# mickeysjm/TaxoExpan

Hardware: AMD Instinct MI355X
Metric: egonet_edges_per_sec_pgat_fwd_bwd (higher is better)
Workload: dtype f32; 1 GPU; MAG-CS synthetic taxonomy (29,654 nodes, d=250), PGAT+WMR+LBM fp32 dims 250/50/500/500 heads [4,1], 128 queries x 32 = 4096 egonets per GPU per step, fwd + InfoNCE + bwd + Adam(amsgrad), dropout 0.1; parallelism=dp1, settle_steps=256

## Files before the change

### include/txe.h

```cpp
#ifndef TXE_H
#define TXE_H
#include <stddef.h>

#ifdef __cplusplus
extern "C" {
#endif

#define TXE_OK 0
#define TXE_ERR_ARG -1
#define TXE_ERR_LAUNCH -2
#define TXE_ERR_WORKSPACE -3

size_t txe_dropout_mask_bytes(long long n_rows, int n_cols);
int txe_dropout_mask(long long n_rows, int n_cols, float p, unsigned long long seed, unsigned* mask, void* stream);

int txe_gat_padded_k(int Kh, int Pd);
int txe_gat_padded_f(int H, int D);
int txe_gat_pack_weights(const float* W, const float* attn_l, const float* attn_r, int H, int D, int Kt, float* Wp, void* stream);
int txe_gat_build_x(const float* h, long long ld_h, int n_nodes, int Kh, const int* pos, const float* P, int Pd, float* X, void* stream);

int txe_gat_layer_prepare(const float* h, long long ld_h, int n_nodes, int Kh, const int* pos, const float* P, int Pd, float* X,
                          const float* W, const float* attn_l, const float* attn_r, int H, int D, float* Wp, float feat_drop_p,
                          unsigned long long seed, unsigned* mask, void* stream);

struct txe_gat_prepare_desc {
    const float* h; long long ld_h; int n_nodes, Kh; const int* pos; const float* P; int Pd; float* X;
    const float *W, *attn_l, *attn_r; int H, D; float* Wp; float feat_drop_p; unsigned long long seed; unsigned* mask;
    int x_dropped;
};
int txe_gat_layers_prepare(const struct txe_gat_prepare_desc* descs, int n_layers, void* stream);

int txe_gcn_layer_prepare(const float* h, long long ld_h, int n_nodes, int Kh, const int* pos, const float* P, int Pd, float* X,
                          const float* W, int Fo, float* Wp, float drop_p, unsigned long long seed, unsigned* mask, int x_dropped,
                          const float* bias_row ,
                          void* stream);
struct txe_gcn_prepare_desc {
    const float* h; long long ld_h; int n_nodes, Kh; const int* pos; const float* P; int Pd; float* X;
    const float* W; int Fo; float* Wp; float drop_p; unsigned long long seed; unsigned* mask; int x_dropped; const float* bias_row;
};
int txe_gcn_layers_prepare(const struct txe_gcn_prepare_desc* descs, int n_layers, const int* rowptr_in, int n_nodes, float* norm, void* stream);

int txe_gather_add_rows(const float* T, long long ld_t, const int* row, const float* T2, long long ld_t2, const int* row2, long long n_rows,
                        int n_cols, float* Y, long long ld_y, void* stream);
size_t txe_gat_dense_ws_bytes(int n_nodes, int Kh, int Pd, int H, int D, int vocab);
int txe_gat_dense_fwd(const float* X, int n_nodes, int Kh, int Pd, const float* Wp, int H, int D, float feat_drop_p,
                      const unsigned* mask, float* Y, void* ws, size_t ws_bytes, void* stream);
size_t txe_gat_dense_split_ws_bytes(int n_nodes, int Kh, int Pd, int H, int D);
size_t txe_gat_dense_split_xt_bytes(int n_nodes, int Kh, int Pd, int H, int D);
int txe_gat_dense_fwd_split(const float* X, int n_nodes, int Kh, int Pd, const float* Wp, int H, int D, const void* Xs, const void* Ws,
                            void* Xt_out, float* Y, void* ws, size_t ws_bytes, void* stream);
int txe_gat_dense_fwd_split_src(const float* h, long long ld_h, const int* pos, const float* P, const unsigned* mask, float feat_drop_p,
                                int n_nodes, int Kh, int Pd, const float* Wp, int H, int D, void* Xt_out, float* Y, void* ws, size_t ws_bytes,
                                void* stream);
int txe_gat_dense_bwd(const float* X, int n_nodes, int Kh, int Pd, const int* pos, int vocab, const float* Wp, const float* W,
                      const float* attn_l, const float* attn_r, int H, int D, float feat_drop_p, const unsigned* mask, const float* d_Y,
                      int need_dh, int act_on, float act_slope, float* d_X, float* dW, float* d_attn_l, float* d_attn_r, float* dP,
                      int x_dropped, const void* Xt, int phases, void* chain, void* ws, size_t ws_bytes, void* stream);
size_t txe_gat_dense_bwd_split_ws_bytes(int n_nodes, int Kh, int Pd, int H, int D);
#define TXE_TAIL_CHAIN_BYTES 1024
int txe_gat_tail_flush(void* chain, void* stream);
int txe_zero_cols(float* x, long long ld, int n_rows, int c0, int c1, void* stream);
int txe_gat_dx_streams(int Kh, int Pd, int need_dh);

int txe_gat_aggregate_table_supported(int H, int D, long long ld_t, int vocab, int nx_kp);
int txe_gat_aggregate_table_fwd(const int* rowptr_in, const int* col_src, int n_nodes, const float* T, long long ld_t, const int* rid,
                                const float* T2, const int* pos, int vocab, int H, int D, float attn_slope, int out_mode,
                                float act_slope, float* out, long long ld_out, const float* nx_wa, int nx_kp, float* nx_a12,
                                int npw, void* stream);

int txe_gat_aggregate_fwd(const int* rowptr_in, const int* col_src, int n_nodes, const float* ft, long long ld_ft,
                          const float* a_src, const float* a_dst, int ld_a, int H, int D, float attn_slope, float attn_drop_p,
                          unsigned long long seed, int out_mode, float act_slope, float* out, long long ld_out, float* alpha,
                          const float* nx_wa, int nx_kp, const unsigned* nx_mask, float nx_feat_drop_p, float* nx_a12, int npw, void* stream);
int txe_gat_aggregate_bwd(const int* rowptr_in, const int* col_src, const int* rowptr_out, const int* col_dst,
                          const int* pos_out, int n_nodes, const float* ft, long long ld_ft, const float* a_src,
                          const float* a_dst, int ld_a, int H, int D, float attn_slope, float attn_drop_p,
                          unsigned long long seed, const float* alpha, const float* d_pre, long long ld_dpre, float* d_ft,
                          long long ld_dft, float* d_a_src, float* d_a_dst, int ld_da, float* dz_ws, int n_pad, void* stream);
int txe_leaky_relu_bwd(const float* d_out, const float* out_act, float slope, long long n, float* d_pre, void* stream);
int txe_head_mean_fwd(const float* x, int H, int D, long long n_rows, float* y, void* stream);
int txe_head_mean_bwd(const float* dy, int H, int D, long long n_rows, float* dx, void* stream);

int txe_gcn_padded_f(int Fo);
int txe_gcn_pack_weights(const float* W, int Kt, int Fo, float* Wp, void* stream);
size_t txe_gcn_dense_ws_bytes(int n_nodes, int Kh, int Pd, int Fo, int vocab);
int txe_gcn_dense_fwd(const float* X, int n_nodes, int Kh, int Pd, const float* Wp, int Fo, float drop_p, const unsigned* mask,
                      float* hw, void* ws, size_t ws_bytes, void* stream);
int txe_gcn_dense_bwd(const float* X, int n_nodes, int Kh, int Pd, const int* pos, int vocab, const float* Wp, int Fo, float drop_p,
                      const unsigned* mask, const float* d_hw, int need_dh, int act_on, float act_slope, float* d_X, float* dW,
                      float* dP, int x_dropped, void* ws, size_t ws_bytes, void* stream);
int txe_gcn_norm(const int* rowptr_in, int n_nodes, float* norm, void* stream);
int txe_gcn_aggregate_fwd(const int* rowptr_in, const int* col_src, int n_nodes, const float* hw, long long ld_hw,
                          const float* norm, const float* bias, int has_act, float act_slope, int F, float* out, long long ld_out,
                          void* stream);
size_t txe_gcn_aggregate_bwd_ws_bytes(int n_nodes, int F);
int txe_gcn_aggregate_bwd(const int* rowptr_out, const int* col_dst, int n_nodes, const float* d_pre, long long ld_dpre,
                          const float* norm, int F, float* d_hw, long long ld_dhw, float* d_bias, void* ws, size_t ws_bytes,
                          void* stream);

int txe_readout_fwd(const int* graph_off, int G, const float* h, long long ld_h, const int* pos, const float* pw, int D,
                    float* hg, float* wsum, void* stream);
int txe_readout_bwd(const int* graph_off, int G, const float* h, long long ld_h, const int* pos, const float* pw, int vocab,
                    int D, const float* hg, const float* wsum, const float* d_hg, float* d_h, long long ld_dh, float* d_pw,
                    float* dpw_ws, void* stream);

int txe_readout_multi_fwd(const int* graph_off, int G, const float* h, long long ld_h, const int* pos, int D, int mode, float* hg,
                          int* argmax, void* stream);
int txe_readout_multi_bwd(const int* graph_off, int G, const int* pos, int D, int mode, const float* d_hg, const int* argmax,
                          float* d_h, long long ld_dh, void* stream);

int txe_bilinear_project(const float* e1, long long ld_e1, int G, int l, const float* W, int r, float* U, long long ld_u,
                         void* sws, size_t sws_bytes, void* stream);
int txe_bilinear_pair_fwd(const float* e1, long long ld_e1, const float* e2, long long ld_e2, int G, int l, int r,
// ... 195 lines not shown
```

### taxoexpan_amd/_lib.py

```python
import ctypes as C
import os

_HERE = os.path.dirname(os.path.abspath(__file__))
LIB_PATH = os.path.join(_HERE, "csrc", "libtxe.so")
TAIL_CHAIN_BYTES = 1024

P, I, L, F, D, U64, SZ = C.c_void_p, C.c_int, C.c_longlong, C.c_float, C.c_double, C.c_ulonglong, C.c_size_t

SIGNATURES = {
    "txe_dropout_mask_bytes": (SZ, [L, I]),
    "txe_dropout_mask": (I, [L, I, F, U64, P, P]),
    "txe_gat_padded_k": (I, [I, I]),
    "txe_gat_padded_f": (I, [I, I]),
    "txe_gat_pack_weights": (I, [P, P, P, I, I, I, P, P]),
    "txe_gat_build_x": (I, [P, L, I, I, P, P, I, P, P]),
    "txe_gat_layer_prepare": (I, [P, L, I, I, P, P, I, P, P, P, P, I, I, P, F, U64, P, P]),
    "txe_gcn_layer_prepare": (I, [P, L, I, I, P, P, I, P, P, I, P, F, U64, P, I, P, P]),
    "txe_gcn_layers_prepare": (I, [P, I, P, I, P, P]),
    "txe_gather_add_rows": (I, [P, L, P, P, L, P, L, I, P, L, P]),
    "txe_gat_dense_ws_bytes": (SZ, [I, I, I, I, I, I]),
    "txe_gat_dense_fwd": (I, [P, I, I, I, P, I, I, F, P, P, P, SZ, P]),
    "txe_gat_dense_split_ws_bytes": (SZ, [I, I, I, I, I]),
    "txe_gat_dense_split_xt_bytes": (SZ, [I, I, I, I, I]),
    "txe_gat_dense_bwd_split_ws_bytes": (SZ, [I, I, I, I, I]),
    "txe_gat_dense_fwd_split": (I, [P, I, I, I, P, I, I, P, P, P, P, P, SZ, P]),
    "txe_gat_dense_bwd": (I, [P, I, I, I, P, I, P, P, P, P, I, I, F, P, P, I, I, F, P, P, P, P, P, I, P, I, P, P, SZ, P]),
    "txe_gat_tail_flush": (I, [P, P]),
    "txe_zero_cols": (I, [P, L, I, I, I, P]),
    "txe_gat_dx_streams": (I, [I, I, I]),
    "txe_gat_aggregate_fwd": (I, [P, P, I, P, L, P, P, I, I, I, F, F, U64, I, F, P, L, P, P, I, P, F, P, I, P]),
    "txe_gat_aggregate_table_supported": (I, [I, I, L, I, I]),
    "txe_gat_aggregate_table_fwd": (I, [P, P, I, P, L, P, P, P, I, I, I, F, I, F, P, L, P, I, P, I, P]),
    "txe_gat_aggregate_bwd": (I, [P, P, P, P, P, I, P, L, P, P, I, I, I, F, F, U64, P, P, L, P, L, P, P, I, P, I, P]),
    "txe_leaky_relu_bwd": (I, [P, P, F, L, P, P]),
    "txe_head_mean_fwd": (I, [P, I, I, L, P, P]),
    "txe_head_mean_bwd": (I, [P, I, I, L, P, P]),
    "txe_gcn_padded_f": (I, [I]),
    "txe_gcn_pack_weights": (I, [P, I, I, P, P]),
    "txe_gcn_dense_ws_bytes": (SZ, [I, I, I, I, I]),
    "txe_gcn_dense_fwd": (I, [P, I, I, I, P, I, F, P, P, P, SZ, P]),
    "txe_gcn_dense_bwd": (I, [P, I, I, I, P, I, P, I, F, P, P, I, I, F, P, P, P, I, P, SZ, P]),
    "txe_gcn_norm": (I, [P, I, P, P]),
    "txe_gcn_aggregate_fwd": (I, [P, P, I, P, L, P, P, I, F, I, P, L, P]),
    "txe_gcn_aggregate_bwd_ws_bytes": (SZ, [I, I]),
    "txe_gcn_aggregate_bwd": (I, [P, P, I, P, L, P, I, P, L, P, P, SZ, P]),
    "txe_readout_fwd": (I, [P, I, P, L, P, P, I, P, P, P]),
    "txe_readout_bwd": (I, [P, I, P, L, P, P, I, I, P, P, P, P, L, P, P, P]),
    "txe_readout_multi_fwd": (I, [P, I, P, L, P, I, I, P, P, P]),
    "txe_readout_multi_bwd": (I, [P, I, P, I, I, P, P, P, L, P]),
    "txe_linear_fwd": (I, [P, L, I, P, L, I, I, P, P, I, I, P, P]),
    "txe_linear_bwd_ws_bytes": (SZ, [I, I, I, I]),
    "txe_linear_bwd": (I, [P, L, I, P, L, I, I, P, I, I, P, P, P, L, P, L, P, P, P, SZ, P]),
    "txe_bilinear_project": (I, [P, L, I, I, P, I, P, L, P, SZ, P]),
    "txe_bilinear_pair_fwd": (I, [P, L, P, L, I, I, I, P, I, P, P, P]),
    "txe_bilinear_query_fwd": (I, [P, L, P, L, I, I, I, P, I, P, P, P]),
    "txe_bilinear_query_project": (I, [P, L, I, I, I, P, P, P]),
    "txe_bilinear_query_dot": (I, [P, L, P, I, I, I, P, P]),
    "txe_bilinear_query_bwd_ws_bytes": (SZ, [I, I, I]),
    "txe_bilinear_query_bwd": (I, [P, L, P, L, I, I, I, I, P, P, P, P, L, P, P, SZ, P]),
    "txe_bilinear_runs_fwd": (I, [P, L, P, L, P, I, I, I, I, P, I, P, P, P]),
    "txe_bilinear_runs_bwd_ws_bytes": (SZ, [I, I, I]),
    "txe_bilinear_runs_bwd": (I, [P, L, P, L, P, I, I, I, I, I, P, P, P, P, L, P, P, SZ, P]),
    "txe_rows_find_runs": (I, [P, L, I, I, P, P, P, P]),
    "txe_score_topk_tiles": (I, [I]),
    "txe_score_topk_block": (I, [P, L, I, P, L, I, I, I, I, I, I, P, P, P, P, P, P, SZ, P, P]),
    "txe_topk_merge": (I, [P, P, I, L, I, I, P, P, P]),
    "txe_bilinear_stacked_fwd": (I, [P, L, P, L, P, P, I, I, I, P, I, P, P, P]),
    "txe_bilinear_stacked_bwd_ws_bytes": (SZ, [I, I, I]),
    "txe_bilinear_stacked_bwd": (I, [P, L, P, L, P, P, I, I, I, I, P, P, P, P, L, P, P, SZ, P]),
    "txe_bilinear_folded_fwd": (I, [P, L, I, I, P, L, I, P, L, I, P, P, I, I, P, I, P, P, P, I, I, I, P]),
    "txe_runs_expand": (I, [P, I, I, P, P]),
    "txe_bilinear_folded_bwd": (I, [P, L, I, I, P, L, I, P, L, I, P, P, I, I, I, P, P, P, P, P, L, P, P, P, P, I, I, P]),
    "txe_bilinear_pair_bwd_ws_bytes": (SZ, [I, I, I]),
    "txe_bilinear_pair_bwd": (I, [P, L, P, L, I, I, I, P, I, P, P, P, P, L, P, L, P, P, SZ, P]),
    "txe_score_block": (I, [P, L, I, P, L, I, I, I, P, L, P, SZ, P, SZ, P, P]),
    "txe_mlp_padded_h": (I, [I]),
    "txe_mlp_project": (I, [P, L, I, I, P, P, P, P, P, P]),
    "txe_mlp_query_project": (I, [P, L, I, I, P, I, P, P, P, P, P]),
    "txe_mlp_score_block": (I, [P, P, I, P, P, P, I, I, P, P, L, P]),
    "txe_mlp_score_positives": (I, [P, P, I, P, P, P, I, I, P, P, P, I, P, P]),
    "txe_mlp_score_count_block": (I, [P, P, I, P, P, P, I, I, P, P, P, I, P, P]),
    "txe_mlp_score_topk_block": (I, [P, P, I, P, P, P, I, I, P, I, I, I, P, P, P, P, P, P]),
    "txe_score_split_ws_bytes": (SZ, [I, I, I]),
    "txe_score_count_block": (I, [P, L, I, P, L, I, I, I, P, P, I, P, P, SZ, P, P]),
    "txe_score_positives": (I, [P, L, I, P, L, I, I, I, P, P, P, SZ, P]),
    "txe_rank_finalize": (I, [P, I, P, P, I, P, P]),
    "txe_gemm_tail_ws_bytes": (SZ, []),
    "txe_gemm_plain_split_ws_bytes": (SZ, [I, I, I]),
    "txe_gat_collapse_split_ws_bytes": (SZ, [I, I, I, I]),
    "txe_gemm_plain": (I, [I, P, L, P, L, P, L, I, I, I, I, I, P, SZ, P]),
    "txe_build_csr_ws_bytes": (SZ, [I, I]),
    "txe_build_csr": (I, [P, P, I, I, P, P, P, P, P, P, P, SZ, P]),
    "txe_rank_block": (I, [P, L, I, I, P, P, P, I, P, P]),
    "txe_gat_collapse_ws_bytes": (SZ, [I, I, I, I, I, I, I]),
    "txe_gat_collapse_fwd": (I, [P, P, P, P, P, P, I, I, I, P, I, I, P, I, F, P, F, F, U64, P, P, P, I, P, P, P, P, P, P, L, P, P, P, P, SZ, P]),
    "txe_gat_collapse_e_tiles": (I, [I, I, I, I]),
    "txe_gat_collapse_fold_scores": (I, [P, I, I, I, I, P, P, P, F, I, I, P, P]),
    "txe_gat_collapse_bwd": (I, [P, P, P, P, P, P, I, I, I, P, I, I, P, I, P, P, P, P, I, F, P, F, F, U64, P, P, P, P, P, P, P, P, L, P, L, I, F,
                                 P, P, P, P, P, P, P, SZ, P]),
    "txe_gat_layers_prepare": (I, [P, I, P]),
    "txe_gat_fused_bwd_supported": (I, [I, I, I, I]),
    "txe_gat_collapse_bwd_fused_ws_bytes": (SZ, [I, I, I, I, I, I, I, I]),
    "txe_gat_collapse_bwd_fused": (I, [P, P, P, P, P, P, I, I, I, P, I, I, P, I, P, P, P, P, I, F, P, F, F, U64, P, P, P, P, P, P, P, P, L, P, L,
                                       F, P, L, I, I, F, F, U64, P, P, L, I, P, P, P, P, P, P, I, P, I, P, P, P, I, P, P, P, P, P, P, SZ, P]),
    "txe_gat_dense_fwd_split_src": (I, [P, L, P, P, P, F, I, I, I, P, I, I, P, P, P, SZ, P]),
    "txe_egonet_walk_plan_bytes": (SZ, [I]),
    "txe_egonet_walk_plan": (I, [P, P, P, P, P, P, I, I, P, P]),
    "txe_gcn_collapse_ws_bytes": (SZ, [I, I, I, I, I, I]),
    "txe_gcn_collapse_fwd": (I, [P, P, P, I, I, P, I, I, P, I, P, F, P, P, P, P, P, P, P, P, P, L, P, SZ, P]),
    "txe_gcn_collapse_bwd": (I, [P, P, P, I, I, P, I, I, P, I, P, I, F, P, P, P, P, P, P, P, P, L, I, F, P, P, P, P, P, I, P, SZ, P]),
    "txe_egonet_ws_bytes": (SZ, [I]),
    "txe_egonet_offsets": (I, [P, P, P, P, P, I, I, U64, I, P, P, SZ, P]),
    "txe_egonet_fill": (I, [P, P, P, P, P, P, I, I, U64, I, P, P, P, P, P, P, P, P, P, P]),
    "txe_sample_anchors": (I, [P, I, I, I, P, P, P, P, P, P, I, P, I, U64, I, I, P, P, P]),
    "txe_sample_groups": (I, [P, I, I, I, P, P, P, P, P, P, I, I, U64, I, I, I, P, P, P, P, P, P]),
    "txe_group_rank_ws_bytes": (SZ, [I]),
    "txe_group_rank": (I, [P, P, I, I, I, P, P, P, P, SZ, P]),
    "txe_group_metrics": (I, [P, P, P, U64, I, P, P]),
    "txe_info_nce": (I, [P, L, I, I, P, P, P, L, P]),
    "txe_adam_step": (I, [I, P, P, P, P, P, P, D, D, D, D, D, L, P]),
    "txe_dropout_uniform_host": (F, [U64, U64]),
    "txe_dropout_mask_word_host": (C.c_uint, [U64, U64, F]),
    "txe_profile_enable": (I, [I]),
    "txe_profile_reset": (I, []),
    "txe_profile_count": (I, []),
    "txe_profile_get": (I, [I, P, I, P, P, P]),
    "txe_profile_stream": (I, [I, P]),
    "txe_stream_order": (I, [P, P]),
    "txe_copy_stream": (I, [P, P, L, P]),
    "txe_split_packed_bytes": (SZ, [I, I]),
    "txe_split_pack": (I, [P, L, I, I, I, P, P]),
    "txe_split_packed_t_bytes": (SZ, [I, I]),
    "txe_split_pack_t": (I, [P, L, I, I, P, P]),
    "txe_gemm_tn_split": (I, [P, L, I, P, I, I, I, I, P, L, L, P]),
    "txe_gemm_nt_split": (I, [P, P, I, I, I, P, L, P]),
}

class GatPrepareDesc(C.Structure):
    _fields_ = [("h", P), ("ld_h", L), ("n_nodes", I), ("Kh", I), ("pos", P), ("P", P), ("Pd", I), ("X", P), ("W", P), ("attn_l", P),
                ("attn_r", P), ("H", I), ("D", I), ("Wp", P), ("feat_drop_p", F), ("seed", U64), ("mask", P), ("x_dropped", I)]


class GcnPrepareDesc(C.Structure):
    _fields_ = [("h", P), ("ld_h", L), ("n_nodes", I), ("Kh", I), ("pos", P), ("P", P), ("Pd", I), ("X", P), ("W", P), ("Fo", I), ("Wp", P),
                ("drop_p", F), ("seed", U64), ("mask", P), ("x_dropped", I), ("bias_row", P)]


_ERR = {-1: "TXE_ERR_ARG", -2: "TXE_ERR_LAUNCH", -3: "TXE_ERR_WORKSPACE"}
VALUE_RETURNING = {"txe_gat_padded_k", "txe_gat_collapse_e_tiles", "txe_gat_padded_f", "txe_gcn_padded_f", "txe_profile_count", "txe_gat_fused_bwd_supported",
                   "txe_gat_aggregate_table_supported", "txe_gat_dx_streams", "txe_score_topk_tiles",
                   "txe_mlp_padded_h"}

_lib = None


class TxeError(RuntimeError):
    pass


def load():
    global _lib
    if _lib is not None:
        return _lib
    if not os.path.exists(LIB_PATH):
        raise TxeError(f"HIP extension missing: {LIB_PATH} not built -- run taxoexpan_amd/csrc/build.py "
                       "(there is no CPU fallback)")
    lib = C.CDLL(LIB_PATH)
    for name, (res, args) in SIGNATURES.items():
        fn = getattr(lib, name)
        fn.restype, fn.argtypes = res, args
    _lib = lib
    return lib


_bound = {}


def call(name, *args):
    ent = _bound.get(name)
    if ent is None:
        ent = _bound[name] = (getattr(load(), name), SIGNATURES[name][0] is I and name not in VALUE_RETURNING)
    rc = ent[0](*args)
    if rc != 0 and ent[1]:
        raise TxeError(f"{name} failed: {_ERR.get(rc, rc)}")
    return rc


_pure = {}
_get_device = None


def _current_device():
    global _get_device
    if _get_device is None:
        import torch
        _get_device = torch._C._cuda_getDevice if torch.cuda.is_available() else (lambda: -1)
    return _get_device()


def pure(name, *args):
    key = (name, _current_device()) + args
    v = _pure.get(key)
    if v is None:
        if len(_pure) > 4096:
            _pure.clear()
        v = _pure[key] = call(name, *args)
    return v


class _NoGuard:
    def __enter__(self):
        return None

    def __exit__(self, *exc):
        return False


_NO_GUARD = _NoGuard()


def on_device(dev):
    import torch
    if dev.index is None or dev.index == torch.cuda.current_device():
        return _NO_GUARD
    return torch.cuda.device(dev)
# ... 20 lines not shown
```

### taxoexpan_amd/csrc/build.py

```python
#!/usr/bin/env python3
import concurrent.futures as cf
import os
import subprocess
import sys

HERE = os.path.dirname(os.path.abspath(__file__))
SOURCES = ["txe_gemm_nt.hip", "txe_gemm_nn.hip", "txe_gemm_tn.hip", "txe_gemm_split.hip", "txe_gat.hip", "txe_gcn.hip", "txe_project.hip", "txe_fold.hip", "txe_fold_bwd.hip", "txe_dxpos.hip", "txe_readout.hip", "txe_match.hip",
           "txe_graph.hip", "txe_rank.hip", "txe_profile.hip", "txe_egonet.hip", "txe_optim.hip", "txe_loss.hip",
           "txe_mlp_score.hip", "txe_sample.hip", "txe_grouprank.hip"]
HEADERS = ["txe_common.h", "txe_gemm.h", "txe_gather.h", "txe_colsum.h", "txe_dxpos.h", "txe_gemm_tnlds.h", "txe_skinny.h", "txe_gemm_split.h", "txe_tail.h", "txe_fold.h"]
LIB = os.path.join(HERE, "libtxe.so")
OBJ_DIR = os.path.join(HERE, "build")
HIPCC = os.environ.get("HIPCC", "/opt/rocm/bin/hipcc")
FLAGS = ["--offload-arch=gfx950", "-O3", "-std=c++17", "-fPIC", "-Wall", "-Wno-unused-function"] + os.environ.get("TXE_HIPCC_FLAGS", "").split()


def _newer(a, b):
    return (not os.path.exists(b)) or os.path.getmtime(a) > os.path.getmtime(b)


def _compile(src):
    obj = os.path.join(OBJ_DIR, src.replace(".hip", ".o"))
    deps = [os.path.join(HERE, src)] + [os.path.join(HERE, h) for h in HEADERS]
    if not any(_newer(d, obj) for d in deps):
        return obj, ""
    cmd = [HIPCC] + FLAGS + ["-c", os.path.join(HERE, src), "-o", obj]
    r = subprocess.run(cmd, capture_output=True, text=True)
    if r.returncode != 0:
        raise RuntimeError(f"hipcc failed for {src}:\n{r.stdout}\n{r.stderr}")
    return obj, r.stderr


def build(force=False, verbose=True):
    os.makedirs(OBJ_DIR, exist_ok=True)
    srcs = [s for s in SOURCES if os.path.exists(os.path.join(HERE, s))]
    if force:
        for s in srcs:
            o = os.path.join(OBJ_DIR, s.replace(".hip", ".o"))
            if os.path.exists(o):
                os.remove(o)
    with cf.ThreadPoolExecutor(max_workers=min(8, len(srcs))) as ex:
        results = list(ex.map(_compile, srcs))
    objs = [o for o, _ in results]
    warn = "".join(w for _, w in results)
    if verbose and warn.strip():
        print(warn, file=sys.stderr)
    if force or any(_newer(o, LIB) for o in objs):
        cmd = [HIPCC, "--offload-arch=gfx950", "-shared", "-fPIC"] + objs + ["-o", LIB]
        r = subprocess.run(cmd, capture_output=True, text=True)
        if r.returncode != 0:
            raise RuntimeError(f"link failed:\n{r.stdout}\n{r.stderr}")
    return LIB


if __name__ == "__main__":
    print(build(force="--force" in sys.argv))
```

### taxoexpan_amd/csrc/txe_gemm_split.h

```cpp
#pragma once
#include <hip/hip_runtime.h>
#include <stdint.h>

namespace txe {

constexpr int SPL_BM = 128, SPL_BN = 128, SPL_KT = 16;
constexpr int SPL_FRAG_BYTES = 1024;

static inline size_t split_packed_bytes(int rows, int cols) {
    const size_t rb = (size_t)((rows + 767) / 768) * 24, nkt = (size_t)(cols + SPL_KT - 1) / SPL_KT;
    return rb * nkt * 3 * SPL_FRAG_BYTES;
}

static inline size_t split_pair_bytes(int M, int N, int K) {
    return (split_packed_bytes(M, K) + 255) / 256 * 256 + (split_packed_bytes(N, K) + 255) / 256 * 256;
}

typedef float split_f2 __attribute__((ext_vector_type(2)));
typedef __bf16 split_b2 __attribute__((ext_vector_type(2)));
__device__ __forceinline__ unsigned pk_bf16(float lo, float hi) {
    const split_f2 v = {lo, hi};
    return __builtin_bit_cast(unsigned, __builtin_convertvector(v, split_b2));
}
__device__ __forceinline__ void split3x2(float x0, float x1, unsigned& w1, unsigned& w2, unsigned& w3) {
    w1 = pk_bf16(x0, x1);
    const float r0 = x0 - __uint_as_float(w1 << 16), r1 = x1 - __uint_as_float(w1 & 0xffff0000u);
    w2 = pk_bf16(r0, r1);
    const float q0 = r0 - __uint_as_float(w2 << 16), q1 = r1 - __uint_as_float(w2 & 0xffff0000u);
    w3 = pk_bf16(q0, q1);
}
constexpr unsigned SPL_RAW_MARK = 0x7FC07FC0u;
__device__ __forceinline__ bool split_exceptional(float x) {
    return (__float_as_uint(x) & 0x7fffffffu) >= (247u << 23);
}
__device__ __forceinline__ void split_raw2(float x0, float x1, unsigned& w1, unsigned& w2, unsigned& w3) {
    const unsigned b0 = __float_as_uint(x0), b1 = __float_as_uint(x1);
    w1 = (b0 >> 16) | (b1 & 0xffff0000u);
    w2 = (b0 & 0xffffu) | (b1 << 16);
    w3 = SPL_RAW_MARK;
}
__device__ __forceinline__ void split_decode8(const uint4& w1, const uint4& w2, const uint4& w3, float (&x)[8]) {
    const unsigned a[4] = {w1.x, w1.y, w1.z, w1.w}, b[4] = {w2.x, w2.y, w2.z, w2.w}, c[4] = {w3.x, w3.y, w3.z, w3.w};
    const bool raw = c[0] == SPL_RAW_MARK;
#pragma unroll
    for (int i = 0; i < 4; ++i) {
        if (raw) {
            x[2 * i] = __uint_as_float((a[i] << 16) | (b[i] & 0xffffu));
            x[2 * i + 1] = __uint_as_float((a[i] & 0xffff0000u) | (b[i] >> 16));
        } else {
            x[2 * i] = (__uint_as_float(a[i] << 16) + __uint_as_float(b[i] << 16)) + __uint_as_float(c[i] << 16);
            x[2 * i + 1] = (__uint_as_float(a[i] & 0xffff0000u) + __uint_as_float(b[i] & 0xffff0000u)) + __uint_as_float(c[i] & 0xffff0000u);
        }
    }
}
__device__ __forceinline__ bool not_finite(float v) { return (__float_as_uint(v) & 0x7f800000u) == 0x7f800000u; }

__device__ __forceinline__ void split3x8(const float (&x)[8], uint4& w1, uint4& w2, uint4& w3) {
    split3x2(x[0], x[1], w1.x, w2.x, w3.x);
    split3x2(x[2], x[3], w1.y, w2.y, w3.y);
    split3x2(x[4], x[5], w1.z, w2.z, w3.z);
    split3x2(x[6], x[7], w1.w, w2.w, w3.w);
}
__device__ __forceinline__ void split_raw8(const float (&x)[8], uint4& w1, uint4& w2, uint4& w3) {
    split_raw2(x[0], x[1], w1.x, w2.x, w3.x);
    split_raw2(x[2], x[3], w1.y, w2.y, w3.y);
    split_raw2(x[4], x[5], w1.z, w2.z, w3.z);
    split_raw2(x[6], x[7], w1.w, w2.w, w3.w);
}
__device__ __forceinline__ bool split_exceptional8(const float (&x)[8]) {
    bool bad = false;
#pragma unroll
    for (int q = 0; q < 8; ++q) bad |= split_exceptional(x[q]);
    return bad;
}
__device__ __forceinline__ void split3x4(const float (&x)[4], uint2& w1, uint2& w2, uint2& w3) {
    split3x2(x[0], x[1], w1.x, w2.x, w3.x);
    split3x2(x[2], x[3], w1.y, w2.y, w3.y);
}
__device__ __host__ __forceinline__ int split_slot_row(int side, int rb, int s) {
    return side == 0 ? 32 * rb + s : 128 * (rb >> 2) + 64 * ((rb & 3) >> 1) + 2 * s + (rb & 1);
}

static inline size_t split_packed_t_bytes(int rows, int cols) {
    return (size_t)((rows + 15) / 16) * (size_t)(((cols + 159) / 160) * 5) * 3 * SPL_FRAG_BYTES;
}
static inline bool split_tn_eligible(int M, int N) { return M % 128 == 0 && N % 4 == 0 && M > 0 && N > 0; }
static inline bool split_tn_fits(int n_rows, long long lda) { return (double)n_rows * (double)lda * 4.0 < 2147483648.0; }

int split_pack_launch(const float* src, long long ld, int rows, int cols, int side, void* packed, hipStream_t stream);
struct SplitEpi {
    const unsigned* mask; int mask_ld, mask_col0; float drop_scale;
    const float* act_src; long long ld_act; float act_slope; int cols_act;
};
int gemm_nt_split_launch(const void* Ap, const void* Bp, int M, int N, int K, float* C, long long ldc, double alg_flops, hipStream_t stream,
                         const SplitEpi* epi = nullptr);
int split_pack_t_launch(const float* src, long long ld, int rows, int cols, void* packed, hipStream_t stream);
struct Epi;
int gemm_nt_split_epi_launch(const void* Ap, const void* Bp, const Epi& E, int M, int N, int K, hipStream_t stream);
struct SplitVSrc { const float* h; long long ld_h; const int* pos; const float* P; int Kh, Pd; const unsigned* mask; int wpr; float scale; };
int split_pack_layer_launch(const float* X, long long ldx, int n, const float* W, long long ldw, int f, int K, int Kt_cols, void* Xs, void* Ws,
                            void* Xt, hipStream_t stream, const SplitVSrc* vs = nullptr);
int gemm_tn_split_launch(const float* A, long long lda, int M, const void* Bt, int N, int n_rows, int S, int ksplit, float* part, long long ldc,
                         long long split_stride, double alg_flops, hipStream_t stream);

}
```

### taxoexpan_amd/csrc/txe_gemm_split.hip

```cpp
#include <string.h>
#include "txe_common.h"
#include "txe_gemm.h"
#include "txe_gemm_split.h"

namespace txe {

typedef __attribute__((ext_vector_type(8))) short bf16x8;
typedef __attribute__((ext_vector_type(16))) float f32x16s;

template <int NC, int R>
__device__ __forceinline__ void vsrc_load_rows(const SplitVSrc& v, const int (&row)[R], const int c0, float (&x)[R][NC]) {
    unsigned word[R];
    const bool masked = v.mask != nullptr && c0 < v.wpr * 32;
#pragma unroll
    for (int r = 0; r < R; ++r) word[r] = masked ? v.mask[(long long)row[r] * v.wpr + (c0 >> 5)] : 0xFFFFFFFFu;
    if (c0 + NC <= v.Kh) {
        const bool two = (NC & 1) == 0 && ((reinterpret_cast<uintptr_t>(v.h + c0) & 7) == 0) && (v.ld_h & 1) == 0;
        if (two) {
#pragma unroll
            for (int r = 0; r < R; ++r) {
                const float* hr = v.h + (long long)row[r] * v.ld_h + c0;
#pragma unroll
                for (int q = 0; q + 1 < NC; q += 2) { const float2 t = *reinterpret_cast<const float2*>(hr + q); x[r][q] = t.x; x[r][q + 1] = t.y; }
            }
        } else {
#pragma unroll
            for (int r = 0; r < R; ++r)
#pragma unroll
                for (int q = 0; q < NC; ++q) x[r][q] = v.h[(long long)row[r] * v.ld_h + c0 + q];
        }
    } else if (c0 >= v.Kh + v.Pd) {
#pragma unroll
        for (int r = 0; r < R; ++r)
#pragma unroll
            for (int q = 0; q < NC; ++q) x[r][q] = 0.f;
        return;
    } else {
        int pr[R];
#pragma unroll
        for (int r = 0; r < R; ++r) pr[r] = (v.Pd > 0) ? v.pos[row[r]] : 0;
#pragma unroll
        for (int r = 0; r < R; ++r)
#pragma unroll
            for (int q = 0; q < NC; ++q) {
                const int c = c0 + q;
                const float hv = v.h[(long long)row[r] * v.ld_h + min(c, v.Kh - 1)];
                const float pv = (v.Pd > 0) ? v.P[(long long)pr[r] * v.Pd + min(max(c - v.Kh, 0), v.Pd - 1)] : 0.f;
                x[r][q] = (c < v.Kh) ? hv : ((c < v.Kh + v.Pd) ? pv : 0.f);
            }
    }
    if (masked) {
#pragma unroll
        for (int r = 0; r < R; ++r)
#pragma unroll
            for (int q = 0; q < NC; ++q) x[r][q] = ((word[r] >> ((c0 & 31) + q)) & 1u) ? x[r][q] * v.scale : 0.f;
    }
}
struct SplitPackArgs { const float* src; long long ld; int rows, cols, side, nrb, nkt; uint4* dst; int transposed; SplitVSrc v; };
__device__ __forceinline__ void split_pack_job(const SplitPackArgs& a, const int bid, const int nb) {
    const float* __restrict__ src = a.src;
    uint4* __restrict__ dst = a.dst;
    const int nkt = a.nkt, rows = a.rows, cols = a.cols;
    const long long ld = a.ld;
    const long long total = (long long)a.nrb * nkt * 64;
    for (long long i = (long long)bid * blockDim.x + threadIdx.x; i < total; i += (long long)nb * blockDim.x) {
        const int l = (int)(i & 63);
        const long long f = i >> 6;
        const int kt = (int)(f % nkt), rb = (int)(f / nkt);
        const int row = split_slot_row(a.side, rb, l & 31), k0 = kt * SPL_KT + 8 * (l >> 5);
        float x[8];
#pragma unroll
        for (int q = 0; q < 8; ++q) x[q] = 0.f;
        if (a.v.h != nullptr) {
            if (row < rows) {
                const int r1[1] = {row};
                float x1[1][8];
                vsrc_load_rows<8, 1>(a.v, r1, k0, x1);
#pragma unroll
                for (int q = 0; q < 8; ++q) x[q] = x1[0][q];
            }
        } else if (a.transposed) {
            if (row < rows) {
#pragma unroll
                for (int q = 0; q < 8; ++q)
                    if (k0 + q < cols) x[q] = src[(long long)(k0 + q) * ld + row];
            }
        } else if (row < rows) {
            const float* p = src + (long long)row * ld + k0;
            if (k0 + 7 < cols && ((reinterpret_cast<uintptr_t>(p) & 15) == 0)) {
                const float4 u = *reinterpret_cast<const float4*>(p), v = *reinterpret_cast<const float4*>(p + 4);
                x[0] = u.x; x[1] = u.y; x[2] = u.z; x[3] = u.w; x[4] = v.x; x[5] = v.y; x[6] = v.z; x[7] = v.w;
            } else {
#pragma unroll
                for (int q = 0; q < 8; ++q)
                    if (k0 + q < cols) x[q] = p[q];
            }
        }
        uint4 w1, w2, w3;
        if (__ballot(split_exceptional8(x)) != 0ull) split_raw8(x, w1, w2, w3);
        else split3x8(x, w1, w2, w3);
        uint4* o = dst + f * 3 * 64 + l;
        o[0] = w1; o[64] = w2; o[128] = w3;
    }
}
__global__ __launch_bounds__(256) void split_pack_kernel(const SplitPackArgs a) { split_pack_job(a, blockIdx.x, gridDim.x); }

struct SplitGemm {
    const char* A; const char* B;
    int nkt;
    float* C; long long ldc; int M, N;
    int nbm, nbn, apply_exp;
    const unsigned* mask; int mask_ld, mask_col0, mask_on; float drop_scale;
    const float* act_src; long long ld_act; float act_slope; int act_on, cols_act;
};

template <int MI>
__device__ __forceinline__ void gemm_nt_split_slow_tile(const char* __restrict__ A, const char* __restrict__ B, const int nkt, const int tm,
                                                        const int tn, float* __restrict__ Cs) {
    constexpr int NA = 2 * MI, NB = 4;
    const int c = threadIdx.x & 127;
    const uint4* fb0 = reinterpret_cast<const uint4*>(B + ((long long)(NB * tn + 2 * (c >> 6) + (c & 1)) * nkt * 3) * SPL_FRAG_BYTES) + ((c & 63) >> 1);
#pragma unroll 1
    for (int r = threadIdx.x >> 7; r < 64 * MI; r += 2) {
        const uint4* fa0 = reinterpret_cast<const uint4*>(A + ((long long)(NA * tm + (r >> 5)) * nkt * 3) * SPL_FRAG_BYTES) + (r & 31);
        float sum = 0.f;
#pragma unroll 1
        for (int h = 0; h < 2 * nkt; ++h) {
            const uint4* fa = fa0 + (h >> 1) * 192 + (h & 1) * 32;
            const uint4* fb = fb0 + (h >> 1) * 192 + (h & 1) * 32;
            float a[8], b[8];
            split_decode8(fa[0], fa[64], fa[128], a);
            split_decode8(fb[0], fb[64], fb[128], b);
#pragma unroll
            for (int q = 0; q < 8; ++q) sum = __builtin_fmaf(a[q], b[q], sum);
        }
        Cs[r * 129 + c] = sum;
    }
}

template <int MI, int NST, int MINB, int EPI = 0>
__global__ __launch_bounds__(256, MINB) void gemm_nt_split_kernel(const SplitGemm p, const Epi E) {
    constexpr int NA = 2 * MI, NB = 4;
    constexpr int NF = 3 * (NA + NB), CP = (NF + 3) / 4;
    static_assert(NST == 2 || NF % 4 == 0, "the three-stage ring waits on an exact copy count");
    constexpr int STAGE_U4 = NF * 64;
    __shared__ __attribute__((aligned(16))) uint4 smem_u4[NST * STAGE_U4];
    uint4* const st0 = smem_u4;
    uint4* const st1 = smem_u4 + STAGE_U4;
    uint4* const st2 = smem_u4 + (NST == 3 ? 2 : 0) * STAGE_U4;
    static_assert(EPI != 2 || (MI == 2 && NST * STAGE_U4 * 4 >= 128 * 132 + 128 * 10), "the epilogue's C tile + count scratch live in the stages");
    typedef __attribute__((address_space(3))) uint4 lds_u4;
    const int w = __builtin_amdgcn_readfirstlane(threadIdx.x >> 6), l = threadIdx.x & 63;
    const int lb = xcd_remap(blockIdx.x, gridDim.x);
    int tm, tn;
    {
        constexpr int GM = 16, GN = 8;
        const int srt = GM * p.nbn, sr = lb / srt, rem = lb - sr * srt;
        const int hgt = min(GM, p.nbm - sr * GM);
        const int cg = rem / (hgt * GN), r = rem - cg * hgt * GN, wg = min(GN, p.nbn - cg * GN);
        tm = sr * GM + r / wg; tn = cg * GN + r % wg;
    }
    const int wm = w >> 1, wn = w & 1;
    const int nkt = p.nkt;
    int cnt_pb = 0, cnt_np = 0;
    float cnt_th[8] = {0.f, 0.f, 0.f, 0.f, 0.f, 0.f, 0.f, 0.f};
    if constexpr (EPI == 2) {
        const int m0 = tm * 128, n0 = tn * SPL_BN;
        if (E.cnt_mode == 3) {
            const int lo = E.cnt_off[m0], hi = E.cnt_off[min(m0 + 128, p.M)];
            if (n0 >= hi || n0 + SPL_BN <= lo) return;
        }
        if ((E.cnt_mode == 1 || E.cnt_mode == 2) && threadIdx.x < 128 && m0 + (int)threadIdx.x < p.M) {
            cnt_pb = E.cnt_off[m0 + threadIdx.x];
            cnt_np = E.cnt_off[m0 + threadIdx.x + 1] - cnt_pb;
#pragma unroll
            for (int k = 0; k < 8; ++k) cnt_th[k] = E.cnt_thr[(k < cnt_np) ? cnt_pb + k : 0];
        }
    }
    const char* gsrc[CP];
#pragma unroll
    for (int q = 0; q < CP; ++q) {
        const int f = min(CP * w + q, NF - 1);
        const bool isa = f < 3 * NA;
        const int blk = isa ? f / 3 : (f - 3 * NA) / 3, pl = isa ? f % 3 : (f - 3 * NA) % 3;
        const char* base = isa ? p.A : p.B;
        const long long b0 = isa ? (long long)NA * tm + blk : (long long)NB * tn + blk;
        gsrc[q] = base + (b0 * nkt) * (3 * SPL_FRAG_BYTES) + pl * SPL_FRAG_BYTES;
// ... 72 lines not shown
#undef TXE_SP_STEP
#undef TXE_SP_SYNC
#undef TXE_SP_COMPUTE
#undef TXE_SP_MFMA
#undef TXE_SP_PRODUCTS
#undef TXE_SP_ISSUE
#undef TXE_SP_COPY

    {
        bool odd = false;
#pragma unroll
        for (int i = 0; i < MI; ++i)
#pragma unroll
            for (int j = 0; j < 2; ++j)
#pragma unroll
                for (int e = 0; e < 16; ++e) odd |= not_finite(acc[i][j][e]);
        static_assert(NST * STAGE_U4 * 4 >= 64 * MI * 129, "the recomputed tile lives in the stage ring");
        if (__syncthreads_or(odd)) {
            float* Cs = reinterpret_cast<float*>(smem_u4);
            gemm_nt_split_slow_tile<MI>(p.A, p.B, nkt, tm, tn, Cs);
            __syncthreads();
#pragma unroll
            for (int i = 0; i < MI; ++i)
#pragma unroll
                for (int j = 0; j < 2; ++j)
#pragma unroll
                    for (int e = 0; e < 16; ++e)
                        acc[i][j][e] = Cs[(32 * MI * wm + 32 * i + 4 * (l >> 5) + (e & 3) + 8 * (e >> 2)) * 129 + 64 * wn + 2 * (l & 31) + j];
            __syncthreads();
        }
    }

    if constexpr (EPI == 2) {
        float* Cs = reinterpret_cast<float*>(smem_u4);
        __syncthreads();
#pragma unroll
        for (int i = 0; i < MI; ++i)
#pragma unroll
            for (int j = 0; j < 2; ++j)
#pragma unroll
                for (int e = 0; e < 16; ++e) {
                    const int row = 32 * MI * wm + 32 * i + 4 * (l >> 5) + (e & 3) + 8 * (e >> 2);
                    Cs[row * 132 + 64 * wn + 2 * (l & 31) + j] = acc[i][j][e];
                }
        __syncthreads();
        gemm_tile_epilogue<128, NST * STAGE_U4 * 4>(E, Cs, tm * 128, tn * SPL_BN, p.M, p.N, tn, p.nbn, 0, cnt_pb, cnt_np, cnt_th);
        return;
    }
    const int c0 = tn * SPL_BN + 64 * wn + 2 * (l & 31);
    const int r0 = tm * (64 * MI) + 32 * MI * wm + 4 * (l >> 5);
    const bool vec = ((p.ldc & 1) == 0) && ((reinterpret_cast<uintptr_t>(p.C) & 7) == 0);
#pragma unroll
    for (int i = 0; i < MI; ++i)
#pragma unroll
        for (int e = 0; e < 16; ++e) {
            const int m = r0 + 32 * i + (e & 3) + 8 * (e >> 2);
            if (m < p.M) {
                float* dst = p.C + (long long)m * p.ldc + c0;
                float v0 = acc[i][0][e], v1 = acc[i][1][e];
                if constexpr (EPI == 1) {
#pragma unroll
                    for (int q = 0; q < 2; ++q) {
                        const int c = c0 + q;
                        if (c >= p.N) continue;
                        float g = 1.f;
                        if (p.mask_on) {
                            const int cm = c + p.mask_col0;
                            g = ((p.mask[(long long)m * p.mask_ld + (cm >> 5)] >> (cm & 31)) & 1u) ? p.drop_scale : 0.f;
                        }
                        if (p.act_on && c < p.cols_act && !(p.act_src[(long long)m * p.ld_act + c] > 0.f)) g *= p.act_slope;
                        if (q == 0) v0 *= g; else v1 *= g;
                    }
                }
                if (p.apply_exp) { v0 = __expf(v0); v1 = __expf(v1); }
                if (vec && c0 + 1 < p.N) *reinterpret_cast<float2*>(dst) = make_float2(v0, v1);
                else {
                    if (c0 < p.N) dst[0] = v0;
                    if (c0 + 1 < p.N) dst[1] = v1;
                }
            }
        }
}

struct SplitPackTArgs { const float* src; long long ld; int rows, cols, nht, nnt; uint4* dst; SplitVSrc v; };
__device__ __forceinline__ void split_pack_t_job(const SplitPackTArgs& a, const int bid, const int nb) {
    const float* __restrict__ src = a.src;
    uint4* __restrict__ dst = a.dst;
    const int rows = a.rows, nht = a.nht;
    const long long ld = a.ld;
    const long long total = (long long)a.nnt * nht * 64;
    const int nkb = nht * 5;
    for (long long i = (long long)bid * blockDim.x + threadIdx.x; i < total; i += (long long)nb * blockDim.x) {
        const int l = (int)(i & 63), s = l & 31, nh = l >> 5;
        const long long g = i >> 6;
        const int h = (int)(g % nht), nt = (int)(g / nht);
        const int n0 = nt * 16 + nh * 8;
        float4 q[8];
        float o[8];
        const int c4 = min(160 * h + 4 * s, a.cols - 4), c1 = min(160 * h + 128 + s, a.cols - 1);
        const bool ok4 = 160 * h + 4 * s + 3 < a.cols, ok1 = 160 * h + 128 + s < a.cols;
        if (a.v.h != nullptr) {
            int rr[8];
            float t4[8][4], t1[8][1];
#pragma unroll
            for (int r = 0; r < 8; ++r) rr[r] = min(n0 + r, rows - 1);
            vsrc_load_rows<4, 8>(a.v, rr, c4, t4);
            vsrc_load_rows<1, 8>(a.v, rr, c1, t1);
#pragma unroll
            for (int r = 0; r < 8; ++r) { q[r] = make_float4(t4[r][0], t4[r][1], t4[r][2], t4[r][3]); o[r] = t1[r][0]; }
        } else {
#pragma unroll
        for (int r = 0; r < 8; ++r) {
            const int row = min(n0 + r, rows - 1);
            const float* p = src + (long long)row * ld;
            q[r] = *reinterpret_cast<const float4*>(p + c4);
            o[r] = p[c1];
        }
        }
#pragma unroll
        for (int r = 0; r < 8; ++r) {
            if (n0 + r >= rows || !ok4) q[r] = make_float4(0.f, 0.f, 0.f, 0.f);
            if (n0 + r >= rows || !ok1) o[r] = 0.f;
        }
        uint4* base = dst + ((long long)nt * nkb + 5 * h) * 3 * 64 + l;
#pragma unroll
        for (int j = 0; j < 5; ++j) {
            float x[8];
#pragma unroll
            for (int r = 0; r < 8; ++r) x[r] = j == 0 ? q[r].x : (j == 1 ? q[r].y : (j == 2 ? q[r].z : (j == 3 ? q[r].w : o[r])));
            uint4 w1, w2, w3;
            if (__ballot(split_exceptional8(x)) != 0ull) split_raw8(x, w1, w2, w3);
            else split3x8(x, w1, w2, w3);
            base[(j * 3 + 0) * 64] = w1; base[(j * 3 + 1) * 64] = w2; base[(j * 3 + 2) * 64] = w3;
        }
    }
}
__global__ __launch_bounds__(256) void split_pack_t_kernel(const SplitPackTArgs a) { split_pack_t_job(a, blockIdx.x, gridDim.x); }

struct SplitPackMulti { SplitPackArgs a[2]; SplitPackTArgs t; int nb[3]; };
__global__ __launch_bounds__(256) void split_pack_multi_kernel(const SplitPackMulti m) {
    int b = blockIdx.x;
    if (b < m.nb[0]) { split_pack_job(m.a[0], b, m.nb[0]); return; }
    b -= m.nb[0];
    if (b < m.nb[1]) { split_pack_job(m.a[1], b, m.nb[1]); return; }
    split_pack_t_job(m.t, b - m.nb[1], m.nb[2]);
}

struct SplitTn {
    const float* A; long long lda; const char* Bt; int nkb;
    float* C; long long ldc, split_stride;
    int n_rows, ksplit, ntm, ntn, N;
};
constexpr int SPT_A_U4 = 4 * 3 * 64, SPT_B_U4 = 5 * 3 * 64, SPT_STAGE_U4 = SPT_A_U4 + SPT_B_U4;
constexpr int SPT_RAW_F = 16 * 128;

__device__ __forceinline__ void gemm_tn_split_slow_block(const SplitTn& p, const int tm, const int h, const int kbeg, const int kend,
                                                         const int blk, float* __restrict__ Cs) {
#pragma unroll 1
    for (int o = threadIdx.x; o < 32 * 160; o += 256) {
        const int sa = o / 160, cc = o - sa * 160;
        const int j = cc < 128 ? (cc & 3) : 4, sb = cc < 128 ? (cc >> 2) : cc - 128;
        const float* a = p.A + (long long)tm * 128 + 64 * (blk >> 1) + 2 * sa + (blk & 1);
        float sum = 0.f;
#pragma unroll 1
        for (int n0 = kbeg; n0 < kend; n0 += 8) {
            const uint4* f = reinterpret_cast<const uint4*>(p.Bt + ((((long long)(n0 >> 4) * p.nkb + 5 * h + j) * 3) * SPL_FRAG_BYTES)) + ((n0 >> 3) & 1) * 32 + sb;
            float b[8];
            split_decode8(f[0], f[64], f[128], b);
#pragma unroll
            for (int q = 0; q < 8; ++q)
                if (n0 + q < kend) sum = __builtin_fmaf(a[(long long)(n0 + q) * p.lda], b[q], sum);
        }
        Cs[sa * 161 + cc] = sum;
    }
}

__global__ __launch_bounds__(256, 2) void gemm_tn_split_kernel(const SplitTn p) {
    __shared__ __attribute__((aligned(16))) uint4 st0[SPT_STAGE_U4];
    __shared__ __attribute__((aligned(16))) uint4 st1[SPT_STAGE_U4];
    __shared__ __attribute__((aligned(16))) float raw0[SPT_RAW_F];
    __shared__ __attribute__((aligned(16))) float raw1[SPT_RAW_F];
    typedef __attribute__((address_space(3))) uint4 lds_u4;
    typedef __attribute__((address_space(3))) float lds_f;
    const int w = __builtin_amdgcn_readfirstlane(threadIdx.x >> 6), l = threadIdx.x & 63;
    const int ntiles = p.ntm * p.ntn;
    const int vb = xcd_remap(blockIdx.x, gridDim.x);
    const int z = vb / ntiles, lb = vb % ntiles;
    const int tm = lb / p.ntn, h = lb % p.ntn;
    const int kbeg = z * p.ksplit, kend = min(p.n_rows, kbeg + p.ksplit);
    const int nk = kend > kbeg ? (kend - kbeg + 15) / 16 : 0;
    const char* gb = p.Bt + (((long long)(kbeg / 16) * p.nkb + 5 * h) * 3 + 4 * w) * SPL_FRAG_BYTES;
    const long long adv_b = (long long)p.nkb * 3 * SPL_FRAG_BYTES;
    const unsigned lane_off = l * 16;
    const float* ga = p.A + (long long)tm * 128;
    const unsigned a_col = (l & 31) * 16;
    const int last_row = p.n_rows - 1;
    const int g = l >> 5, s = l & 31;

    f32x16s acc[5];
#pragma unroll
    for (int j = 0; j < 5; ++j)
#pragma unroll
        for (int e = 0; e < 16; ++e) acc[j][e] = 0.f;

#define TXE_ST_COPY(v_, g_, d_)                                                                                       \
    asm volatile("s_mov_b32 m0, %2\n\tglobal_load_lds_dwordx4 %0, %1" ::"v"(v_), "s"(g_), "s"((unsigned)(uintptr_t)(d_)) : "memory");
#define TXE_ST_ISSUE_B(st_, t_)                                                                                       \
    {                                                                                                                \
        const char* sb = gb + (long long)min((t_), nk - 1) * adv_b;                                                  \
        lds_u4* d0 = (lds_u4*)(st_) + SPT_A_U4 + (4 * w) * 64;                                                       \
        const int q3 = w < 3 ? 3 : 2;                                                                                \
        TXE_ST_COPY(lane_off, sb, d0)                                                                                \
        TXE_ST_COPY(lane_off, sb + SPL_FRAG_BYTES, d0 + 64)                                                          \
        TXE_ST_COPY(lane_off, sb + 2 * SPL_FRAG_BYTES, d0 + 128)                                                     \
        TXE_ST_COPY(lane_off, sb + q3 * SPL_FRAG_BYTES, d0 + q3 * 64)                                                \
    }
#define TXE_ST_ISSUE_A(raw_, t_)                                                                                      \
    _Pragma("unroll") for (int i = 0; i < 2; ++i) {                                                                  \
        const int row = min(kbeg + min((t_), nk - 1) * 16 + 4 * w + 2 * i + (l >> 5), last_row);                     \
// ... 14 lines not shown
    }
#define TXE_ST_MFMA(pa_, pb_)                                                                                         \
    _Pragma("unroll") for (int j = 0; j < 5; ++j)                                                                    \
        acc[j] = __builtin_amdgcn_mfma_f32_32x32x16_bf16(fa[pa_], fb[j][pb_], acc[j], 0, 0, 0);
#define TXE_ST_COMPUTE(st_)                                                                                           \
    {                                                                                                                \
        bf16x8 fa[3], fb[5][3];                                                                                      \
        _Pragma("unroll") for (int c = 0; c < 3; ++c) fa[c] = __builtin_bit_cast(bf16x8, (st_)[(w * 3 + c) * 64 + l]); \
        _Pragma("unroll") for (int j = 0; j < 5; ++j)                                                                \
            _Pragma("unroll") for (int c = 0; c < 3; ++c)                                                            \
                fb[j][c] = __builtin_bit_cast(bf16x8, (st_)[SPT_A_U4 + (j * 3 + c) * 64 + l]);                       \
        TXE_ST_MFMA(2, 0) TXE_ST_MFMA(0, 2) TXE_ST_MFMA(1, 1) TXE_ST_MFMA(1, 0) TXE_ST_MFMA(0, 1) TXE_ST_MFMA(0, 0)  \
    }
#define TXE_ST_STEP(cur_, nxt_, rcur_, rnxt_, t_)                                                                     \
    asm volatile("s_waitcnt vmcnt(2)" ::: "memory");                                            \
    __syncthreads();                                          \
    TXE_ST_ISSUE_B(nxt_, (t_) + 1)                                                                                   \
    TXE_ST_ISSUE_A(rcur_, (t_) + 2)                                     \
    __builtin_amdgcn_sched_barrier(0);                                                                               \
    TXE_ST_COMPUTE(cur_)                                                                                             \
    __builtin_amdgcn_sched_barrier(0);                                                                               \
    asm volatile("s_waitcnt vmcnt(6)" ::: "memory");                   \
    if ((t_) + 1 < nk) TXE_ST_CONVERT(rnxt_, nxt_)

    if (nk > 0) {
        TXE_ST_ISSUE_B(st0, 0)
        TXE_ST_ISSUE_A(raw0, 0)
        TXE_ST_ISSUE_A(raw1, 1)
        asm volatile("s_waitcnt vmcnt(2)" ::: "memory");
        TXE_ST_CONVERT(raw0, st0)
        for (int t = 0; t < nk; t += 2) {
            TXE_ST_STEP(st0, st1, raw0, raw1, t)
            if (t + 1 >= nk) break;
            TXE_ST_STEP(st1, st0, raw1, raw0, t + 1)
        }
        asm volatile("s_waitcnt vmcnt(0)" ::: "memory");
    }
#undef TXE_ST_STEP
#undef TXE_ST_COMPUTE
#undef TXE_ST_MFMA
#undef TXE_ST_CONVERT
#undef TXE_ST_ISSUE_A
#undef TXE_ST_ISSUE_B
#undef TXE_ST_COPY

    {
        bool odd = false;
#pragma unroll
        for (int j = 0; j < 5; ++j)
#pragma unroll
            for (int e = 0; e < 16; ++e) odd |= not_finite(acc[j][e]);
        static_assert(SPT_STAGE_U4 * 4 >= 32 * 161, "a block's recomputed rows live in one fragment stage");
        if (__syncthreads_or(odd)) {
            float* Cs = reinterpret_cast<float*>(st0);
#pragma unroll 1
            for (int blk = 0; blk < 4; ++blk) {
                gemm_tn_split_slow_block(p, tm, h, kbeg, kend, blk, Cs);
                __syncthreads();
                if (blk == w) {
#pragma unroll
                    for (int e = 0; e < 16; ++e) {
                        const float* row = Cs + ((e & 3) + 8 * (e >> 2) + 4 * (l >> 5)) * 161;
#pragma unroll
                        for (int j = 0; j < 4; ++j) acc[j][e] = row[4 * (l & 31) + j];
                        acc[4][e] = row[128 + (l & 31)];
                    }
                }
                __syncthreads();
            }
        }
    }

    float* cb = p.C + (long long)z * p.split_stride + (long long)(tm * 128 + 64 * (w >> 1) + (w & 1)) * p.ldc + 160 * h;
    const int sl = l & 31;
#pragma unroll
    for (int e = 0; e < 16; ++e) {
        const int slot = (e & 3) + 8 * (e >> 2) + 4 * (l >> 5);
        float* dst = cb + (long long)(2 * slot) * p.ldc;
        if (160 * h + 4 * sl + 3 < p.N) *reinterpret_cast<float4*>(dst + 4 * sl) = make_float4(acc[0][e], acc[1][e], acc[2][e], acc[3][e]);
        if (160 * h + 128 + sl < p.N) dst[128 + sl] = acc[4][e];
    }
}

static bool fill_pack(SplitPackArgs& a, int& nb, const float* src, long long ld, int rows, int cols, int side, void* packed) {
    const int tr = side >> 1;
    if (!src || !packed || rows < 1 || cols < 1 || ld < (tr ? rows : cols) || side < 0 || side > 3) return false;
    a.src = src; a.ld = ld; a.rows = rows; a.cols = cols; a.side = side & 1; a.dst = (uint4*)packed; a.transposed = tr;
    memset(&a.v, 0, sizeof(a.v));
    a.nrb = ((rows + 767) / 768) * 24; a.nkt = (cols + SPL_KT - 1) / SPL_KT;
    const long long total = (long long)a.nrb * a.nkt * 64;
    nb = (int)((total + 255) / 256 < 8192 ? (total + 255) / 256 : 8192);
    return true;
}
static bool fill_pack_t(SplitPackTArgs& a, int& nb, const float* src, long long ld, int rows, int cols, void* packed) {
    if (!src || !packed || rows < 1 || cols < 4 || cols % 4 != 0 || ld < cols || (ld & 3) != 0 || (reinterpret_cast<uintptr_t>(src) & 15) != 0)
        return false;
    a.src = src; a.ld = ld; a.rows = rows; a.cols = cols; a.nht = (cols + 159) / 160; a.nnt = (rows + 15) / 16; a.dst = (uint4*)packed;
    memset(&a.v, 0, sizeof(a.v));
    const long long total = (long long)a.nnt * a.nht * 64;
    nb = (int)((total + 255) / 256);
    return true;
}
int split_pack_launch(const float* src, long long ld, int rows, int cols, int side, void* packed, hipStream_t stream) {
    SplitPackArgs a;
    int nb;
    if (!fill_pack(a, nb, src, ld, rows, cols, side, packed)) return TXE_ERR_ARG;
    ProfScope prof("split_pack_kernel", stream, 10.0 * rows * (double)cols, 1);
    hipLaunchKernelGGL(split_pack_kernel, dim3(nb), dim3(256), 0, stream, a);
    TXE_CHECK_LAUNCH();
    return TXE_OK;
}
int split_pack_layer_launch(const float* X, long long ldx, int n, const float* W, long long ldw, int f, int K, int Kt_cols, void* Xs, void* Ws,
                            void* Xt, hipStream_t stream, const SplitVSrc* vs) {
    SplitPackMulti m;
    memset(&m, 0, sizeof(m));
    if (vs && (!vs->h || vs->Kh < 1 || vs->Pd < 0 || vs->ld_h < vs->Kh || (vs->Pd > 0 && (!vs->pos || !vs->P)) || (vs->mask && vs->wpr < 1))) return TXE_ERR_ARG;
    if (vs) X = reinterpret_cast<const float*>(W);
    if (!fill_pack(m.a[0], m.nb[0], X, ldx, n, K, 0, Xs) || !fill_pack(m.a[1], m.nb[1], W, ldw, f, K, 1, Ws)) return TXE_ERR_ARG;
    if (Xt && !fill_pack_t(m.t, m.nb[2], X, ldx, n, Kt_cols, Xt)) return TXE_ERR_ARG;
    if (vs) { m.a[0].v = *vs; m.t.v = *vs; }
    ProfScope prof("split_pack_multi_kernel", stream, 10.0 * K * ((Xt ? 2.0 : 1.0) * n + f), 1);
    hipLaunchKernelGGL(split_pack_multi_kernel, dim3(m.nb[0] + m.nb[1] + m.nb[2]), dim3(256), 0, stream, m);
    TXE_CHECK_LAUNCH();
    return TXE_OK;
}

int gemm_nt_split_launch(const void* Ap, const void* Bp, int M, int N, int K, float* C, long long ldc, double alg_flops, hipStream_t stream,
                         const SplitEpi* epi) {
    if (!Ap || !Bp || !C || M < 1 || N < 1 || K < 1 || ldc < N) return TXE_ERR_ARG;
    SplitGemm p;
    memset(&p, 0, sizeof(p));
    p.A = (const char*)Ap; p.B = (const char*)Bp; p.nkt = (K + SPL_KT - 1) / SPL_KT;
    p.C = C; p.ldc = ldc; p.M = M; p.N = N;
    p.nbm = (M + 127) / 128; p.nbn = (N + SPL_BN - 1) / SPL_BN;
    const Epi E0 = epi_plain(C, ldc, N);
    ProfScope prof(epi ? "gemm_nt_split_kernel<2, 3, 2, 1>" : "gemm_nt_split_kernel<2, 3, 2, 0>", stream, alg_flops > 0.0 ? alg_flops : 2.0 * M * (double)N * K, 0);
    const dim3 grid(p.nbm * p.nbn), blk(256);
    if (epi) {
        p.mask = epi->mask; p.mask_ld = epi->mask_ld; p.mask_col0 = epi->mask_col0; p.mask_on = epi->mask ? 1 : 0;
        p.drop_scale = epi->drop_scale;
        p.act_src = epi->act_src; p.ld_act = epi->ld_act; p.act_slope = epi->act_slope; p.act_on = epi->act_src ? 1 : 0; p.cols_act = epi->cols_act;
        hipLaunchKernelGGL((gemm_nt_split_kernel<2, 3, 2, 1>), grid, blk, 0, stream, p, E0);
        TXE_CHECK_LAUNCH();
        return TXE_OK;
    }
    hipLaunchKernelGGL((gemm_nt_split_kernel<2, 3, 2>), grid, blk, 0, stream, p, E0);
    TXE_CHECK_LAUNCH();
    return TXE_OK;
}

int gemm_nt_split_epi_launch(const void* Ap, const void* Bp, const Epi& E, int M, int N, int K, hipStream_t stream) {
    if (!Ap || !Bp || M < 1 || N < 1 || K < 1 || E.mask_on || E.act_on || E.c2) return TXE_ERR_ARG;
    SplitGemm p;
    memset(&p, 0, sizeof(p));
    p.A = (const char*)Ap; p.B = (const char*)Bp; p.nkt = (K + SPL_KT - 1) / SPL_KT;
    p.C = E.c; p.ldc = E.ldc; p.M = M; p.N = N;
    p.nbm = (M + 127) / 128; p.nbn = (N + SPL_BN - 1) / SPL_BN;
    Epi E2 = E;
    {
        const void* valid = E2.c ? (const void*)E2.c : (const void*)Ap;
        E2.act_src = (const float*)valid;
        E2.mask = (const unsigned*)valid;
    }
    ProfScope prof("gemm_nt_split_kernel<2, 3, 2, 2>", stream, E.alg_flops > 0.0 ? E.alg_flops : 2.0 * M * (double)N * K, 0);
    hipLaunchKernelGGL((gemm_nt_split_kernel<2, 3, 2, 2>), dim3(p.nbm * p.nbn), dim3(256), 0, stream, p, E2);
    TXE_CHECK_LAUNCH();
    return TXE_OK;
}

int split_pack_t_launch(const float* src, long long ld, int rows, int cols, void* packed, hipStream_t stream) {
    SplitPackTArgs a;
    int nb;
    if (!fill_pack_t(a, nb, src, ld, rows, cols, packed)) return TXE_ERR_ARG;
    ProfScope prof("split_pack_t_kernel", stream, 10.0 * rows * (double)cols, 1);
    hipLaunchKernelGGL(split_pack_t_kernel, dim3(nb), dim3(256), 0, stream, a);
    TXE_CHECK_LAUNCH();
    return TXE_OK;
}

int gemm_tn_split_launch(const float* A, long long lda, int M, const void* Bt, int N, int n_rows, int S, int ksplit, float* part, long long ldc,
                         long long split_stride, double alg_flops, hipStream_t stream) {
    if (!A || !Bt || !part || !split_tn_eligible(M, N) || n_rows < 1 || S < 1 || ksplit < 16 || ksplit % 16 != 0 || ldc < N || (ldc & 3) != 0 ||
        (lda & 3) != 0 || (reinterpret_cast<uintptr_t>(A) & 15) != 0 || !split_tn_fits(n_rows, lda) || (reinterpret_cast<uintptr_t>(part) & 15) != 0 || (split_stride & 3) != 0)
        return TXE_ERR_ARG;
    SplitTn p;
    p.A = A; p.lda = lda; p.Bt = (const char*)Bt; p.nkb = ((N + 159) / 160) * 5; p.N = N;
    p.C = part; p.ldc = ldc; p.split_stride = split_stride;
    p.n_rows = n_rows; p.ksplit = ksplit; p.ntm = M / 128; p.ntn = (N + 159) / 160;
    ProfScope prof("gemm_tn_split_kernel", stream, alg_flops > 0.0 ? alg_flops : 2.0 * M * (double)N * n_rows, 0);
    hipLaunchKernelGGL(gemm_tn_split_kernel, dim3(p.ntm * p.ntn * S), dim3(256), 0, stream, p);
    TXE_CHECK_LAUNCH();
    return TXE_OK;
}

}
using namespace txe;
extern "C" {

size_t txe_split_packed_bytes(int rows, int cols) { return (rows < 1 || cols < 1) ? 0 : split_packed_bytes(rows, cols); }

int txe_split_pack(const float* src, long long ld, int rows, int cols, int side, void* packed, void* stream) {
    return split_pack_launch(src, ld, rows, cols, side, packed, (hipStream_t)stream);
}

// ... 17 lines not shown
```

### taxoexpan_amd/csrc/txe_project.hip

```cpp
#include <string.h>

#include "txe_gemm.h"
#include "txe_gather.h"
#include "txe_dxpos.h"
#include "txe_gemm_split.h"
#include "txe_tail.h"

namespace txe {

constexpr int FOLD_DG = 16;
__device__ __forceinline__ void fold_attn_job(const int bx, const int r , const float* __restrict__ W, long long ldw, int Kt,
                                              const float* __restrict__ attn_l, const float* __restrict__ attn_r, int H, int D,
                                              float* __restrict__ wa, long long ld_wa) {
    __shared__ float red[FOLD_DG][64];
    const int h = r % H;
    const float* attn = ((r < H) ? attn_l : attn_r) + (long long)h * D;
    const float* Wh = W + (long long)h * D * ldw;
    const int kl = threadIdx.x & 63, dg = threadIdx.x >> 6;
    const int k = bx * 64 + kl;
    const int kc = (k < Kt) ? k : 0;
    float acc = 0.f;
#pragma unroll 4
    for (int d = dg; d < D; d += FOLD_DG) acc = fmaf(attn[d], Wh[(long long)d * ldw + kc], acc);
    red[dg][kl] = acc;
    __syncthreads();
    if (dg == 0 && k < Kt) {
        float s = 0.f;
#pragma unroll
        for (int g = 0; g < FOLD_DG; ++g) s += red[g][kl];
        wa[(long long)r * ld_wa + k] = s;
    }
}
__global__ __launch_bounds__(64 * FOLD_DG) void fold_attn_kernel(const float* __restrict__ W, long long ldw, int Kt,
                                                                 const float* __restrict__ attn_l, const float* __restrict__ attn_r,
                                                                 int H, int D, float* __restrict__ wa, long long ld_wa) {
    fold_attn_job(blockIdx.x, blockIdx.y, W, ldw, Kt, attn_l, attn_r, H, D, wa, ld_wa);
}

__global__ void reduce_ext_rows_kernel(const float* __restrict__ part, int S, long long split_stride, int F, int H2, int ldp,
                                       float* __restrict__ dwa) {
    ext_rows_job(blockIdx.y, blockIdx.x * blockDim.x + threadIdx.x, part, S, split_stride, F, ldp, dwa);
}

__device__ __forceinline__ void unfold_job(const int f, const UnfoldArgs& a) {
    __shared__ float red[2][4];
    const int h = f / a.D;
    const float al = a.attn_l[f], ar = a.attn_r[f];
    float dl = 0.f, dr = 0.f;
    for (int k = threadIdx.x; k < a.Kt; k += blockDim.x) {
        const float* pp = a.part + (long long)f * a.ldp + k;
        const float gl = a.dwa[(long long)h * a.ldp + k], gr = a.dwa[(long long)(a.H + h) * a.ldp + k];
        const float wv = a.W[(long long)f * a.ldw + k];
        float acc = 0.f;
        for (int s0 = 0; s0 < a.S; s0 += 8) {
            float v[8];
#pragma unroll
            for (int j = 0; j < 8; ++j) v[j] = pp[(long long)min(s0 + j, a.S - 1) * a.split_stride];
#pragma unroll
            for (int j = 0; j < 8; ++j) acc += (s0 + j < a.S) ? v[j] : 0.f;
        }
        a.dW[(long long)f * a.ld_dw + k] = acc + al * gl + ar * gr;
        dl = fmaf(gl, wv, dl);
        dr = fmaf(gr, wv, dr);
    }
    dl = wave_sum(dl);
    dr = wave_sum(dr);
    const int w = threadIdx.x >> 6;
    if ((threadIdx.x & 63) == 0) { red[0][w] = dl; red[1][w] = dr; }
    __syncthreads();
    if (threadIdx.x == 0) {
        a.d_attn_l[f] = red[0][0] + red[0][1] + red[0][2] + red[0][3];
        a.d_attn_r[f] = red[1][0] + red[1][1] + red[1][2] + red[1][3];
    }
}

__global__ void reduce_splits_kernel(const float* __restrict__ part, int S, long long stride, long long n, float* __restrict__ out) {
    for (long long i = (long long)blockIdx.x * blockDim.x + threadIdx.x; i < n; i += (long long)gridDim.x * blockDim.x) {
        float acc = 0.f;
        for (int s = 0; s < S; ++s) acc += part[(long long)s * stride + i];
        out[i] = acc;
    }
}

__global__ __launch_bounds__(256) void pos_segsum_stage1(const float* __restrict__ x, long long ldx, const int* __restrict__ pos,
                                                         int n_rows, int cols, int vocab, int rows_per_block,
                                                         float* __restrict__ part ) {
    Seg1Args a{x, ldx, cols, part};
    segsum1_job(blockIdx.x, a, pos, n_rows, vocab, rows_per_block);
}
__global__ __launch_bounds__(256) void pos_segsum_stage2(const float* __restrict__ part, int nb, int vocab, int cols,
                                                         float* __restrict__ out) {
    Seg2Args a{part, nb, vocab * cols, out};
    segsum2_job(blockIdx.x, a);
}
int pos_segsum_launch(const float* x, long long ldx, const int* pos, int n_rows, int cols, int vocab, int nb, int rows_per_block, float* part,
                      float* out, hipStream_t s) {
    if (n_rows > 0) {
        hipLaunchKernelGGL(pos_segsum_stage1, dim3(nb), dim3(256), 0, s, x, ldx, pos, n_rows, cols, vocab, rows_per_block, part);
        TXE_CHECK_LAUNCH();
    }
    hipLaunchKernelGGL(pos_segsum_stage2, dim3((vocab * cols + 63) / 64), dim3(256), 0, s, (const float*)part, n_rows > 0 ? nb : 0, vocab, cols, out);
    TXE_CHECK_LAUNCH();
    return TXE_OK;
}

__global__ __launch_bounds__(256) void gat_bwd_reduce_a_kernel(const TailA a) { reduce_a_job(blockIdx.x, a); }
int tail_a_launch(const TailA& a, hipStream_t s) {
    hipLaunchKernelGGL(gat_bwd_reduce_a_kernel, dim3(a.nb_dx + a.nb_s1a + a.nb_s1b + a.nb_r), dim3(256), 0, s, a);
    TXE_CHECK_LAUNCH();
    return TXE_OK;
}
__device__ __forceinline__ void tail_b_job(int b, const TailB& a) {
    if (b < a.nb_u) { unfold_job(b, a.u); return; }
    b -= a.nb_u;
    if (b < a.nb_2a) { segsum2_job(b, a.s2a); return; }
    segsum2_job(b - a.nb_2a, a.s2b);
}
__global__ __launch_bounds__(256) void gat_bwd_reduce_b_kernel(const TailB a) { tail_b_job(blockIdx.x, a); }

// ... 135 lines not shown
            if (h) {
#pragma unroll
                for (int u = 0; u < PREP_UX; ++u) {
                    const float* hrow = h + (long long)(r0 + max(li[u], 0)) * ld_h;
                    const int c = ci[u];
                    if (v2) {
                        const float2 a = *reinterpret_cast<const float2*>(hrow + min(c, Kh - 2));
                        const float2 b = *reinterpret_cast<const float2*>(hrow + min(c + 2, Kh - 2));
                        hv[u][0] = a.x; hv[u][1] = a.y; hv[u][2] = b.x; hv[u][3] = b.y;
                    } else {
#pragma unroll
                        for (int e = 0; e < 4; ++e) hv[u][e] = hrow[min(c + e, Kh - 1)];
                    }
                }
            }
            if (lds_words && pb == 0) {
                for (int wi = threadIdx.x; wi < nr * nw; wi += T) {
                    const int lr = wi / nw, wl = w_lo + (wi - lr * nw);
                    const unsigned long long w = (unsigned long long)(r0 + lr) * wpr + wl;
                    const unsigned word = (wl < wpr) ? drop_mask_word(drop_seed, w, drop_thr16) : 0u;
                    s_words[wi] = word;
                    if (mask && wl < wpr) mask[w] = word;
                }
                __syncthreads();
            }
            if (Pd > 0) {
#pragma unroll
                for (int u = 0; u < PREP_UX; ++u) {
                    const float* prow = P + (long long)pr[u] * Pd;
#pragma unroll
                    for (int e = 0; e < 4; ++e) pv[u][e] = prow[min(max(ci[u] + e - Kh, 0), Pd - 1)];
                }
            }
#pragma unroll
            for (int u = 0; u < PREP_UX; ++u) {
                if (li[u] < 0) continue;
                const int r = r0 + li[u], c = ci[u];
                float v[4];
#pragma unroll
                for (int e = 0; e < 4; ++e) v[e] = (c + e < Kh) ? (h ? hv[u][e] : 0.f) : ((c + e < Kt) ? pv[u][e] : 0.f);
                if (drop && c < Kt) {
                    const unsigned word = lds_words ? s_words[li[u] * nw + (c >> 5) - w_lo]
                                                    : drop_mask_word(drop_seed, (unsigned long long)r * wpr + (c >> 5), drop_thr16);
#pragma unroll
                    for (int e = 0; e < 4; ++e)
                        v[e] = ((word >> ((c & 31) + e)) & 1u) ? v[e] * drop_scale : 0.f;
                }
                float* dst = X + (long long)r * Kp + c;
                if (!h && c < Kh) {
#pragma unroll
                    for (int e = 0; e < 4; ++e)
                        if (c + e >= Kh) dst[e] = v[e];
                } else {
                    *reinterpret_cast<float4*>(dst) = make_float4(v[0], v[1], v[2], v[3]);
                }
            }
        }
        if (lds_words) __syncthreads();
    }
}
__global__ void build_x_kernel(const float* __restrict__ h, long long ld_h, const int* __restrict__ pos, const float* __restrict__ P,
                               int n_rows, int Kh, int Pd, int Kp, float* __restrict__ X) {
    build_x_job(blockIdx.x, gridDim.x, h, ld_h, pos, P, n_rows, Kh, Pd, Kp, X);
}

static inline int build_x_blocks(int T, int n_rows, int Kh, int Pd, int Kp, bool has_h, bool drop, int cap) {
    const int q0 = has_h ? 0 : (Kh >> 2), qn = (Kp >> 2) - q0, nw = (Kp >> 5) - ((q0 * 4) >> 5);
    if (qn <= 0 || n_rows <= 0) return 0;
    int RB = (T * PREP_UX) / qn;
    if (RB < 1) RB = 1;
    if (drop && nw <= PREP_LDSW && RB * nw > PREP_LDSW) RB = PREP_LDSW / nw;
    const long long b = ((long long)n_rows + RB - 1) / RB;
    return (int)(b < cap ? b : cap);
}
struct PrepArgs {
    int nb_x, nb_w, nb_f, nb_m, fold_bx;
    const float* h; long long ld_h; const int* pos; const float* P; int n_rows, Kh, Pd, Kp; float* X;
    const float *W, *attn_l, *attn_r; int H, D, F, Fe, Fp, Kt; float* Wp;
    int pk_rows, pk_ext, pk_prows, pk_cols, pk_pcols;
    const float* pk_extra;
    long long n_words; unsigned long long seed; unsigned thr16; unsigned* mask;
    int x_dropped; float drop_scale;
    int x_mask;
};
__device__ __forceinline__ void prepare_jobs(const PrepArgs& a, int b) {
    if (b < a.nb_f) {
        fold_attn_job(b % a.fold_bx, b / a.fold_bx, a.W, (long long)a.Kt, a.Kt, a.attn_l, a.attn_r, a.H, a.D, a.Wp + (long long)a.F * a.Kp,
                      (long long)a.Kp);
        return;
    }
    b -= a.nb_f;
    if (b < a.nb_w) { pack_w_job(b, a.nb_w, a.W, a.pk_rows, a.pk_ext, a.pk_prows, a.pk_cols, a.pk_pcols, a.Wp, a.pk_extra); return; }
    b -= a.nb_w;
    if (b < a.nb_m) { dropout_mask_job(b, a.nb_m, a.n_words, a.seed, a.thr16, a.mask); return; }
    b -= a.nb_m;
    build_x_job(b, a.nb_x, a.h, a.ld_h, a.pos, a.P, a.n_rows, a.Kh, a.Pd, a.Kp, a.X, a.seed, a.x_dropped ? a.thr16 : 0u, a.drop_scale,
                a.x_mask ? a.mask : nullptr);
}
__global__ __launch_bounds__(64 * FOLD_DG) void gat_prepare_kernel(const PrepArgs a) { prepare_jobs(a, blockIdx.x); }

__global__ void zero_cols_kernel(float* __restrict__ x, long long ld, int n_rows, int c0, int c1) {
    const int wdt = c1 - c0;
    const long long n = (long long)n_rows * wdt;
    for (long long i = (long long)blockIdx.x * blockDim.x + threadIdx.x; i < n; i += (long long)gridDim.x * blockDim.x)
        x[(i / wdt) * ld + c0 + (i % wdt)] = 0.f;
}

__global__ __launch_bounds__(256) void gather_add_rows_kernel(const float* __restrict__ T, long long ld_t, const int* __restrict__ row,
                                                              const float* __restrict__ T2, long long ld_t2, const int* __restrict__ row2,
                                                              long long n_rows, int nvec, float* __restrict__ Y, long long ld_y) {
    const long long total = n_rows * nvec;
    for (long long i = (long long)blockIdx.x * blockDim.x + threadIdx.x; i < total; i += (long long)gridDim.x * blockDim.x) {
        const long long v = i / nvec;
        const int j = (int)(i % nvec);
        float4 a = *reinterpret_cast<const float4*>(T + (long long)row[v] * ld_t + 4 * j);
        if (T2) {
            const float4 b = *reinterpret_cast<const float4*>(T2 + (long long)row2[v] * ld_t2 + 4 * j);
            a.x += b.x; a.y += b.y; a.z += b.z; a.w += b.w;
        }
        *reinterpret_cast<float4*>(Y + v * ld_y + 4 * j) = a;
    }
}

struct DenseWs {
    float* dwa;
    float* dxpart;
    float* ppart;
    float* part;
    void* tail;
    size_t tail_bytes;
    int splits, seg_blocks, seg_rows;
    size_t total;
};

static DenseWs plan_dense_ws(void* ws, int n, int Fp, int H2, int Kp, int Pd, int vocab, bool dx_stream = true, int min_splits = 0) {
    DenseWs p;
    char* b = (char*)ws;
    size_t off = 0;
    auto take = [&](size_t bytes) { float* r = (float*)(b + off); off += align_up(bytes, 256); return r; };
    p.dwa = take((size_t)H2 * Kp * 4);
    p.seg_rows = 64;
    p.seg_blocks = (n + p.seg_rows - 1) / p.seg_rows;
    if (p.seg_blocks < 1) p.seg_blocks = 1;
    const int ppart_blocks = dxpos_blocks(n) > p.seg_blocks ? dxpos_blocks(n) : p.seg_blocks;
    p.ppart = take((size_t)ppart_blocks * (vocab > 0 ? vocab : 1) * (Pd > 0 ? Pd : 1) * 4);
    p.dxpart = take((Pd > 0 && dx_stream) ? dxpos_part_bytes(n, Fp) : 0);
    p.splits = choose_splits(Fp, Kp, n);
    p.part = take((size_t)(p.splits > min_splits ? p.splits : min_splits) * Fp * Kp * 4);
    p.tail_bytes = gemm_tail_ws_bytes();
    p.tail = take(p.tail_bytes);
    p.total = off;
    return p;
}

static int gcn_dwt_splits(int n, int Kp, int Fop) {
    if (n < 4096 || ((Kp + 159) / 160) * 160 > ((Kp + 63) / 64) * 64) return 0;
    const int tiles = ((Fop + 127) / 128) * ((Kp + 159) / 160);
    const int slots = 2 * device_cu_count();
    int S = slots / tiles;
    const int nkt = (n + GEMM_BK - 1) / GEMM_BK;
    if (S > nkt / 8) S = nkt / 8;
    if (S > 64) S = 64;
    return S >= 2 ? S : 0;
}
__global__ __launch_bounds__(256) void reduce_splits_transposed_kernel(const float* __restrict__ part, int S, long long stride, int rows, int cols,
                                                                        int ldp, float* __restrict__ out) {
    __shared__ float tile[8][33];
    const int f0 = blockIdx.x * 8, k0 = blockIdx.y * 32;
    const int tx = threadIdx.x & 31, ty = threadIdx.x >> 5;
    const int f = min(f0 + ty, cols - 1), k = min(k0 + tx, rows - 1);
    const float* p = part + (long long)f * ldp + k;
    float acc = 0.f;
    for (int s0 = 0; s0 < S; s0 += 16) {
        float v[16];
#pragma unroll
        for (int q = 0; q < 16; ++q) v[q] = p[(long long)min(s0 + q, S - 1) * stride];
#pragma unroll
        for (int q = 0; q < 16; ++q) acc += (s0 + q < S) ? v[q] : 0.f;
    }
    tile[ty][tx] = acc;
    __syncthreads();
    const int kk = threadIdx.x >> 3, ff = threadIdx.x & 7;
    if (k0 + kk < rows && f0 + ff < cols) out[(long long)(k0 + kk) * cols + f0 + ff] = tile[ff][kk];
}

}
using namespace txe;
extern "C" {

int txe_gat_padded_k(int Kh, int Pd) { return round_up(Kh + Pd, 32); }
int txe_gat_padded_f(int H, int D) { return round_up(H * D + 2 * H, 128); }

int txe_gat_pack_weights(const float* W, const float* attn_l, const float* attn_r, int H, int D, int Kt, float* Wp, void* stream) {
    if (!W || !attn_l || !attn_r || !Wp || H < 1 || D < 1 || Kt < 1) return TXE_ERR_ARG;
    const int F = H * D, Fe = F + 2 * H, Fp = round_up(Fe, 128), Kp = round_up(Kt, 32);
    hipStream_t s = (hipStream_t)stream;
    const long long n = (long long)Fp * Kp;
    hipLaunchKernelGGL(pack_w_kernel, dim3((int)((n + 255) / 256 < 2048 ? (n + 255) / 256 : 2048)), dim3(256), 0, s, W, F, Fe, Fp, Kt, Kp, Wp);
    hipLaunchKernelGGL(fold_attn_kernel, dim3((Kt + 63) / 64, 2 * H), dim3(64 * FOLD_DG), 0, s, W, (long long)Kt, Kt, attn_l, attn_r, H, D,
                       Wp + (long long)F * Kp, (long long)Kp);
    TXE_CHECK_LAUNCH();
    return TXE_OK;
}

int txe_gat_build_x(const float* h, long long ld_h, int n_nodes, int Kh, const int* pos, const float* P, int Pd, float* X, void* stream) {
    if (n_nodes < 0 || Kh < 1 || Pd < 0 || !X || (Pd > 0 && (!pos || !P))) return TXE_ERR_ARG;
    if (n_nodes == 0) return TXE_OK;
    const int Kp = round_up(Kh + Pd, 32);
    const long long n = (long long)n_nodes * (Kp - (h ? 0 : Kh));
    if (n == 0) return TXE_OK;
    hipLaunchKernelGGL(build_x_kernel, dim3((int)((n + 255) / 256 < 4096 ? (n + 255) / 256 : 4096)), dim3(256), 0, (hipStream_t)stream, h,
                       ld_h, pos, P, n_nodes, Kh, Pd, Kp, X);
    TXE_CHECK_LAUNCH();
    return TXE_OK;
}

int txe_gat_layer_prepare(const float* h, long long ld_h, int n_nodes, int Kh, const int* pos, const float* P, int Pd, float* X,
                          const float* W, const float* attn_l, const float* attn_r, int H, int D, float* Wp, float feat_drop_p,
                          unsigned long long seed, unsigned* mask, void* stream) {
    if (n_nodes < 0 || Kh < 1 || Pd < 0 || !X || (Pd > 0 && (!pos || !P)) || !W || !attn_l || !attn_r || !Wp || H < 1 || D < 1)
        return TXE_ERR_ARG;
    if (feat_drop_p < 0.f || feat_drop_p >= 1.f || (feat_drop_p > 0.f && !mask)) return TXE_ERR_ARG;
    const int T = 64 * FOLD_DG;
    PrepArgs a;
    memset(&a, 0, sizeof(a));
    a.Kt = Kh + Pd; a.Kp = round_up(a.Kt, 32);
    a.F = H * D; a.Fe = a.F + 2 * H; a.Fp = round_up(a.Fe, 128);
    auto blocks = [&](long long n, int cap) { const long long b = (n + T - 1) / T; return (int)(b < cap ? b : cap); };
    const long long nx = (long long)n_nodes * (a.Kp - (h ? 0 : Kh));
    a.nb_x = nx > 0 ? build_x_blocks(T, n_nodes, Kh, Pd, a.Kp, h != nullptr, false, 2048) : 0;
    a.n_words = (feat_drop_p > 0.f) ? (long long)n_nodes * ((a.Kt + 31) / 32) : 0;
    a.nb_m = blocks(a.n_words, 1024);
    a.nb_w = blocks(((long long)a.Fp * a.Kp / 4 + PREP_U - 1) / PREP_U, 512);
    a.fold_bx = (a.Kt + 63) / 64;
    a.nb_f = a.fold_bx * 2 * H;
    a.h = h; a.ld_h = ld_h; a.pos = pos; a.P = P; a.n_rows = n_nodes; a.Kh = Kh; a.Pd = Pd; a.X = X;
    a.W = W; a.attn_l = attn_l; a.attn_r = attn_r; a.H = H; a.D = D; a.Wp = Wp;
    a.pk_rows = a.F; a.pk_ext = a.Fe; a.pk_prows = a.Fp; a.pk_cols = a.Kt; a.pk_pcols = a.Kp;
    a.seed = seed; a.thr16 = (unsigned)(feat_drop_p * 65536.0f + 0.5f); a.mask = mask;
    a.x_dropped = 0; a.drop_scale = 1.f;
    hipLaunchKernelGGL(gat_prepare_kernel, dim3(a.nb_x + a.nb_m + a.nb_w + a.nb_f), dim3(T), 0, (hipStream_t)stream, a);
    TXE_CHECK_LAUNCH();
    return TXE_OK;
}

struct txe_gat_prepare_desc {
    const float* h; long long ld_h; int n_nodes, Kh; const int* pos; const float* P; int Pd; float* X;
    const float *W, *attn_l, *attn_r; int H, D; float* Wp; float feat_drop_p; unsigned long long seed; unsigned* mask;
    int x_dropped;
};
}
namespace txe {
constexpr int PREP_MAXL = 4;
struct PrepMulti {
    int n; int nb_end[PREP_MAXL]; PrepArgs a[PREP_MAXL];
    int nb_norm; const int* norm_rowptr; int norm_n; float* norm;
};
__global__ __launch_bounds__(64 * FOLD_DG) void gat_prepare_multi_kernel(const PrepMulti m) {
    int b = blockIdx.x, i = 0;
    if (b < m.nb_norm) {
        const int v = b * (64 * FOLD_DG) + threadIdx.x;
        if (v < m.norm_n) { const int deg = m.norm_rowptr[v + 1] - m.norm_rowptr[v]; m.norm[v] = deg > 0 ? 1.0f / sqrtf((float)deg) : 0.f; }
        return;
    }
    b -= m.nb_norm;
    while (i + 1 < m.n && b >= m.nb_end[i]) ++i;
    prepare_jobs(m.a[i], b - ((i > 0) ? m.nb_end[i - 1] : 0));
}
static int fill_prep(PrepArgs& a, const txe_gat_prepare_desc& d) {
    if (d.n_nodes < 0 || d.Kh < 1 || d.Pd < 0 || (!d.X && !d.h) || (d.Pd > 0 && (!d.pos || !d.P)) || !d.W || !d.attn_l || !d.attn_r || !d.Wp || d.H < 1 ||
        d.D < 1 || d.feat_drop_p < 0.f || d.feat_drop_p >= 1.f || (d.feat_drop_p > 0.f && !d.mask))
        return TXE_ERR_ARG;
    const int T = 64 * FOLD_DG;
    a.Kt = d.Kh + d.Pd; a.Kp = round_up(a.Kt, 32);
    a.F = d.H * d.D; a.Fe = a.F + 2 * d.H; a.Fp = round_up(a.Fe, 128);
    auto blocks = [&](long long n, int cap) { const long long b = (n + T - 1) / T; return (int)(b < cap ? b : cap); };
    const long long nx = d.X ? (long long)d.n_nodes * (a.Kp - (d.h ? 0 : d.Kh)) : 0;
    a.seed = d.seed; a.thr16 = (unsigned)(d.feat_drop_p * 65536.0f + 0.5f); a.mask = d.mask;
    a.x_dropped = (d.x_dropped && d.feat_drop_p > 0.f && a.thr16 != 0u) ? 1 : 0;
    a.x_mask = (a.x_dropped && d.h != nullptr && nx > 0) ? 1 : 0;
    a.drop_scale = 1.f / (1.f - d.feat_drop_p);
    a.nb_x = nx > 0 ? build_x_blocks(T, d.n_nodes, d.Kh, d.Pd, a.Kp, d.h != nullptr, a.x_dropped != 0, 2048) : 0;
    a.n_words = (d.feat_drop_p > 0.f) ? (long long)d.n_nodes * ((a.Kt + 31) / 32) : 0;
    a.nb_m = a.x_mask ? 0 : blocks(a.n_words, 1024);
    a.nb_w = blocks(((long long)a.Fp * a.Kp / 4 + PREP_U - 1) / PREP_U, 512);
    a.fold_bx = (a.Kt + 63) / 64;
    a.nb_f = a.fold_bx * 2 * d.H;
    a.h = d.h; a.ld_h = d.ld_h; a.pos = d.pos; a.P = d.P; a.n_rows = d.n_nodes; a.Kh = d.Kh; a.Pd = d.Pd; a.X = d.X;
    a.W = d.W; a.attn_l = d.attn_l; a.attn_r = d.attn_r; a.H = d.H; a.D = d.D; a.Wp = d.Wp;
    a.pk_rows = a.F; a.pk_ext = a.Fe; a.pk_prows = a.Fp; a.pk_cols = a.Kt; a.pk_pcols = a.Kp;
    return TXE_OK;
}
}
extern "C" {
int txe_gat_layers_prepare(const struct txe_gat_prepare_desc* descs, int n_layers, void* stream) {
    if (!descs || n_layers < 1) return TXE_ERR_ARG;
    for (int i0 = 0; i0 < n_layers; i0 += PREP_MAXL) {
        PrepMulti m;
        memset(&m, 0, sizeof(m));
        m.n = n_layers - i0 < PREP_MAXL ? n_layers - i0 : PREP_MAXL;
        int total = 0;
        for (int i = 0; i < m.n; ++i) {
            const int rc = fill_prep(m.a[i], descs[i0 + i]);
            if (rc) return rc;
            total += m.a[i].nb_x + m.a[i].nb_m + m.a[i].nb_w + m.a[i].nb_f;
            m.nb_end[i] = total;
        }
        if (total == 0) continue;
        hipLaunchKernelGGL(gat_prepare_multi_kernel, dim3(total), dim3(64 * FOLD_DG), 0, (hipStream_t)stream, m);
        TXE_CHECK_LAUNCH();
    }
    return TXE_OK;
}

struct txe_gcn_prepare_desc {
    const float* h; long long ld_h; int n_nodes, Kh; const int* pos; const float* P; int Pd; float* X;
    const float* W; int Fo; float* Wp; float drop_p; unsigned long long seed; unsigned* mask; int x_dropped; const float* bias_row;
};
}
namespace txe {
static int fill_prep_gcn(PrepArgs& a, const txe_gcn_prepare_desc& d) {
    if (d.n_nodes < 0 || d.Kh < 1 || d.Pd < 0 || !d.X || (d.Pd > 0 && (!d.pos || !d.P)) || !d.W || !d.Wp || d.Fo < 1) return TXE_ERR_ARG;
    if (d.bias_row && ((d.Kh + d.Pd) % 32) == 0) return TXE_ERR_ARG;
    if (d.drop_p < 0.f || d.drop_p >= 1.f || (d.drop_p > 0.f && !d.mask)) return TXE_ERR_ARG;
    const int T = 64 * FOLD_DG;
    memset(&a, 0, sizeof(a));
    a.Kt = d.Kh + d.Pd; a.Kp = round_up(a.Kt, 32);
    auto blocks = [&](long long n, int cap) { const long long b = (n + T - 1) / T; return (int)(b < cap ? b : cap); };
    const long long nx = (long long)d.n_nodes * (a.Kp - (d.h ? 0 : d.Kh));
    a.seed = d.seed; a.thr16 = (unsigned)(d.drop_p * 65536.0f + 0.5f); a.mask = d.mask;
    a.x_dropped = (d.x_dropped && d.drop_p > 0.f && a.thr16 != 0u) ? 1 : 0;
    a.x_mask = (a.x_dropped && d.h != nullptr && nx > 0) ? 1 : 0;
    a.drop_scale = 1.f / (1.f - d.drop_p);
    a.nb_x = nx > 0 ? build_x_blocks(T, d.n_nodes, d.Kh, d.Pd, a.Kp, d.h != nullptr, a.x_dropped != 0, 2048) : 0;
    a.n_words = (d.drop_p > 0.f) ? (long long)d.n_nodes * ((a.Kt + 31) / 32) : 0;
    a.nb_m = a.x_mask ? 0 : blocks(a.n_words, 1024);
    a.pk_rows = a.Kt; a.pk_ext = a.Kt; a.pk_prows = round_up(a.Kp, 128); a.pk_cols = d.Fo; a.pk_pcols = round_up(d.Fo, 32);
    a.nb_w = blocks(((long long)a.pk_prows * a.pk_pcols / 4 + PREP_U - 1) / PREP_U, 512);
    a.nb_f = 0; a.fold_bx = 1;
    a.h = d.h; a.ld_h = d.ld_h; a.pos = d.pos; a.P = d.P; a.n_rows = d.n_nodes; a.Kh = d.Kh; a.Pd = d.Pd; a.X = d.X;
    a.W = d.W; a.Wp = d.Wp; a.pk_extra = d.bias_row;
    return TXE_OK;
}
}
extern "C" {
int txe_gcn_layer_prepare(const float* h, long long ld_h, int n_nodes, int Kh, const int* pos, const float* P, int Pd, float* X,
                          const float* W, int Fo, float* Wp, float drop_p, unsigned long long seed, unsigned* mask, int x_dropped,
                          const float* bias_row, void* stream) {
    const txe_gcn_prepare_desc d{h, ld_h, n_nodes, Kh, pos, P, Pd, X, W, Fo, Wp, drop_p, seed, mask, x_dropped, bias_row};
    PrepArgs a;
    const int rc = fill_prep_gcn(a, d);
    if (rc) return rc;
    hipLaunchKernelGGL(gat_prepare_kernel, dim3(a.nb_x + a.nb_m + a.nb_w), dim3(64 * FOLD_DG), 0, (hipStream_t)stream, a);
    TXE_CHECK_LAUNCH();
    return TXE_OK;
}

int txe_gcn_layers_prepare(const struct txe_gcn_prepare_desc* descs, int n_layers, const int* rowptr_in, int n_nodes, float* norm, void* stream) {
    if (!descs || n_layers < 1 || (rowptr_in && (n_nodes < 0 || !norm))) return TXE_ERR_ARG;
    for (int i0 = 0; i0 < n_layers; i0 += PREP_MAXL) {
        PrepMulti m;
        memset(&m, 0, sizeof(m));
        m.n = n_layers - i0 < PREP_MAXL ? n_layers - i0 : PREP_MAXL;
        if (i0 == 0 && rowptr_in && n_nodes > 0) {
            m.nb_norm = (n_nodes + 64 * FOLD_DG - 1) / (64 * FOLD_DG); m.norm_rowptr = rowptr_in; m.norm_n = n_nodes; m.norm = norm;
        }
        int total = 0;
        for (int i = 0; i < m.n; ++i) {
            const int rc = fill_prep_gcn(m.a[i], descs[i0 + i]);
            if (rc) return rc;
            total += m.a[i].nb_x + m.a[i].nb_m + m.a[i].nb_w;
            m.nb_end[i] = total;
        }
        if (total + m.nb_norm == 0) continue;
        hipLaunchKernelGGL(gat_prepare_multi_kernel, dim3(total + m.nb_norm), dim3(64 * FOLD_DG), 0, (hipStream_t)stream, m);
        TXE_CHECK_LAUNCH();
    }
    return TXE_OK;
}

int txe_gather_add_rows(const float* T, long long ld_t, const int* row, const float* T2, long long ld_t2, const int* row2, long long n_rows,
                        int n_cols, float* Y, long long ld_y, void* stream) {
    if (n_rows < 0 || n_cols < 4 || (n_cols & 3) || !T || !row || !Y || (T2 && !row2) || (ld_t & 3) || (ld_y & 3) || (T2 && (ld_t2 & 3)))
        return TXE_ERR_ARG;
    if ((((uintptr_t)T | (uintptr_t)Y | (uintptr_t)T2) & 15) != 0) return TXE_ERR_ARG;
    if (n_rows == 0) return TXE_OK;
    const int nvec = n_cols / 4;
    const long long total = n_rows * nvec;
    const int nb = (int)((total + 255) / 256 < 16384 ? (total + 255) / 256 : 16384);
    ProfScope prof("gather_add_rows_kernel", (hipStream_t)stream, 4.0 * 2.0 * n_rows * (double)n_cols, 1);
    hipLaunchKernelGGL(gather_add_rows_kernel, dim3(nb), dim3(256), 0, (hipStream_t)stream, T, ld_t, row, T2, ld_t2, row2, n_rows, nvec, Y, ld_y);
    TXE_CHECK_LAUNCH();
    return TXE_OK;
}

int txe_gat_dx_streams(int Kh, int Pd, int need_dh) {
    if (need_dh || Pd < 1 || Kh < 1) return 0;
    const int c0 = (Kh / 4) * 4;
    return (Kh + Pd - c0 <= DXPOS_MAXC && Kh - c0 + Pd <= DXPOS_MAXC) ? 1 : 0;
}

static inline size_t dense_bwd_split_bytes(int n_nodes, int Fp, int Kt) {
    return align_up(split_packed_bytes(n_nodes, Fp), 256) + align_up(split_packed_bytes(Kt, Fp), 256);
}
size_t txe_gat_dense_bwd_split_ws_bytes(int n_nodes, int Kh, int Pd, int H, int D) {
    if (n_nodes < 1 || Kh < 1 || Pd < 0 || H < 1 || D < 1) return 0;
    return dense_bwd_split_bytes(n_nodes, round_up(H * D + 2 * H, 128), Kh + Pd);
}
size_t txe_gat_dense_ws_bytes(int n_nodes, int Kh, int Pd, int H, int D, int vocab) {
    return plan_dense_ws(nullptr, n_nodes, round_up(H * D + 2 * H, 128), 2 * H, round_up(Kh + Pd, 32), Pd, vocab).total;
}

int txe_gat_dense_fwd(const float* X, int n_nodes, int Kh, int Pd, const float* Wp, int H, int D, float feat_drop_p,
                      const unsigned* mask, float* Y, void* ws, size_t ws_bytes, void* stream) {
    if (n_nodes < 0 || Kh < 1 || Pd < 0 || H < 1 || D < 1 || !X || !Wp || !Y) return TXE_ERR_ARG;
    if (feat_drop_p < 0.f || feat_drop_p >= 1.f) return TXE_ERR_ARG;
    if (n_nodes == 0) return TXE_OK;
    const int Fe = H * D + 2 * H, Fp = round_up(Fe, 128), Kp = round_up(Kh + Pd, 32);
    VMat A = vmat_plain(X, Kp, n_nodes, Kp);
    vmat_set_mask(A, mask, feat_drop_p);
    VMat B = vmat_plain(Wp, Kp, Fp, Kp);
    Epi E = epi_plain(Y, Fp, Fe);
    E.alg_flops = 2.0 * n_nodes * (double)Fe * (Kh + Pd);
    E.k_valid = Kh + Pd;
    const bool tail_ok = ws && ws_bytes >= gemm_tail_ws_bytes();
    return gemm_nt(A, B, E, n_nodes, Fe, Kp, 1, (hipStream_t)stream, tail_ok ? ws : nullptr, tail_ok ? ws_bytes : 0);
}

size_t txe_gat_dense_split_ws_bytes(int n_nodes, int Kh, int Pd, int H, int D) {
    if (n_nodes < 1 || Kh < 1 || Pd < 0 || H < 1 || D < 1) return 0;
    const int Fp = round_up(H * D + 2 * H, 128), Kp = round_up(Kh + Pd, 32);
    return align_up(split_packed_bytes(n_nodes, Kp), 256) + align_up(split_packed_bytes(Fp, Kp), 256);
}
size_t txe_gat_dense_split_xt_bytes(int n_nodes, int Kh, int Pd, int H, int D) {
    if (n_nodes < 1 || Kh < 1 || Pd < 0 || H < 1 || D < 1) return 0;
    const int Fp = round_up(H * D + 2 * H, 128), Kp = round_up(Kh + Pd, 32);
    return (split_tn_eligible(Fp, Kp) && split_tn_fits(n_nodes, Fp)) ? split_packed_t_bytes(n_nodes, Kp) : 0;
}
int txe_gat_dense_fwd_split(const float* X, int n_nodes, int Kh, int Pd, const float* Wp, int H, int D, const void* Xs, const void* Ws,
                            void* Xt_out, float* Y, void* ws, size_t ws_bytes, void* stream) {
    if (n_nodes < 0 || Kh < 1 || Pd < 0 || H < 1 || D < 1 || !Y || (!Xs && !X) || (!Ws && !Wp)) return TXE_ERR_ARG;
    if (n_nodes == 0) return TXE_OK;
    const int Fe = H * D + 2 * H, Fp = round_up(Fe, 128), Kp = round_up(Kh + Pd, 32);
    hipStream_t s = (hipStream_t)stream;
    char* w = (char*)ws;
    size_t off = 0;
    int rc;
    if (Xt_out && (!X || !split_tn_eligible(Fp, Kp))) return TXE_ERR_ARG;
    bool xt_done = false;
    const int Kc = round_up(Kh + Pd, 16);
    if (!Xs && !Ws) {
        const size_t ba = align_up(split_packed_bytes(n_nodes, Kp), 256), bb = align_up(split_packed_bytes(Fp, Kp), 256);
        if (!ws || ws_bytes < ba + bb) return TXE_ERR_WORKSPACE;
        rc = split_pack_layer_launch(X, Kp, n_nodes, Wp, Kp, Fp, Kc, Kp, w, w + ba, Xt_out, s);
        if (rc) return rc;
        Xs = w; Ws = w + ba; xt_done = true;
    }
    if (!Xs) {
        const size_t b = align_up(split_packed_bytes(n_nodes, Kp), 256);
        if (!ws || ws_bytes < off + b) return TXE_ERR_WORKSPACE;
        rc = split_pack_launch(X, Kp, n_nodes, Kc, 0, w + off, s);
        if (rc) return rc;
        Xs = w + off; off += b;
    }
    if (!Ws) {
        const size_t b = align_up(split_packed_bytes(Fp, Kp), 256);
        if (!ws || ws_bytes < off + b) return TXE_ERR_WORKSPACE;
        rc = split_pack_launch(Wp, Kp, Fp, Kc, 1, w + off, s);
        if (rc) return rc;
        Ws = w + off; off += b;
    }
    rc = gemm_nt_split_launch(Xs, Ws, n_nodes, Fe, Kc, Y, Fp, 2.0 * n_nodes * (double)Fe * (Kh + Pd), s);
    if (rc) return rc;
    if (Xt_out && !xt_done) return split_pack_t_launch(X, Kp, n_nodes, Kp, Xt_out, s);
    return TXE_OK;
}

int txe_gat_dense_fwd_split_src(const float* h, long long ld_h, const int* pos, const float* P, const unsigned* mask, float feat_drop_p,
                                int n_nodes, int Kh, int Pd, const float* Wp, int H, int D, void* Xt_out, float* Y, void* ws, size_t ws_bytes,
                                void* stream) {
    if (n_nodes < 0 || Kh < 1 || Pd < 0 || H < 1 || D < 1 || !Y || !h || !Wp || ld_h < Kh || (Pd > 0 && (!pos || !P)) || feat_drop_p < 0.f ||
        feat_drop_p >= 1.f || (feat_drop_p > 0.f && !mask))
        return TXE_ERR_ARG;
    if (n_nodes == 0) return TXE_OK;
    const int Fe = H * D + 2 * H, Fp = round_up(Fe, 128), Kp = round_up(Kh + Pd, 32);
    hipStream_t s = (hipStream_t)stream;
    char* w = (char*)ws;
    if (Xt_out && !split_tn_eligible(Fp, Kp)) return TXE_ERR_ARG;
    const int Kc = round_up(Kh + Pd, 16);
    const size_t ba = align_up(split_packed_bytes(n_nodes, Kp), 256), bb = align_up(split_packed_bytes(Fp, Kp), 256);
    if (!ws || ws_bytes < ba + bb) return TXE_ERR_WORKSPACE;
    SplitVSrc vs{h, ld_h, pos, P, Kh, Pd, feat_drop_p > 0.f ? mask : nullptr, (Kh + Pd + 31) / 32, 1.f / (1.f - feat_drop_p)};
    int rc = split_pack_layer_launch(nullptr, Kp, n_nodes, Wp, Kp, Fp, Kc, Kp, w, w + ba, Xt_out, s, &vs);
    if (rc) return rc;
    return gemm_nt_split_launch(w, w + ba, n_nodes, Fe, Kc, Y, Fp, 2.0 * n_nodes * (double)Fe * (Kh + Pd), s);
}

int txe_gat_dense_bwd(const float* X, int n_nodes, int Kh, int Pd, const int* pos, int vocab, const float* Wp, const float* W,
                      const float* attn_l, const float* attn_r, int H, int D, float feat_drop_p, const unsigned* mask, const float* d_Y,
                      int need_dh, int act_on, float act_slope, float* d_X, float* dW, float* d_attn_l, float* d_attn_r, float* dP,
                      int x_dropped, const void* Xt, int phases, void* chain, void* ws, size_t ws_bytes, void* stream) {
    if (n_nodes < 0 || Kh < 1 || Pd < 0 || H < 1 || D < 1 || (!X && (!Xt || act_on)) || !Wp || !W || !attn_l || !attn_r || !d_Y || !dW || !d_attn_l || !d_attn_r || !ws)
        return TXE_ERR_ARG;
    static_assert(sizeof(TailChain) <= TXE_TAIL_CHAIN_BYTES, "txe.h: TXE_TAIL_CHAIN_BYTES");
    if ((need_dh || Pd > 0) && !d_X) return TXE_ERR_ARG;
    if (Pd > 0 && (!pos || !dP || vocab < 1 || vocab > MAX_VOCAB)) return TXE_ERR_ARG;
    if (feat_drop_p < 0.f || feat_drop_p >= 1.f) return TXE_ERR_ARG;
    const int F = H * D, H2 = 2 * H, Fe = F + H2, Fp = round_up(Fe, 128), Kt = Kh + Pd, Kp = round_up(Kt, 32);
    DenseWs p = plan_dense_ws(ws, n_nodes, Fp, H2, Kp, Pd, vocab);
    if (ws_bytes < p.total) return TXE_ERR_WORKSPACE;
    hipStream_t s = (hipStream_t)stream;
    int rc;
    const int c0 = need_dh ? 0 : (Kh / 4) * 4;
    const bool stream_dx = txe_gat_dx_streams(Kh, Pd, need_dh) == 1 && n_nodes > 0;
    DxPosArgs da;
    memset(&da, 0, sizeof(da));
    if (stream_dx) {
        da.dY = d_Y; da.ld_dy = Fp; da.n_rows = n_nodes; da.K = Fp;
        da.Wp = Wp; da.ld_w = Kp; da.Kp = Kp; da.c0 = c0; da.NC = Kt - c0;
        da.mask = mask; da.mask_ld = (Kt + 31) / 32; da.mask_on = (mask && feat_drop_p > 0.f) ? 1 : 0;
        da.drop_scale = da.mask_on ? 1.f / (1.f - feat_drop_p) : 1.f;
        da.dX = d_X; da.ld_dx = Kp;
        da.pos = pos; da.vocab = vocab; da.Pd = Pd; da.pcol0 = Kh - c0; da.ppart = p.ppart; da.part = p.dxpart;
        rc = dxpos_prepare(da);
        if (rc) return rc;
    }
    if ((phases & 1) && stream_dx) {
        rc = dxpos_launch(da, s);
        if (rc) return rc;
    } else if ((phases & 1) && (phases & 16) && need_dh && n_nodes > 0) {
        if (ws_bytes < p.total + dense_bwd_split_bytes(n_nodes, Fp, Kt)) return TXE_ERR_WORKSPACE;
        char* sw = (char*)ws + p.total;
        const size_t ba = align_up(split_packed_bytes(n_nodes, Fp), 256);
        const int Fc = round_up(Fe, 16);
        rc = split_pack_launch(d_Y, Fp, n_nodes, Fc, 0, sw, s);
        if (rc) return rc;
        rc = split_pack_launch(Wp, Kp, Kt, Fc, 3, sw + ba, s);
        if (rc) return rc;
        SplitEpi e;
        memset(&e, 0, sizeof(e));
        e.drop_scale = 1.f;
        if (mask && feat_drop_p > 0.f) { e.mask = mask; e.mask_ld = (Kt + 31) / 32; e.mask_col0 = 0; e.drop_scale = 1.f / (1.f - feat_drop_p); }
        if (act_on) { e.act_src = X; e.ld_act = Kp; e.act_slope = act_slope; e.cols_act = Kh; }
        rc = gemm_nt_split_launch(sw, sw + ba, n_nodes, Kt, Fc, d_X, Kp, 2.0 * n_nodes * (double)Kt * Fe, s, &e);
        if (rc) return rc;
    } else if ((phases & 1) && Kt - c0 > 0 && n_nodes > 0 && (need_dh || Pd > 0)) {
        VMat A = vmat_plain(d_Y, Fp, n_nodes, Fp);
        VMat B = vmat_plain(Wp + c0, Kp, Fp, Kp - c0);
        Epi E = epi_plain(d_X + c0, Kp, Kh > c0 ? Kh - c0 : 0);
        E.c2 = d_X + c0 + E.cols_main; E.ldc2 = Kp;
        epi_set_mask(E, mask, Kt, c0, feat_drop_p);
        if (act_on && need_dh) epi_set_act(E, X + c0, Kp, act_slope);
        E.alg_flops = 2.0 * n_nodes * (double)(need_dh ? Kt : Pd) * Fe;
        rc = gemm_nn(A, B, E, n_nodes, Kt - c0, Fp, 1, s, p.tail, p.tail_bytes);
        if (rc) return rc;
    }
    VMat A = vmat_plain(d_Y, Fp, n_nodes, Fp);
    VMat B = vmat_plain(X, Kp, n_nodes, Kp);
    if (!x_dropped) vmat_set_mask(B, mask, feat_drop_p);
    Epi E = epi_plain(p.part, Kp, Kp);
    E.split_stride = (long long)Fp * Kp;
    E.alg_flops = 2.0 * Fe * (double)Kt * n_nodes;
    const int splits = p.splits;
    if ((phases & 2) && Xt && x_dropped + (feat_drop_p == 0.f) > 0 && split_tn_eligible(Fp, Kp) && split_tn_fits(n_nodes, Fp) && n_nodes > 0) {
        const int ks = round_up((n_nodes + splits - 1) / splits, 16);
        rc = gemm_tn_split_launch(d_Y, Fp, Fp, Xt, Kp, n_nodes, splits, ks, p.part, Kp, E.split_stride, E.alg_flops, s);
        if (rc) return rc;
    } else if (phases & 2) {
        if (!X) return TXE_ERR_ARG;
        rc = gemm_tn(A, B, E, Fp, Kp, n_nodes, splits, s);
        if (rc) return rc;
    }
    if (!(phases & 4)) return TXE_OK;
    const int S = n_nodes > 0 ? splits : 0;
    const int nseg = (Pd > 0 && n_nodes > 0) ? (stream_dx ? dxpos_blocks(n_nodes) : p.seg_blocks) : 0;
    TailA ta;
    memset(&ta, 0, sizeof(ta));
    ta.nb_dx = stream_dx ? nseg : 0; ta.dx = da;
// ... 145 lines not shown
```

### taxoexpan_amd/ops.py

```python
import weakref

import torch

from . import _lib
from ._lib import call, ptr, pure

LEAKY_SLOPE = 0.01


def _need_cuda(*ts):
    for t in ts:
        if t is not None and not t.is_cuda:
            raise RuntimeError("taxoexpan_amd: tensors must live on the MI355X (no CPU fallback exists); "
                               "got a host tensor")


def _f32(t):
    if t is None:
        return None
    if t.dtype != torch.float32:
        t = t.float()
    return t if t.is_contiguous() else t.contiguous()


def _rows(t):
    if t.dtype != torch.float32:
        t = t.float()
    if t.dim() != 2 or t.stride(1) != 1 or t.stride(0) < t.shape[1]:
        t = t.contiguous()
    return t, t.stride(0)


_BACKWARD_TWICE = ("taxoexpan_amd: backward through this propagation stack a second time -- its saved activations (several hundred MB per "
                   "batch) are released by the first backward; run the forward again (retain_graph=True is not supported here)")
_NO_FUSED_LOGITS = False
_NO_TABLE_SWEEP = False
_NO_SIDE_STREAM = False
_NO_MATCH_FOLD = False
_NO_FOLD_EDOT = False
_NO_FUSED_BWD = False
_NO_QUERY_RUNS = False
_NO_SPLIT_GEMM = False
_NO_TAIL_CHAIN = False
_FWD_SWEEP = 0
_NO_VIRTUAL_X = False
_NO_WALK_PLAN = False
_NO_EGO_WALK = False
_I32_MEMO = {}


def _i32(t, device):
    if t is None:
        return None
    if t.dtype == torch.int32 and t.device == device:
        return t.contiguous()
    key = id(t)
    hit = _I32_MEMO.get(key)
    if hit is not None and hit[0]() is t and hit[1] == t._version and hit[2] == device:
        return hit[3]
    out = t.to(device=device, dtype=torch.int32).contiguous()
    if len(_I32_MEMO) > 64:
        for k in [k for k, v in _I32_MEMO.items() if v[0]() is None]:
            del _I32_MEMO[k]
        if len(_I32_MEMO) > 64:
            _I32_MEMO.clear()
    _I32_MEMO[key] = (weakref.ref(t), t._version, device, out)
    return out


def _empty(shape, ref, dtype=torch.float32):
    return torch.empty(shape, dtype=dtype, device=ref.device)


def _ws(nbytes, ref):
    return torch.empty(max(int(nbytes), 16), dtype=torch.uint8, device=ref.device)


def new_seed():
    return int(torch.randint(0, 2 ** 62, (1,), dtype=torch.int64).item())


ROUTES = {}


def note_route(kind, name):
    ROUTES[kind] = name
    if _CAPTURE is not None:
        _CAPTURE.routes.append((kind, name))


_GRAD_READY = None
_GRAD_FLUSH = None
_CAPTURE = None


class _CaptureList(list):

    def __init__(self):
        super().__init__()
        self.routes = []


class debug_capture:

    def __enter__(self):
        global _CAPTURE
        self._prev, _CAPTURE = _CAPTURE, _CaptureList()
        return _CAPTURE

    def __exit__(self, *exc):
        global _CAPTURE
        _CAPTURE = self._prev
        return False


def apply_stack(fn, csr, cfg, *args):
    cfg.grad_enabled = torch.is_grad_enabled()
    return fn.apply(csr, cfg, *args)


class GatheredRows:

    def __init__(self, table, index):
        self.table, self.index = table, index
        self._tensor = None

    shape = property(lambda self: torch.Size((self.index.shape[0], self.table.shape[1])))
    device = property(lambda self: self.table.device)
# ... 86 lines not shown
    s = _lib.stream_ptr()
    Kt = pure("txe_gat_padded_k", Kh, 0)
    Xt = _empty((n_tab, Kt), tab)
    call("txe_gat_build_x", ptr(tab), tab.stride(0), n_tab, Kh, None, None, 0, ptr(Xt), s)
    Wp = _empty((Fp, Kp), tab)
    call("txe_gat_pack_weights", ptr(st.W), ptr(st.al), ptr(st.ar), st.H, st.D, Kh + st.Pd, ptr(Wp), s)
    tws = _tail_ws(tab)
    T = _empty((n_tab, Fp), tab)
    if _NO_SPLIT_GEMM:
        call("txe_gemm_plain", 0, ptr(Xt), Kt, ptr(Wp), Kp, ptr(T), Fp, n_tab, Fp, min(Kt, Kp), 1, 0, ptr(tws), tws.numel(), s)
    else:
        wsb = pure("txe_gemm_plain_split_ws_bytes", n_tab, Fp, min(Kt, Kp))
        sws = _ws(wsb, tab)
        call("txe_gemm_plain", 0, ptr(Xt), Kt, ptr(Wp), Kp, ptr(T), Fp, n_tab, Fp, min(Kt, Kp), 1, 8, ptr(sws), wsb, s)
    T2 = None
    if st.Pd > 0:
        T2 = _empty((st.P.shape[0], Fp), tab)
        call("txe_gemm_plain", 0, ptr(st.P), st.Pd, ptr(Wp) + 4 * Kh, Kp, ptr(T2), Fp, st.P.shape[0], Fp, st.Pd, 1, 0, None, 0, s)
    if _PROJ_CACHE is not None:
        _PROJ_CACHE[key] = (T, T2, Wp, src.table, st.W)
        return _PROJ_CACHE[key]
    return T, T2


def _gcn_table_projection(st, src):
    key = ("gcn", src.table.data_ptr(), tuple(src.table.shape), st.W.data_ptr(), None if st.P is None else st.P.data_ptr())
    if _PROJ_CACHE is not None and key in _PROJ_CACHE:
        return _PROJ_CACHE[key]
    tab = src.table
    n_tab, Kh, Fop = tab.shape[0], st.Kh, st.Fop
    s = _lib.stream_ptr()
    Kt = pure("txe_gat_padded_k", Kh, 0)
    Xt = _empty((n_tab, Kt), tab)
    call("txe_gat_build_x", ptr(tab), tab.stride(0), n_tab, Kh, None, None, 0, ptr(Xt), s)
    kp128 = (st.Kp + 127) // 128 * 128
    Wp = _empty((kp128, Fop), tab)
    call("txe_gcn_pack_weights", ptr(st.W), Kh + st.Pd, st.Fo, ptr(Wp), s)
    tws = _tail_ws(tab)
    T = _empty((n_tab, Fop), tab)
    call("txe_gemm_plain", 1, ptr(Xt), Kt, ptr(Wp), Fop, ptr(T), Fop, n_tab, Fop, min(Kt, kp128), 1, 0, ptr(tws), tws.numel(), s)
    T2 = None
    if st.Pd > 0:
        T2 = _empty((st.P.shape[0], Fop), tab)
        call("txe_gemm_plain", 1, ptr(st.P), st.Pd, ptr(Wp) + 4 * Kh * Fop, Fop, ptr(T2), Fop, st.P.shape[0], Fop, st.Pd, 1, 0, None, 0, s)
    if _PROJ_CACHE is not None:
        _PROJ_CACHE[key] = (T, T2, Wp, src.table, st.W)
        return _PROJ_CACHE[key]
    return T, T2


class GATConfig:

    def __init__(self, heads, out_dims, pos_dims, vocab, attn_slope, act_slope, feat_p, attn_p, final, seed):
        self.heads, self.out_dims, self.pos_dims, self.vocab = list(heads), list(out_dims), list(pos_dims), vocab
        self.attn_slope, self.act_slope = float(attn_slope), act_slope
        self.feat_p, self.attn_p = float(feat_p), float(attn_p)
        self.final = final
        self.seed = int(seed)
        self.n_layers = len(self.heads)


def dropout_mask(n_rows, n_cols, p, seed, ref):
    if p <= 0.0:
        return None
    mask = torch.empty((n_rows, (n_cols + 31) // 32), dtype=torch.int32, device=ref.device)
    call("txe_dropout_mask", n_rows, n_cols, p, seed, ptr(mask), _lib.stream_ptr())
    return mask


_tail_ws_cache = {}


def _tail_ws(ref):
    key = (ref.device.index, torch.cuda.current_stream(ref.device).cuda_stream)
    t = _tail_ws_cache.get(key)
    if t is None:
        t = torch.empty(pure("txe_gemm_tail_ws_bytes"), dtype=torch.uint8, device=ref.device)
        _tail_ws_cache[key] = t
    return t


class _GatLayerState:
    __slots__ = ("X", "Wp", "mask", "Y", "alpha", "W", "al", "ar", "P", "Kh", "Pd", "Kp", "Fp", "H", "D", "seed", "cl", "prepared", "x_dropped", "Xt",
                 "vx")


def _virtual_x_ok(st, h, ld_h, N, need, first_is_folded):
    if _NO_SPLIT_GEMM or _NO_VIRTUAL_X or first_is_folded or N == 0 or not torch.is_tensor(h) or h.dtype != torch.float32:
        return False
    if pure("txe_gat_dense_split_ws_bytes", N, st.Kh, st.Pd, st.H, st.D) == 0:
        return False
    return (not need) or pure("txe_gat_dense_split_xt_bytes", N, st.Kh, st.Pd, st.H, st.D) > 0


def _x_dropped_ok(cfg, states, l, collapse):
    L = len(states)
    if collapse and l == L - 1:
        return False
    if l == 0:
        return True
    sp = states[l - 1]
    return sp.D % 4 == 0 and states[l].Kp % 4 == 0 and sp.H <= 4


def _gat_layers_prepare(items, feat_p):
    import ctypes
    descs = (_lib.GatPrepareDesc * len(items))()
    for d, (st, h, ld_h, pos, dropped) in zip(descs, items):
        N = st.X.shape[0]
        st.vx = getattr(st, "vx", False)
        st.Wp = _empty((st.Fp, st.Kp), st.X)
        st.mask = torch.empty((N, (st.Kh + st.Pd + 31) // 32), dtype=torch.int32, device=st.X.device) if feat_p > 0.0 else None
        d.h, d.ld_h, d.n_nodes, d.Kh, d.pos, d.P, d.Pd, d.X = ptr(h), ld_h, N, st.Kh, ptr(pos), ptr(st.P), st.Pd, (None if st.vx else ptr(st.X))
        d.W, d.attn_l, d.attn_r, d.H, d.D, d.Wp = ptr(st.W), ptr(st.al), ptr(st.ar), st.H, st.D, ptr(st.Wp)
        d.feat_drop_p, d.seed, d.mask = feat_p, st.seed, ptr(st.mask)
        st.x_dropped = bool(dropped and feat_p > 0.0)
        d.x_dropped = int(st.x_dropped)
        st.prepared = True
    call("txe_gat_layers_prepare", ctypes.cast(descs, ctypes.c_void_p), len(items), _lib.stream_ptr())


def _gat_layer_prepare(st, h, ld_h, pos, feat_p):
    if getattr(st, "prepared", False):
        return
    N = st.X.shape[0]
    s = _lib.stream_ptr()
    st.Wp = _empty((st.Fp, st.Kp), st.X)
    st.mask = torch.empty((N, (st.Kh + st.Pd + 31) // 32), dtype=torch.int32, device=st.X.device) if feat_p > 0.0 else None
    call("txe_gat_layer_prepare", ptr(h), ld_h, N, st.Kh, ptr(pos), ptr(st.P), st.Pd, ptr(st.X), ptr(st.W), ptr(st.al), ptr(st.ar),
         st.H, st.D, ptr(st.Wp), feat_p, st.seed, ptr(st.mask), s)


def _gat_collapse_fwd(csr, st, h, ld_h, pos, rpos, pw, feat_p, attn_p, attn_slope, a12=None, z_only=False, fold_job=None, link=None):
    N, G, E = st.X.shape[0], csr.n_graphs, csr.n_edges
    ready = a12 is not None
    if not ready:
        _gat_layer_prepare(st, h, ld_h, pos, feat_p)
        a12 = _empty((max(N, 1), 2), st.X)
    alpha, coef = _empty((max(E, 1),), st.X), _empty((max(N, 1),), st.X)
    wsum, Z, hg = _empty((max(G, 1),), st.X), _empty((max(G, 1), st.Kp), st.X), (None if z_only else _empty((G, st.D), st.X))
    gid = torch.empty(max(N, 1), dtype=torch.int32, device=st.X.device)
    wsb = pure("txe_gat_collapse_ws_bytes", N, E, G, st.Kh, st.Pd, st.D, 8)
    split_hg = not z_only and G > 0 and not _NO_SPLIT_GEMM
    if split_hg:
        wsb += pure("txe_gat_collapse_split_ws_bytes", G, st.Kh, st.Pd, st.D)
    ws = _ws(wsb, st.X)
    Tf = zrow = e_part = None
    if z_only and fold_job is not None and link is not None and N > 0 and G > 0 and not _NO_FOLD_EDOT:
        nt = pure("txe_gat_collapse_e_tiles", N, G, st.Kh, st.Pd)
        fw = fold_job(st.Wp, st.D) if nt > 0 else None
        if fw is not None:
            Tf, zrow, e_part = fw["T"], _fold_job_run_ids(fw, G, st.X), _empty((N, nt), st.X)
            link.fwd, link.e_part = fw, e_part
            fw["score"] = (csr.graph_off, N, G, st.Kh, st.Pd, coef, wsum, feat_p, int(st.mask is not None and feat_p > 0.0))
    call("txe_gat_collapse_fwd", ptr(csr.rowptr_in), ptr(csr.col_src), ptr(csr.rowptr_out), ptr(csr.col_dst), ptr(csr.pos_out),
         ptr(csr.graph_off), N, E, G, ptr(st.X), st.Kh, st.Pd, ptr(st.Wp), st.D, feat_p, ptr(st.mask), attn_slope, attn_p, st.seed + 1,
         ptr(rpos), ptr(pw), ptr(a12), int(ready) | (2 if split_hg else 0), ptr(alpha), ptr(coef), ptr(wsum), ptr(gid), ptr(Z), ptr(hg), st.D, ptr(Tf), ptr(zrow),
         ptr(e_part), ptr(ws), wsb, _lib.stream_ptr())
    st.cl = (a12, alpha, coef, wsum, gid, Z, hg)
    return Z if z_only else hg


def _gat_collapse_bwd(csr, st, pos, rpos, pw, vocab, feat_p, attn_p, attn_slope, d_hg, act_on, act_slope):
    N, G, E = st.X.shape[0], csr.n_graphs, csr.n_edges
    a12, alpha, coef, wsum, gid, Z, hg = st.cl
    d_hg, ld = _rows(d_hg)
    dW, dal, dar = torch.empty_like(st.W), torch.empty_like(st.al), torch.empty_like(st.ar)
    dP = torch.empty_like(st.P) if st.P is not None else None
    d_pw = torch.empty_like(pw) if pw is not None else None
    d_X = _empty((N, st.Kp), st.X)
    v = max(vocab, pw.numel() if pw is not None else 0)
    wsb = pure("txe_gat_collapse_ws_bytes", N, E, G, st.Kh, st.Pd, st.D, max(v, 8))
    ws = _ws(wsb, st.X)
    call("txe_gat_collapse_bwd", ptr(csr.rowptr_in), ptr(csr.col_src), ptr(csr.rowptr_out), ptr(csr.col_dst), ptr(csr.pos_out),
         ptr(csr.graph_off), N, E, G, ptr(st.X), st.Kh, st.Pd, ptr(pos if pos is not None else rpos), v, ptr(st.Wp), ptr(st.W),
         ptr(st.al), ptr(st.ar), st.D, feat_p, ptr(st.mask), attn_slope, attn_p, st.seed + 1, ptr(pw), ptr(a12), ptr(alpha), ptr(coef),
         ptr(wsum), ptr(gid), ptr(Z), ptr(hg), st.D, ptr(d_hg), ld, int(act_on), act_slope if act_slope else 1.0, ptr(d_X), ptr(dW), ptr(dal), ptr(dar), ptr(dP),
         ptr(d_pw), ptr(ws), wsb, _lib.stream_ptr())
    return d_X, dW, dal, dar, dP, d_pw


def _gat_layer_fwd(csr, st, h, ld_h, pos, out, ld_out, feat_p, attn_p, attn_slope, out_mode, act_slope, save, nxt=None, out_drop=None):
    H, D, Kh, Pd, Kp, Fp = st.H, st.D, st.Kh, st.Pd, st.Kp, st.Fp
    F = H * D
    s = _lib.stream_ptr()
    if isinstance(h, GatheredRows):
        N = h.index.shape[0]
        T, T2 = _gat_table_projection(st, h)[:2]
        nx_kp = nxt[0].Kp if nxt is not None else 0
        if (T2 is not None and pos is not None and not save and not _NO_TABLE_SWEEP and attn_p == 0.0
                and pure("txe_gat_aggregate_table_supported", H, D, Fp, T2.shape[0], nx_kp) == 1):
            st.Y = st.alpha = None
            call("txe_gat_aggregate_table_fwd", ptr(csr.rowptr_in), ptr(csr.col_src), N, ptr(T), Fp, ptr(_i32(h.index, T.device)), ptr(T2),
                 ptr(pos), T2.shape[0], H, D, attn_slope, out_mode, act_slope, ptr(out), ld_out,
                 *((ptr(nxt[0].Wp) + 4 * nxt[0].D * nxt[0].Kp, nx_kp, ptr(nxt[1])) if nxt is not None else (None, 0, None)),
                 4 if _NO_EGO_WALK else (_FWD_SWEEP if H == 4 and D % 4 == 0 else 0), s)
            return
        st.Y = _empty((N, Fp), T)
        call("txe_gather_add_rows", ptr(T), Fp, ptr(_i32(h.index, T.device)), ptr(T2), Fp, ptr(pos) if T2 is not None else None, N, Fp,
             ptr(st.Y), Fp, s)
    else:
        N = st.X.shape[0]
        _gat_layer_prepare(st, h, ld_h, pos, feat_p)
        st.Y = _empty((N, Fp), st.X)
        tws = _tail_ws(st.X)
        dropped = getattr(st, "x_dropped", False)
        if (dropped or feat_p == 0.0) and not _NO_SPLIT_GEMM:
            wsb = pure("txe_gat_dense_split_ws_bytes", N, Kh, Pd, H, D)
            sws = _ws(wsb, st.X)
            xtb = pure("txe_gat_dense_split_xt_bytes", N, Kh, Pd, H, D) if save else 0
            st.Xt = _ws(xtb, st.X) if xtb else None
            if getattr(st, "vx", False):
                call("txe_gat_dense_fwd_split_src", ptr(h), ld_h, ptr(pos), ptr(st.P), ptr(st.mask), feat_p if st.mask is not None else 0.0,
                     N, Kh, Pd, ptr(st.Wp), H, D, ptr(st.Xt), ptr(st.Y), ptr(sws), wsb, s)
            else:
                call("txe_gat_dense_fwd_split", ptr(st.X), N, Kh, Pd, ptr(st.Wp), H, D, None, None, ptr(st.Xt), ptr(st.Y), ptr(sws), wsb, s)
            note_route("proj", "bf16x6")
        else:
            call("txe_gat_dense_fwd", ptr(st.X), N, Kh, Pd, ptr(st.Wp), H, D, 0.0 if dropped else feat_p, None if dropped else ptr(st.mask), ptr(st.Y),
                 ptr(tws), tws.numel(), s)
            note_route("proj", "fp32")
        _launch_pending_prefetch()
    st.alpha = _empty((max(csr.n_edges, 1), H), st.Y) if save else None
    call("txe_gat_aggregate_fwd", ptr(csr.rowptr_in), ptr(csr.col_src), N, ptr(st.Y), Fp, ptr(st.Y) + 4 * F, ptr(st.Y) + 4 * (F + H), Fp,
         H, D, attn_slope, attn_p, st.seed + 1, out_mode, act_slope, ptr(out), ld_out, ptr(st.alpha),
         *((ptr(nxt[0].Wp) + 4 * nxt[0].D * nxt[0].Kp, nxt[0].Kp, ptr(nxt[0].mask), feat_p, ptr(nxt[1])) if nxt is not None
           else ((None, out_drop.Kp, ptr(out_drop.mask), feat_p, None) if out_drop is not None else (None, 0, None, 0.0, None))),
         4 if _NO_EGO_WALK else (_FWD_SWEEP if H == 4 and D % 4 == 0 else 0), s)


def _gat_aggregate_bwd(csr, st, attn_p, attn_slope, d_pre, ld_dpre):
    N = st.X.shape[0]
    H, D, Fp = st.H, st.D, st.Fp
    F, Fe = H * D, H * D + 2 * H
    d_Y = _empty((N, Fp), st.X)
    dz = _empty((max(csr.n_edges, 1) * H,), st.X)
    call("txe_gat_aggregate_bwd", ptr(csr.rowptr_in), ptr(csr.col_src), ptr(csr.rowptr_out), ptr(csr.col_dst), ptr(csr.pos_out),
         N, ptr(st.Y), Fp, ptr(st.Y) + 4 * F, ptr(st.Y) + 4 * (F + H), Fp, H, D, attn_slope, attn_p, st.seed + 1, ptr(st.alpha),
         ptr(d_pre), ld_dpre, ptr(d_Y), Fp, ptr(d_Y) + 4 * F, ptr(d_Y) + 4 * (F + H), Fp, ptr(dz), Fp - Fe, _lib.stream_ptr())
    return d_Y


class _TailChain:

    def __init__(self):
        import ctypes
        self.buf = ctypes.create_string_buffer(_lib.TAIL_CHAIN_BYTES)
        self.ptr = ctypes.cast(self.buf, ctypes.c_void_p)
        self.keep = []


def _gat_dense_bwd(st, pos, vocab, feat_p, d_Y, need_dh, act_on, act_slope, chain=None, defer=False):
    N = st.X.shape[0]
    dW, dal, dar = torch.empty_like(st.W), torch.empty_like(st.al), torch.empty_like(st.ar)
    dP = torch.empty_like(st.P) if st.P is not None else None
    d_X = _empty((N, st.Kp), st.X) if (need_dh or st.Pd > 0) else None
    wsb = pure("txe_gat_dense_ws_bytes", N, st.Kh, st.Pd, st.H, st.D, vocab)
    split_dx = bool(need_dh) and not _NO_SPLIT_GEMM
    if split_dx:
        wsb += pure("txe_gat_dense_bwd_split_ws_bytes", N, st.Kh, st.Pd, st.H, st.D)
    ws = _ws(wsb, st.X)
    def run(phases):
        call("txe_gat_dense_bwd", None if getattr(st, "vx", False) else ptr(st.X), N, st.Kh, st.Pd, ptr(pos), vocab, ptr(st.Wp), ptr(st.W), ptr(st.al), ptr(st.ar), st.H, st.D, feat_p,
             ptr(st.mask), ptr(d_Y), int(need_dh), int(act_on), act_slope if act_slope else 1.0, ptr(d_X), ptr(dW), ptr(dal), ptr(dar),
             ptr(dP), int(getattr(st, "x_dropped", False)), ptr(getattr(st, "Xt", None)), phases, chain.ptr if chain is not None else None, ptr(ws), wsb, _lib.stream_ptr())
    run(7 | (16 if split_dx else 0) | (64 if (defer and chain is not None) else 0))
    if chain is not None:
        chain.keep += [ws, d_Y, st]
    return d_X, dW, dal, dar, dP


def _gat_layer_bwd(csr, st, pos, vocab, feat_p, attn_p, attn_slope, d_pre, ld_dpre, need_dh, act_on, act_slope, chain=None, defer=False):
    d_Y = _gat_aggregate_bwd(csr, st, attn_p, attn_slope, d_pre, ld_dpre)
    return _gat_dense_bwd(st, pos, vocab, feat_p, d_Y, need_dh, act_on, act_slope, chain, defer)


def _order(first, then):
    call("txe_stream_order", first.cuda_stream, then.cuda_stream)


_side_streams = {}


def _side_stream(device):
    s = _side_streams.get(device.index)
    if s is None:
        s = _side_streams[device.index] = torch.cuda.Stream(device=device)
    return s


def _fused_bwd_ok(csr, st, sp):
    return (not _NO_FUSED_BWD and sp.alpha is not None and sp.H * sp.D == st.Kh and st.cl is not None and csr.n_edges > 0
            and pure("txe_gat_fused_bwd_supported", st.Kh, st.Pd, sp.H, sp.D) == 1)


class FoldLink:
    __slots__ = ("part", "S", "fwd", "e_part", "m", "by_k", "one_col")

    def __init__(self):
        self.part, self.S = None, 0
        self.by_k, self.one_col = False, -1
        self.fwd, self.e_part, self.m = None, None, None


def walk_plan(csr):
# ... 31 lines not shown
    v = max(vocab, pw.numel() if pw is not None else 0)
    wsb = pure("txe_gat_collapse_bwd_fused_ws_bytes", N, E, G, st.Kh, st.Pd, st.D, max(v, 8), sp.H)
    ws = _ws(wsb, st.X)
    def run(phases):
        call("txe_gat_collapse_bwd_fused", ptr(csr.rowptr_in), ptr(csr.col_src), ptr(csr.rowptr_out), ptr(csr.col_dst), ptr(csr.pos_out),
             ptr(csr.graph_off), N, E, G, ptr(st.X), st.Kh, st.Pd, ptr(pos if pos is not None else rpos), v, ptr(st.Wp), ptr(st.W),
             ptr(st.al), ptr(st.ar), st.D, feat_p, ptr(st.mask), attn_slope, attn_p, st.seed + 1, ptr(pw), ptr(a12), ptr(alpha), ptr(coef),
             ptr(wsum), ptr(gid), ptr(Z), ptr(hg), st.D, ptr(d_hg), ld, act_slope if act_slope else 1.0, ptr(sp.Y), sp.Fp, sp.H, sp.D,
             attn_slope, attn_p, sp.seed + 1, ptr(sp.alpha), ptr(d_Yp), sp.Fp, sp.Fp - Fe, ptr(dz), ptr(dW), ptr(dal), ptr(dar), ptr(dP),
             ptr(d_pw), phases | (512 if edot else 0) | (1024 if _NO_EGO_WALK else 0), ptr(link.part) if (link is not None and link.S > 0) else None,
             link.S if link is not None else 0, *((ptr(link.e_part), ptr(link.m[0]), ptr(link.m[1]), int(link.m[2]), ptr(link.fwd["T"]),
                                                  ptr(link.fwd["run_id"]), ptr(zgid)) if edot else (None, None, None, 0, None, None, None)),
             ptr(plan), chain.ptr if chain is not None else None, ptr(ws), wsb, _lib.stream_ptr())
    zgid = torch.empty(max(N, 1), dtype=torch.int32, device=st.X.device) if edot else None
    plan = walk_plan(csr) if (sp.H == 4 and not _NO_EGO_WALK and not _NO_WALK_PLAN) else None
    last = 8 | (64 if chain is not None else 0)
    if chain is not None:
        chain.keep += [ws, d_hg, st, sp, zgid] + ([link.part, link.fwd, link.m] if link is not None else [])
    if link is not None:
        if ld != st.Kp and not edot:
            raise RuntimeError("folded graph vector: dZ must have the padded row pitch")
        run(4 | 256)
        run(last | 256)
    elif _NO_SIDE_STREAM:
        run(7 | last)
    else:
        main, side = torch.cuda.current_stream(), _side_stream(st.X.device)
        _order(main, side)
        with torch.cuda.stream(side):
            run(2 | 128)
        run(1 | 128)
        run(4 | 128)
        _order(side, main)
        run(last | 128)
    return d_Yp, dW, dal, dar, dP, d_pw


class GATStackFunction(torch.autograd.Function):
    accepts_gathered_rows = True

    @staticmethod
    def forward(ctx, csr, cfg, h, pos, rpos, pw, *params):
        need = getattr(cfg, "grad_enabled", True) and any(ctx.needs_input_grad)
        z_only = (cfg.final == "collapse_z")
        collapse = (cfg.final == "collapse") or z_only
        table = _use_table(h, need, cfg.feat_p) and not (collapse and cfg.n_layers == 1)
        if isinstance(h, GatheredRows) and not table:
            h = h.tensor()
        if table:
            _need_cuda(h.table, *[p for p in params if p is not None])
            src, ld_h = h, 0
        else:
            _need_cuda(h, *[p for p in params if p is not None])
            h, ld_h = _rows(h)
            src = h
        pos = _i32(pos, h.device)
        rpos = _i32(rpos, h.device) if (collapse and pw is not None) else None
        pwf = _f32(pw.reshape(-1)) if (collapse and pw is not None) else None
        L = cfg.n_layers
        N = h.shape[0]
        states = []
        with _lib.on_device(h.device):
            kh = h.shape[1]
            ref = h.table if table else h
            for l in range(L):
                st = _GatLayerState()
                st.W, st.al, st.ar, st.P = (_f32(p) for p in params[4 * l:4 * l + 4])
                st.H, st.D, st.Kh = cfg.heads[l], cfg.out_dims[l], kh
                st.Pd = 0 if st.P is None else st.P.shape[1]
                st.Kp = pure("txe_gat_padded_k", st.Kh, st.Pd)
                st.Fp = pure("txe_gat_padded_f", st.H, st.D)
                st.seed = cfg.seed + 16 * l
                st.X = None
                states.append(st)
                kh = st.H * st.D
            h = ref
            states[0].X = None if table else _empty((N, states[0].Kp), h)
            if N > 0:
                for l in range(1, L):
                    states[l].X = _empty((N, states[l].Kp), h)
                states[0].vx = (not table) and _virtual_x_ok(states[0], src, ld_h, N, need, collapse and L == 1)
                _gat_layers_prepare([(st, (src if l == 0 else None), (ld_h if l == 0 else 0), pos if st.P is not None else None,
                                      _x_dropped_ok(cfg, states, l, collapse))
                                     for l, st in enumerate(states) if not (table and l == 0)], cfg.feat_p)
            fused_a12 = None
            for l, st in enumerate(states):
                last = (l == L - 1)
                F = st.H * st.D
                if last and collapse:
                    res = _gat_collapse_fwd(csr, st, src if l == 0 else None, ld_h if l == 0 else 0, pos if st.P is not None else None,
                                            rpos, pwf, cfg.feat_p, cfg.attn_p, cfg.attn_slope, a12=fused_a12, z_only=z_only,
                                            fold_job=getattr(cfg, "fold_job", None) if (z_only and need) else None,
                                            link=getattr(cfg, "link", None))
                    if z_only:
                        res = (res, st.Wp)
                        ctx.mark_non_differentiable(st.Wp)
                        ctx.set_materialize_grads(False)
                    if not need:
                        st.cl = st.mask = st.Wp = st.X = None
                    break
                if last:
                    out, ld_out = _empty((N, F), h), F
                else:
                    if states[l + 1].X is None:
                        states[l + 1].X = _empty((N, states[l + 1].Kp), h)
                    out, ld_out = states[l + 1].X, states[l + 1].Kp
                out_mode = 0 if (last or cfg.act_slope is None) else 1
                nxt = None
                if (collapse and l + 1 == L - 1 and N > 0 and st.D % 4 == 0 and states[l + 1].Kp - st.H * st.D <= 128 and states[l + 1].Kp <= 4096
                        and not _NO_FUSED_LOGITS):
                    sn = states[l + 1]
                    _gat_layer_prepare(sn, None, 0, pos if sn.P is not None else None, cfg.feat_p)
                    fused_a12 = _empty((N, 2), h)
                    nxt = (sn, fused_a12)
                out_drop = states[l + 1] if (not last and nxt is None and getattr(states[l + 1], "x_dropped", False)) else None
                _gat_layer_fwd(csr, st, src if l == 0 else None, ld_h if l == 0 else 0, pos if st.P is not None else None, out, ld_out,
                               cfg.feat_p, cfg.attn_p, cfg.attn_slope, out_mode, cfg.act_slope or 1.0, need, nxt, out_drop)
                if not need:
                    st.Y = st.mask = st.Wp = None
                    if l > 0:
                        st.X = None
            H, D = cfg.heads[-1], cfg.out_dims[-1]
            if collapse:
                pass
            elif cfg.final == "mean":
                if H == 1:
                    res = out.view(N, D)
                else:
                    res = _empty((N, D), h)
                    call("txe_head_mean_fwd", ptr(out), H, D, N, ptr(res), _lib.stream_ptr())
            else:
                res = out.view(N, H, D)
        ctx.csr, ctx.cfg, ctx.pos, ctx.states = csr, cfg, pos, (states if need else None)
        ctx.rpos, ctx.pwf, ctx.pw_shape = rpos, pwf, (pw.shape if pwf is not None else None)
        ctx.h_req = ctx.needs_input_grad[2]
        ctx.param_ids, ctx.pw_id = [id(p) for p in params], id(pw)
        ctx.link = getattr(cfg, "link", None) if z_only else None
        note_route("stack", cfg.final + ("+edot" if (z_only and ctx.link is not None and ctx.link.e_part is not None) else ""))
        if _CAPTURE is not None:
            _CAPTURE.append((csr, cfg, states))
        return res

    @staticmethod
    def backward(ctx, d_res, *_unused):
        csr, cfg, pos, states = ctx.csr, ctx.cfg, ctx.pos, ctx.states
        if states is None:
            raise RuntimeError(_BACKWARD_TWICE)
        L = cfg.n_layers
        H, D = cfg.heads[-1], cfg.out_dims[-1]
        z_only = (cfg.final == "collapse_z")
        collapse = (cfg.final == "collapse") or z_only
        link = ctx.link if z_only else None
        edot = link is not None and link.e_part is not None and link.m is not None
        if d_res is None and not edot:
            ctx.states = None
            return (None,) * (6 + 4 * L)
        d_res = None if edot else _f32(d_res)
        N = states[0].X.shape[0]
        grads = [None] * (4 * L)
        d_pw = None
        note_route("stack_bwd", "fused+edot" if edot else ("collapse" if collapse else "layers"))
        with _lib.on_device(states[0].X.device):
            if collapse:
                d_pre, ld_dpre = None, 0
            elif cfg.final == "mean" and H > 1:
                d_pre = _empty((N, H * D), d_res)
                call("txe_head_mean_bwd", ptr(d_res), H, D, N, ptr(d_pre), _lib.stream_ptr())
# ... 1090 lines not shown
```

Baseline: 42.72 million egonet-edges/s.

## Fuse bf16x3 split packing of X and W planes into GAT layer prepare

Adds a packed prepare path that writes the split-precision X and W planes, and the transposed X, while the layer inputs are built and dropout-masked. The dense projection forward can then run straight from these pre-packed planes instead of repacking X and W in a separate kernel. It also adds a fold-attention-and-pack job for weights and lets the split-pack launch skip the W side when it is already packed. The aim is to remove a pack pass and extra global memory traffic per layer, at the cost of more workspace and a more complex prepare kernel.

```diff
diff --git a/include/txe.h b/include/txe.h
--- a/include/txe.h
+++ b/include/txe.h
@@ -29,6 +29,11 @@
     int x_dropped;
 };
 int txe_gat_layers_prepare(const struct txe_gat_prepare_desc* descs, int n_layers, void* stream);
+
+struct txe_gat_prepare_pack { void* Xs; void* Ws; void* Xt; };
+int txe_gat_layers_prepare_packed(const struct txe_gat_prepare_desc* descs, const struct txe_gat_prepare_pack* packs, int n_layers, int flags,
+                                  void* stream);
+int txe_gat_dense_fwd_planes(const void* Xs, const void* Ws, int n_nodes, int Kh, int Pd, int H, int D, float* Y, void* stream);
 
 int txe_gcn_layer_prepare(const float* h, long long ld_h, int n_nodes, int Kh, const int* pos, const float* P, int Pd, float* X,
                           const float* W, int Fo, float* Wp, float drop_p, unsigned long long seed, unsigned* mask, int x_dropped,
diff --git a/taxoexpan_amd/_lib.py b/taxoexpan_amd/_lib.py
--- a/taxoexpan_amd/_lib.py
+++ b/taxoexpan_amd/_lib.py
@@ -99,6 +99,8 @@
     "txe_gat_collapse_bwd": (I, [P, P, P, P, P, P, I, I, I, P, I, I, P, I, P, P, P, P, I, F, P, F, F, U64, P, P, P, P, P, P, P, P, L, P, L, I, F,
                                  P, P, P, P, P, P, P, SZ, P]),
     "txe_gat_layers_prepare": (I, [P, I, P]),
+    "txe_gat_layers_prepare_packed": (I, [P, P, I, I, P]),
+    "txe_gat_dense_fwd_planes": (I, [P, P, I, I, I, I, I, P, P]),
     "txe_gat_fused_bwd_supported": (I, [I, I, I, I]),
     "txe_gat_collapse_bwd_fused_ws_bytes": (SZ, [I, I, I, I, I, I, I, I]),
     "txe_gat_collapse_bwd_fused": (I, [P, P, P, P, P, P, I, I, I, P, I, I, P, I, P, P, P, P, I, F, P, F, F, U64, P, P, P, P, P, P, P, P, L, P, L,
@@ -141,6 +143,10 @@
                 ("attn_r", P), ("H", I), ("D", I), ("Wp", P), ("feat_drop_p", F), ("seed", U64), ("mask", P), ("x_dropped", I)]
 
 
+class GatPreparePack(C.Structure):
+    _fields_ = [("Xs", P), ("Ws", P), ("Xt", P)]
+
+
 class GcnPrepareDesc(C.Structure):
     _fields_ = [("h", P), ("ld_h", L), ("n_nodes", I), ("Kh", I), ("pos", P), ("P", P), ("Pd", I), ("X", P), ("W", P), ("Fo", I), ("Wp", P),
                 ("drop_p", F), ("seed", U64), ("mask", P), ("x_dropped", I), ("bias_row", P)]
diff --git a/taxoexpan_amd/csrc/build.py b/taxoexpan_amd/csrc/build.py
--- a/taxoexpan_amd/csrc/build.py
+++ b/taxoexpan_amd/csrc/build.py
@@ -8,7 +8,7 @@
 SOURCES = ["txe_gemm_nt.hip", "txe_gemm_nn.hip", "txe_gemm_tn.hip", "txe_gemm_split.hip", "txe_gat.hip", "txe_gcn.hip", "txe_project.hip", "txe_fold.hip", "txe_fold_bwd.hip", "txe_dxpos.hip", "txe_readout.hip", "txe_match.hip",
            "txe_graph.hip", "txe_rank.hip", "txe_profile.hip", "txe_egonet.hip", "txe_optim.hip", "txe_loss.hip",
            "txe_mlp_score.hip", "txe_sample.hip", "txe_grouprank.hip"]
-HEADERS = ["txe_common.h", "txe_gemm.h", "txe_gather.h", "txe_colsum.h", "txe_dxpos.h", "txe_gemm_tnlds.h", "txe_skinny.h", "txe_gemm_split.h", "txe_tail.h", "txe_fold.h"]
+HEADERS = ["txe_common.h", "txe_gemm.h", "txe_gather.h", "txe_colsum.h", "txe_dxpos.h", "txe_gemm_tnlds.h", "txe_skinny.h", "txe_gemm_split.h", "txe_split_pack.h", "txe_tail.h", "txe_fold.h"]
 LIB = os.path.join(HERE, "libtxe.so")
 OBJ_DIR = os.path.join(HERE, "build")
 HIPCC = os.environ.get("HIPCC", "/opt/rocm/bin/hipcc")
diff --git a/taxoexpan_amd/csrc/txe_gemm_split.h b/taxoexpan_amd/csrc/txe_gemm_split.h
--- a/taxoexpan_amd/csrc/txe_gemm_split.h
+++ b/taxoexpan_amd/csrc/txe_gemm_split.h
@@ -97,7 +97,10 @@
 int split_pack_t_launch(const float* src, long long ld, int rows, int cols, void* packed, hipStream_t stream);
 struct Epi;
 int gemm_nt_split_epi_launch(const void* Ap, const void* Bp, const Epi& E, int M, int N, int K, hipStream_t stream);
-struct SplitVSrc { const float* h; long long ld_h; const int* pos; const float* P; int Kh, Pd; const unsigned* mask; int wpr; float scale; };
+struct SplitVSrc {
+    const float* h; long long ld_h; const int* pos; const float* P; int Kh, Pd; const unsigned* mask; int wpr; float scale;
+    unsigned long long seed; unsigned thr16; unsigned* mask_out;
+};
 int split_pack_layer_launch(const float* X, long long ldx, int n, const float* W, long long ldw, int f, int K, int Kt_cols, void* Xs, void* Ws,
                             void* Xt, hipStream_t stream, const SplitVSrc* vs = nullptr);
 int gemm_tn_split_launch(const float* A, long long lda, int M, const void* Bt, int N, int n_rows, int S, int ksplit, float* part, long long ldc,
diff --git a/taxoexpan_amd/csrc/txe_gemm_split.hip b/taxoexpan_amd/csrc/txe_gemm_split.hip
--- a/taxoexpan_amd/csrc/txe_gemm_split.hip
+++ b/taxoexpan_amd/csrc/txe_gemm_split.hip
@@ -2,107 +2,13 @@
 #include "txe_common.h"
 #include "txe_gemm.h"
 #include "txe_gemm_split.h"
+#include "txe_split_pack.h"
 
 namespace txe {
 
 typedef __attribute__((ext_vector_type(8))) short bf16x8;
 typedef __attribute__((ext_vector_type(16))) float f32x16s;
 
-template <int NC, int R>
-__device__ __forceinline__ void vsrc_load_rows(const SplitVSrc& v, const int (&row)[R], const int c0, float (&x)[R][NC]) {
-    unsigned word[R];
-    const bool masked = v.mask != nullptr && c0 < v.wpr * 32;
-#pragma unroll
-    for (int r = 0; r < R; ++r) word[r] = masked ? v.mask[(long long)row[r] * v.wpr + (c0 >> 5)] : 0xFFFFFFFFu;
-    if (c0 + NC <= v.Kh) {
-        const bool two = (NC & 1) == 0 && ((reinterpret_cast<uintptr_t>(v.h + c0) & 7) == 0) && (v.ld_h & 1) == 0;
-        if (two) {
-#pragma unroll
-            for (int r = 0; r < R; ++r) {
-                const float* hr = v.h + (long long)row[r] * v.ld_h + c0;
-#pragma unroll
-                for (int q = 0; q + 1 < NC; q += 2) { const float2 t = *reinterpret_cast<const float2*>(hr + q); x[r][q] = t.x; x[r][q + 1] = t.y; }
-            }
-        } else {
-#pragma unroll
-            for (int r = 0; r < R; ++r)
-#pragma unroll
-                for (int q = 0; q < NC; ++q) x[r][q] = v.h[(long long)row[r] * v.ld_h + c0 + q];
-        }
-    } else if (c0 >= v.Kh + v.Pd) {
-#pragma unroll
-        for (int r = 0; r < R; ++r)
-#pragma unroll
-            for (int q = 0; q < NC; ++q) x[r][q] = 0.f;
-        return;
-    } else {
-        int pr[R];
-#pragma unroll
-        for (int r = 0; r < R; ++r) pr[r] = (v.Pd > 0) ? v.pos[row[r]] : 0;
-#pragma unroll
-        for (int r = 0; r < R; ++r)
-#pragma unroll
-            for (int q = 0; q < NC; ++q) {
-                const int c = c0 + q;
-                const float hv = v.h[(long long)row[r] * v.ld_h + min(c, v.Kh - 1)];
-                const float pv = (v.Pd > 0) ? v.P[(long long)pr[r] * v.Pd + min(max(c - v.Kh, 0), v.Pd - 1)] : 0.f;
-                x[r][q] = (c < v.Kh) ? hv : ((c < v.Kh + v.Pd) ? pv : 0.f);
-            }
-    }
-    if (masked) {
-#pragma unroll
-        for (int r = 0; r < R; ++r)
-#pragma unroll
-            for (int q = 0; q < NC; ++q) x[r][q] = ((word[r] >> ((c0 & 31) + q)) & 1u) ? x[r][q] * v.scale : 0.f;
-    }
-}
-struct SplitPackArgs { const float* src; long long ld; int rows, cols, side, nrb, nkt; uint4* dst; int transposed; SplitVSrc v; };
-__device__ __forceinline__ void split_pack_job(const SplitPackArgs& a, const int bid, const int nb) {
-    const float* __restrict__ src = a.src;
-    uint4* __restrict__ dst = a.dst;
-    const int nkt = a.nkt, rows = a.rows, cols = a.cols;
-    const long long ld = a.ld;
-    const long long total = (long long)a.nrb * nkt * 64;
-    for (long long i = (long long)bid * blockDim.x + threadIdx.x; i < total; i += (long long)nb * blockDim.x) {
-        const int l = (int)(i & 63);
-        const long long f = i >> 6;
-        const int kt = (int)(f % nkt), rb = (int)(f / nkt);
-        const int row = split_slot_row(a.side, rb, l & 31), k0 = kt * SPL_KT + 8 * (l >> 5);
-        float x[8];
-#pragma unroll
-        for (int q = 0; q < 8; ++q) x[q] = 0.f;
-        if (a.v.h != nullptr) {
-            if (row < rows) {
-                const int r1[1] = {row};
-                float x1[1][8];
-                vsrc_load_rows<8, 1>(a.v, r1, k0, x1);
-#pragma unroll
-                for (int q = 0; q < 8; ++q) x[q] = x1[0][q];
-            }
-        } else if (a.transposed) {
-            if (row < rows) {
-#pragma unroll
-                for (int q = 0; q < 8; ++q)
-                    if (k0 + q < cols) x[q] = src[(long long)(k0 + q) * ld + row];
-            }
-        } else if (row < rows) {
-            const float* p = src + (long long)row * ld + k0;
-            if (k0 + 7 < cols && ((reinterpret_cast<uintptr_t>(p) & 15) == 0)) {
-                const float4 u = *reinterpret_cast<const float4*>(p), v = *reinterpret_cast<const float4*>(p + 4);
-                x[0] = u.x; x[1] = u.y; x[2] = u.z; x[3] = u.w; x[4] = v.x; x[5] = v.y; x[6] = v.z; x[7] = v.w;
-            } else {
-#pragma unroll
-                for (int q = 0; q < 8; ++q)
-                    if (k0 + q < cols) x[q] = p[q];
-            }
-        }
-        uint4 w1, w2, w3;
-        if (__ballot(split_exceptional8(x)) != 0ull) split_raw8(x, w1, w2, w3);
-        else split3x8(x, w1, w2, w3);
-        uint4* o = dst + f * 3 * 64 + l;
-        o[0] = w1; o[64] = w2; o[128] = w3;
-    }
-}
 __global__ __launch_bounds__(256) void split_pack_kernel(const SplitPackArgs a) { split_pack_job(a, blockIdx.x, gridDim.x); }
 
 struct SplitGemm {
@@ -341,59 +247,6 @@
         }
 }
 
-struct SplitPackTArgs { const float* src; long long ld; int rows, cols, nht, nnt; uint4* dst; SplitVSrc v; };
-__device__ __forceinline__ void split_pack_t_job(const SplitPackTArgs& a, const int bid, const int nb) {
-    const float* __restrict__ src = a.src;
-    uint4* __restrict__ dst = a.dst;
-    const int rows = a.rows, nht = a.nht;
-    const long long ld = a.ld;
-    const long long total = (long long)a.nnt * nht * 64;
-    const int nkb = nht * 5;
-    for (long long i = (long long)bid * blockDim.x + threadIdx.x; i < total; i += (long long)nb * blockDim.x) {
-        const int l = (int)(i & 63), s = l & 31, nh = l >> 5;
-        const long long g = i >> 6;
-        const int h = (int)(g % nht), nt = (int)(g / nht);
-        const int n0 = nt * 16 + nh * 8;
-        float4 q[8];
-        float o[8];
-        const int c4 = min(160 * h + 4 * s, a.cols - 4), c1 = min(160 * h + 128 + s, a.cols - 1);
-        const bool ok4 = 160 * h + 4 * s + 3 < a.cols, ok1 = 160 * h + 128 + s < a.cols;
-        if (a.v.h != nullptr) {
-            int rr[8];
-            float t4[8][4], t1[8][1];
-#pragma unroll
-            for (int r = 0; r < 8; ++r) rr[r] = min(n0 + r, rows - 1);
-            vsrc_load_rows<4, 8>(a.v, rr, c4, t4);
-            vsrc_load_rows<1, 8>(a.v, rr, c1, t1);
-#pragma unroll
-            for (int r = 0; r < 8; ++r) { q[r] = make_float4(t4[r][0], t4[r][1], t4[r][2], t4[r][3]); o[r] = t1[r][0]; }
-        } else {
-#pragma unroll
-        for (int r = 0; r < 8; ++r) {
-            const int row = min(n0 + r, rows - 1);
-            const float* p = src + (long long)row * ld;
-            q[r] = *reinterpret_cast<const float4*>(p + c4);
-            o[r] = p[c1];
-        }
-        }
-#pragma unroll
-        for (int r = 0; r < 8; ++r) {
-            if (n0 + r >= rows || !ok4) q[r] = make_float4(0.f, 0.f, 0.f, 0.f);
-            if (n0 + r >= rows || !ok1) o[r] = 0.f;
-        }
-        uint4* base = dst + ((long long)nt * nkb + 5 * h) * 3 * 64 + l;
-#pragma unroll
-        for (int j = 0; j < 5; ++j) {
-            float x[8];
-#pragma unroll
-            for (int r = 0; r < 8; ++r) x[r] = j == 0 ? q[r].x : (j == 1 ? q[r].y : (j == 2 ? q[r].z : (j == 3 ? q[r].w : o[r])));
-            uint4 w1, w2, w3;
-            if (__ballot(split_exceptional8(x)) != 0ull) split_raw8(x, w1, w2, w3);
-            else split3x8(x, w1, w2, w3);
-            base[(j * 3 + 0) * 64] = w1; base[(j * 3 + 1) * 64] = w2; base[(j * 3 + 2) * 64] = w3;
-        }
-    }
-}
 __global__ __launch_bounds__(256) void split_pack_t_kernel(const SplitPackTArgs a) { split_pack_t_job(a, blockIdx.x, gridDim.x); }
 
 struct SplitPackMulti { SplitPackArgs a[2]; SplitPackTArgs t; int nb[3]; };
@@ -574,25 +427,6 @@
     }
 }
 
-static bool fill_pack(SplitPackArgs& a, int& nb, const float* src, long long ld, int rows, int cols, int side, void* packed) {
-    const int tr = side >> 1;
-    if (!src || !packed || rows < 1 || cols < 1 || ld < (tr ? rows : cols) || side < 0 || side > 3) return false;
-    a.src = src; a.ld = ld; a.rows = rows; a.cols = cols; a.side = side & 1; a.dst = (uint4*)packed; a.transposed = tr;
-    memset(&a.v, 0, sizeof(a.v));
-    a.nrb = ((rows + 767) / 768) * 24; a.nkt = (cols + SPL_KT - 1) / SPL_KT;
-    const long long total = (long long)a.nrb * a.nkt * 64;
-    nb = (int)((total + 255) / 256 < 8192 ? (total + 255) / 256 : 8192);
-    return true;
-}
-static bool fill_pack_t(SplitPackTArgs& a, int& nb, const float* src, long long ld, int rows, int cols, void* packed) {
-    if (!src || !packed || rows < 1 || cols < 4 || cols % 4 != 0 || ld < cols || (ld & 3) != 0 || (reinterpret_cast<uintptr_t>(src) & 15) != 0)
-        return false;
-    a.src = src; a.ld = ld; a.rows = rows; a.cols = cols; a.nht = (cols + 159) / 160; a.nnt = (rows + 15) / 16; a.dst = (uint4*)packed;
-    memset(&a.v, 0, sizeof(a.v));
-    const long long total = (long long)a.nnt * a.nht * 64;
-    nb = (int)((total + 255) / 256);
-    return true;
-}
 int split_pack_launch(const float* src, long long ld, int rows, int cols, int side, void* packed, hipStream_t stream) {
     SplitPackArgs a;
     int nb;
@@ -608,10 +442,12 @@
     memset(&m, 0, sizeof(m));
     if (vs && (!vs->h || vs->Kh < 1 || vs->Pd < 0 || vs->ld_h < vs->Kh || (vs->Pd > 0 && (!vs->pos || !vs->P)) || (vs->mask && vs->wpr < 1))) return TXE_ERR_ARG;
     if (vs) X = reinterpret_cast<const float*>(W);
-    if (!fill_pack(m.a[0], m.nb[0], X, ldx, n, K, 0, Xs) || !fill_pack(m.a[1], m.nb[1], W, ldw, f, K, 1, Ws)) return TXE_ERR_ARG;
+    if (!fill_pack(m.a[0], m.nb[0], X, ldx, n, K, 0, Xs)) return TXE_ERR_ARG;
+    if (!W && !Ws) m.nb[1] = 0;
+    else if (!fill_pack(m.a[1], m.nb[1], W, ldw, f, K, 1, Ws)) return TXE_ERR_ARG;
     if (Xt && !fill_pack_t(m.t, m.nb[2], X, ldx, n, Kt_cols, Xt)) return TXE_ERR_ARG;
     if (vs) { m.a[0].v = *vs; m.t.v = *vs; }
-    ProfScope prof("split_pack_multi_kernel", stream, 10.0 * K * ((Xt ? 2.0 : 1.0) * n + f), 1);
+    ProfScope prof("split_pack_multi_kernel", stream, 10.0 * K * ((Xt ? 2.0 : 1.0) * n + (m.nb[1] ? f : 0)), 1);
     hipLaunchKernelGGL(split_pack_multi_kernel, dim3(m.nb[0] + m.nb[1] + m.nb[2]), dim3(256), 0, stream, m);
     TXE_CHECK_LAUNCH();
     return TXE_OK;
diff --git a/taxoexpan_amd/csrc/txe_project.hip b/taxoexpan_amd/csrc/txe_project.hip
--- a/taxoexpan_amd/csrc/txe_project.hip
+++ b/taxoexpan_amd/csrc/txe_project.hip
@@ -4,6 +4,7 @@
 #include "txe_gather.h"
 #include "txe_dxpos.h"
 #include "txe_gemm_split.h"
+#include "txe_split_pack.h"
 #include "txe_tail.h"
 
 namespace txe {
@@ -35,6 +36,68 @@
                                                                  const float* __restrict__ attn_l, const float* __restrict__ attn_r,
                                                                  int H, int D, float* __restrict__ wa, long long ld_wa) {
     fold_attn_job(blockIdx.x, blockIdx.y, W, ldw, Kt, attn_l, attn_r, H, D, wa, ld_wa);
+}
+
+constexpr int FOLDP_R = 4;
+struct FoldPackArgs {
+    const float *W, *attn_l, *attn_r; int H, D, F, Fe, Kt, nkt, rb0, nch;
+    float* wa; long long ld_wa;
+    uint4* dst;
+};
+__device__ __forceinline__ void fold_pack_job(const FoldPackArgs& a, const int b) {
+    __shared__ float red[FOLDP_R][FOLD_DG][64];
+    __shared__ float val[32][64];
+    const int rb = a.rb0 + b / a.nch, ch = b % a.nch;
+    const int base = split_slot_row(1, rb, 0);
+    const int kl = threadIdx.x & 63, dg = threadIdx.x >> 6;
+    const int k = ch * 64 + kl, kc = (k < a.Kt) ? k : 0;
+    const long long ldw = a.Kt;
+    const int s_lo = max(0, (a.F - base + 1) >> 1), s_hi = min(31, (a.Fe - 1 - base) >> 1);
+    for (int s0 = s_lo; s0 <= s_hi; s0 += FOLDP_R) {
+        float acc[FOLDP_R];
+        const float* at[FOLDP_R];
+        const float* wh[FOLDP_R];
+#pragma unroll
+        for (int j = 0; j < FOLDP_R; ++j) {
+            const int r = base + 2 * min(s0 + j, s_hi) - a.F, h = r % a.H;
+            at[j] = ((r < a.H) ? a.attn_l : a.attn_r) + (long long)h * a.D;
+            wh[j] = a.W + (long long)h * a.D * ldw + kc;
+            acc[j] = 0.f;
+        }
+#pragma unroll 4
+        for (int d = dg; d < a.D; d += FOLD_DG) {
+#pragma unroll
+            for (int j = 0; j < FOLDP_R; ++j) acc[j] = fmaf(at[j][d], wh[j][(long long)d * ldw], acc[j]);
+        }
+#pragma unroll
+        for (int j = 0; j < FOLDP_R; ++j) red[j][dg][kl] = acc[j];
+        __syncthreads();
+        if (dg < FOLDP_R && s0 + dg <= s_hi) {
+            float s = 0.f;
+#pragma unroll
+            for (int g = 0; g < FOLD_DG; ++g) s += red[dg][g][kl];
+            val[s0 + dg][kl] = (k < a.Kt) ? s : 0.f;
+            if (k < a.Kt) a.wa[(long long)(base + 2 * (s0 + dg) - a.F) * a.ld_wa + k] = s;
+        }
+        __syncthreads();
+    }
+    const int ktl = threadIdx.x >> 6, kt = ch * 4 + ktl;
+    if (ktl >= 4 || kt >= a.nkt) return;
+    const int slot = kl & 31, row = base + 2 * slot, kq = 8 * (kl >> 5), k0 = kt * SPL_KT + kq;
+    float x[8];
+#pragma unroll
+    for (int q = 0; q < 8; ++q) {
+        x[q] = 0.f;
+        if (k0 + q < a.Kt) {
+            if (row < a.F) x[q] = a.W[(long long)row * ldw + k0 + q];
+            else if (row < a.Fe) x[q] = val[slot][ktl * SPL_KT + kq + q];
+        }
+    }
+    uint4 w1, w2, w3;
+    if (__ballot(split_exceptional8(x)) != 0ull) split_raw8(x, w1, w2, w3);
+    else split3x8(x, w1, w2, w3);
+    uint4* o = a.dst + ((long long)rb * a.nkt + kt) * 3 * 64 + kl;
+    o[0] = w1; o[64] = w2; o[128] = w3;
 }
 
 __global__ void reduce_ext_rows_kernel(const float* __restrict__ part, int S, long long split_stride, int F, int H2, int ldp,
@@ -336,6 +399,10 @@
     long long n_words; unsigned long long seed; unsigned thr16; unsigned* mask;
     int x_dropped; float drop_scale;
     int x_mask;
+    int nb_fp, nb_pt, nb_px, nb_pw;
+    FoldPackArgs fp;
+    SplitPackTArgs pt;
+    SplitPackArgs px, pw;
 };
 __device__ __forceinline__ void prepare_jobs(const PrepArgs& a, int b) {
     if (b < a.nb_f) {
@@ -344,12 +411,20 @@
         return;
     }
     b -= a.nb_f;
+    if (b < a.nb_fp) { fold_pack_job(a.fp, b); return; }
+    b -= a.nb_fp;
     if (b < a.nb_w) { pack_w_job(b, a.nb_w, a.W, a.pk_rows, a.pk_ext, a.pk_prows, a.pk_cols, a.pk_pcols, a.Wp, a.pk_extra); return; }
     b -= a.nb_w;
     if (b < a.nb_m) { dropout_mask_job(b, a.nb_m, a.n_words, a.seed, a.thr16, a.mask); return; }
     b -= a.nb_m;
     build_x_job(b, a.nb_x, a.h, a.ld_h, a.pos, a.P, a.n_rows, a.Kh, a.Pd, a.Kp, a.X, a.seed, a.x_dropped ? a.thr16 : 0u, a.drop_scale,
                 a.x_mask ? a.mask : nullptr);
+}
+__device__ __forceinline__ void prepare_pack_jobs(const PrepArgs& a, int b) {
+    if (b < a.nb_pt) { split_pack_t_job(a.pt, b, a.nb_pt); return; }
+    b -= a.nb_pt;
+    if (b < a.nb_px) { split_pack_job(a.px, b, a.nb_px); return; }
+    split_pack_job(a.pw, b - a.nb_px, a.nb_pw);
 }
 __global__ __launch_bounds__(64 * FOLD_DG) void gat_prepare_kernel(const PrepArgs a) { prepare_jobs(a, blockIdx.x); }
 
@@ -509,6 +584,7 @@
 struct PrepMulti {
     int n; int nb_end[PREP_MAXL]; PrepArgs a[PREP_MAXL];
     int nb_norm; const int* norm_rowptr; int norm_n; float* norm;
+    int nb_pack_end[PREP_MAXL];
 };
 __global__ __launch_bounds__(64 * FOLD_DG) void gat_prepare_multi_kernel(const PrepMulti m) {
     int b = blockIdx.x, i = 0;
@@ -518,6 +594,12 @@
         return;
     }
     b -= m.nb_norm;
+    if (b >= m.nb_end[m.n - 1]) {
+        b -= m.nb_end[m.n - 1];
+        while (i + 1 < m.n && b >= m.nb_pack_end[i]) ++i;
+        prepare_pack_jobs(m.a[i], b - ((i > 0) ? m.nb_pack_end[i - 1] : 0));
+        return;
+    }
     while (i + 1 < m.n && b >= m.nb_end[i]) ++i;
     prepare_jobs(m.a[i], b - ((i > 0) ? m.nb_end[i - 1] : 0));
 }
@@ -567,6 +649,81 @@
     return TXE_OK;
 }
 
+struct txe_gat_prepare_pack { void* Xs; void* Ws; void* Xt; };
+}
+namespace txe {
+static int fill_prep_packs(PrepArgs& a, const txe_gat_prepare_desc& d, const txe_gat_prepare_pack& p, int flags) {
+    if (!p.Xs && !p.Ws && !p.Xt) return TXE_OK;
+    const int T = 64 * FOLD_DG;
+    const int Kc = round_up(a.Kt, 16), nkt = Kc / SPL_KT;
+    auto blocks = [&](long long threads) { return (int)((threads + T - 1) / T); };
+    int nb;
+    if (p.Xs || p.Xt) {
+        if (!d.h || d.n_nodes < 1 || d.ld_h < d.Kh || (d.feat_drop_p > 0.f && !a.x_dropped)) return TXE_ERR_ARG;
+        if (p.Xt && !split_tn_eligible(a.Fp, a.Kp)) return TXE_ERR_ARG;
+        SplitVSrc vs;
+        memset(&vs, 0, sizeof(vs));
+        vs.h = d.h; vs.ld_h = d.ld_h; vs.pos = d.pos; vs.P = d.P; vs.Kh = d.Kh; vs.Pd = d.Pd; vs.wpr = (a.Kt + 31) / 32;
+        vs.scale = a.drop_scale; vs.seed = d.seed; vs.thr16 = a.x_dropped ? a.thr16 : 0u;
+        const float* any = d.W;
+        if (p.Xs) {
+            if (!fill_pack(a.px, nb, any, a.Kp, d.n_nodes, Kc, 0, p.Xs)) return TXE_ERR_ARG;
+            a.px.v = vs;
+            a.nb_px = blocks((long long)a.px.nrb * a.px.nkt * 64);
+            if (a.x_dropped && !a.x_mask && !(flags & 1)) { a.px.v.mask_out = d.mask; a.nb_m = 0; }
+        }
+        if (p.Xt) {
+            if (!fill_pack_t(a.pt, nb, any, a.Kp, d.n_nodes, a.Kp, p.Xt)) return TXE_ERR_ARG;
+            a.pt.v = vs;
+            a.nb_pt = blocks((long long)a.pt.nnt * a.pt.nht * 64);
+        }
+    }
+    if (p.Ws) {
+        int lo = 1 << 30, hi = -1;
+        for (int r = a.F; r < a.Fe; ++r) {
+            const int rb = 4 * (r >> 7) + 2 * ((r & 127) >> 6) + (r & 1);
+            lo = rb < lo ? rb : lo; hi = rb > hi ? rb : hi;
+        }
+        if (!fill_pack(a.pw, nb, d.W, a.Kt, a.F, a.Kt, 1, p.Ws)) return TXE_ERR_ARG;
+        a.pw.nrb = ((a.Fp + 767) / 768) * 24; a.pw.nkt = nkt;
+        a.pw.skip_lo = lo; a.pw.skip_n = hi - lo + 1;
+        a.nb_pw = blocks((long long)a.pw.nrb * nkt * 64);
+        a.fp = FoldPackArgs{d.W, d.attn_l, d.attn_r, d.H, d.D, a.F, a.Fe, a.Kt, nkt, lo, (nkt + 3) / 4, a.Wp + (long long)a.F * a.Kp, (long long)a.Kp,
+                            (uint4*)p.Ws};
+        a.nb_fp = (hi - lo + 1) * a.fp.nch;
+        a.nb_f = 0;
+    }
+    return TXE_OK;
+}
+}
+extern "C" {
+int txe_gat_layers_prepare_packed(const struct txe_gat_prepare_desc* descs, const struct txe_gat_prepare_pack* packs, int n_layers, int flags,
+                                  void* stream) {
+    if (!descs || !packs || n_layers < 1) return TXE_ERR_ARG;
+    static_assert(sizeof(PrepMulti) <= 4096, "kernel argument block");
+    for (int i0 = 0; i0 < n_layers; i0 += PREP_MAXL) {
+        PrepMulti m;
+        memset(&m, 0, sizeof(m));
+        m.n = n_layers - i0 < PREP_MAXL ? n_layers - i0 : PREP_MAXL;
+        int total = 0, packs_total = 0;
+        for (int i = 0; i < m.n; ++i) {
+            PrepArgs& a = m.a[i];
+            int rc = fill_prep(a, descs[i0 + i]);
+            if (rc) return rc;
+            rc = fill_prep_packs(a, descs[i0 + i], packs[i0 + i], flags);
+            if (rc) return rc;
+            total += a.nb_x + a.nb_m + a.nb_w + a.nb_f + a.nb_fp;
+            m.nb_end[i] = total;
+            packs_total += a.nb_pt + a.nb_px + a.nb_pw;
+            m.nb_pack_end[i] = packs_total;
+        }
+        if (total + packs_total == 0) continue;
+        hipLaunchKernelGGL(gat_prepare_multi_kernel, dim3(total + packs_total), dim3(64 * FOLD_DG), 0, (hipStream_t)stream, m);
+        TXE_CHECK_LAUNCH();
+    }
+    return TXE_OK;
+}
+
 struct txe_gcn_prepare_desc {
     const float* h; long long ld_h; int n_nodes, Kh; const int* pos; const float* P; int Pd; float* X;
     const float* W; int Fo; float* Wp; float drop_p; unsigned long long seed; unsigned* mask; int x_dropped; const float* bias_row;
@@ -710,6 +867,13 @@
         if (rc) return rc;
         Xs = w; Ws = w + ba; xt_done = true;
     }
+    if (!Xs && Ws && Xt_out) {
+        const size_t b = align_up(split_packed_bytes(n_nodes, Kp), 256);
+        if (!ws || ws_bytes < b) return TXE_ERR_WORKSPACE;
+        rc = split_pack_layer_launch(X, Kp, n_nodes, nullptr, 0, 0, Kc, Kp, w, nullptr, Xt_out, s);
+        if (rc) return rc;
+        Xs = w; off = b; xt_done = true;
+    }
     if (!Xs) {
         const size_t b = align_up(split_packed_bytes(n_nodes, Kp), 256);
         if (!ws || ws_bytes < off + b) return TXE_ERR_WORKSPACE;
@@ -748,6 +912,13 @@
     int rc = split_pack_layer_launch(nullptr, Kp, n_nodes, Wp, Kp, Fp, Kc, Kp, w, w + ba, Xt_out, s, &vs);
     if (rc) return rc;
     return gemm_nt_split_launch(w, w + ba, n_nodes, Fe, Kc, Y, Fp, 2.0 * n_nodes * (double)Fe * (Kh + Pd), s);
+}
+
+int txe_gat_dense_fwd_planes(const void* Xs, const void* Ws, int n_nodes, int Kh, int Pd, int H, int D, float* Y, void* stream) {
+    if (n_nodes < 0 || Kh < 1 || Pd < 0 || H < 1 || D < 1 || !Y || !Xs || !Ws) return TXE_ERR_ARG;
+    if (n_nodes == 0) return TXE_OK;
+    const int Fe = H * D + 2 * H, Fp = round_up(Fe, 128);
+    return gemm_nt_split_launch(Xs, Ws, n_nodes, Fe, round_up(Kh + Pd, 16), Y, Fp, 2.0 * n_nodes * (double)Fe * (Kh + Pd), (hipStream_t)stream);
 }
 
 int txe_gat_dense_bwd(const float* X, int n_nodes, int Kh, int Pd, const int* pos, int vocab, const float* Wp, const float* W,
diff --git a/taxoexpan_amd/csrc/txe_split_pack.h b/taxoexpan_amd/csrc/txe_split_pack.h
--- /dev/null
+++ b/taxoexpan_amd/csrc/txe_split_pack.h
@@ -0,0 +1,190 @@
+#pragma once
+#include <string.h>
+#include "txe_common.h"
+#include "txe_gemm_split.h"
+
+namespace txe {
+
+template <int NC, int R>
+__device__ __forceinline__ void vsrc_load_rows(const SplitVSrc& v, const int (&row)[R], const int c0, float (&x)[R][NC],
+                                               unsigned* __restrict__ word_out = nullptr) {
+    unsigned word[R];
+    const bool hashed = v.mask == nullptr && v.thr16 != 0u;
+    const bool masked = (v.mask != nullptr || hashed) && c0 < v.wpr * 32;
+#pragma unroll
+    for (int r = 0; r < R; ++r) word[r] = (masked && !hashed) ? v.mask[(long long)row[r] * v.wpr + (c0 >> 5)] : 0xFFFFFFFFu;
+    if (c0 + NC <= v.Kh) {
+        const bool two = (NC & 1) == 0 && ((reinterpret_cast<uintptr_t>(v.h + c0) & 7) == 0) && (v.ld_h & 1) == 0;
+        if (two) {
+#pragma unroll
+            for (int r = 0; r < R; ++r) {
+                const float* hr = v.h + (long long)row[r] * v.ld_h + c0;
+#pragma unroll
+                for (int q = 0; q + 1 < NC; q += 2) { const float2 t = *reinterpret_cast<const float2*>(hr + q); x[r][q] = t.x; x[r][q + 1] = t.y; }
+            }
+        } else {
+#pragma unroll
+            for (int r = 0; r < R; ++r)
+#pragma unroll
+                for (int q = 0; q < NC; ++q) x[r][q] = v.h[(long long)row[r] * v.ld_h + c0 + q];
+        }
+    } else if (c0 >= v.Kh + v.Pd) {
+#pragma unroll
+        for (int r = 0; r < R; ++r)
+#pragma unroll
+            for (int q = 0; q < NC; ++q) x[r][q] = 0.f;
+        return;
+    } else {
+        int pr[R];
+#pragma unroll
+        for (int r = 0; r < R; ++r) pr[r] = (v.Pd > 0) ? v.pos[row[r]] : 0;
+#pragma unroll
+        for (int r = 0; r < R; ++r)
+#pragma unroll
+            for (int q = 0; q < NC; ++q) {
+                const int c = c0 + q;
+                const float hv = v.h[(long long)row[r] * v.ld_h + min(c, v.Kh - 1)];
+                const float pv = (v.Pd > 0) ? v.P[(long long)pr[r] * v.Pd + min(max(c - v.Kh, 0), v.Pd - 1)] : 0.f;
+                x[r][q] = (c < v.Kh) ? hv : ((c < v.Kh + v.Pd) ? pv : 0.f);
+            }
+    }
+    if (masked && hashed) {
+#pragma unroll
+        for (int r = 0; r < R; ++r) word[r] = drop_mask_word(v.seed, (unsigned long long)row[r] * v.wpr + (c0 >> 5), v.thr16);
+    }
+    if (word_out) {
+#pragma unroll
+        for (int r = 0; r < R; ++r) word_out[r] = word[r];
+    }
+    if (masked) {
+#pragma unroll
+        for (int r = 0; r < R; ++r)
+#pragma unroll
+            for (int q = 0; q < NC; ++q) x[r][q] = ((word[r] >> ((c0 & 31) + q)) & 1u) ? x[r][q] * v.scale : 0.f;
+    }
+}
+struct SplitPackArgs { const float* src; long long ld; int rows, cols, side, nrb, nkt; uint4* dst; int transposed, skip_lo, skip_n; SplitVSrc v; };
+__device__ __forceinline__ void split_pack_job(const SplitPackArgs& a, const int bid, const int nb) {
+    const float* __restrict__ src = a.src;
+    uint4* __restrict__ dst = a.dst;
+    const int nkt = a.nkt, rows = a.rows, cols = a.cols;
+    const long long ld = a.ld;
+    const long long total = (long long)a.nrb * nkt * 64;
+    for (long long i = (long long)bid * blockDim.x + threadIdx.x; i < total; i += (long long)nb * blockDim.x) {
+        const int l = (int)(i & 63);
+        const long long f = i >> 6;
+        const int kt = (int)(f % nkt), rb = (int)(f / nkt);
+        const int row = split_slot_row(a.side, rb, l & 31), k0 = kt * SPL_KT + 8 * (l >> 5);
+        if (rb >= a.skip_lo && rb < a.skip_lo + a.skip_n) continue;
+        float x[8];
+#pragma unroll
+        for (int q = 0; q < 8; ++q) x[q] = 0.f;
+        if (a.v.h != nullptr) {
+            if (row < rows) {
+                const int r1[1] = {row};
+                float x1[1][8];
+                unsigned word = 0u;
+                vsrc_load_rows<8, 1>(a.v, r1, k0, x1, &word);
+                if (a.v.mask_out != nullptr && (k0 & 31) == 0 && k0 < a.v.wpr * 32) a.v.mask_out[(long long)row * a.v.wpr + (k0 >> 5)] = word;
+#pragma unroll
+                for (int q = 0; q < 8; ++q) x[q] = x1[0][q];
+            }
+        } else if (a.transposed) {
+            if (row < rows) {
+#pragma unroll
+                for (int q = 0; q < 8; ++q)
+                    if (k0 + q < cols) x[q] = src[(long long)(k0 + q) * ld + row];
+            }
+        } else if (row < rows) {
+            const float* p = src + (long long)row * ld + k0;
+            if (k0 + 7 < cols && ((reinterpret_cast<uintptr_t>(p) & 15) == 0)) {
+                const float4 u = *reinterpret_cast<const float4*>(p), v = *reinterpret_cast<const float4*>(p + 4);
+                x[0] = u.x; x[1] = u.y; x[2] = u.z; x[3] = u.w; x[4] = v.x; x[5] = v.y; x[6] = v.z; x[7] = v.w;
+            } else {
+#pragma unroll
+                for (int q = 0; q < 8; ++q)
+                    if (k0 + q < cols) x[q] = p[q];
+            }
+        }
+        uint4 w1, w2, w3;
+        if (__ballot(split_exceptional8(x)) != 0ull) split_raw8(x, w1, w2, w3);
+        else split3x8(x, w1, w2, w3);
+        uint4* o = dst + f * 3 * 64 + l;
+        o[0] = w1; o[64] = w2; o[128] = w3;
+    }
+}
+
+struct SplitPackTArgs { const float* src; long long ld; int rows, cols, nht, nnt; uint4* dst; SplitVSrc v; };
+__device__ __forceinline__ void split_pack_t_job(const SplitPackTArgs& a, const int bid, const int nb) {
+    const float* __restrict__ src = a.src;
+    uint4* __restrict__ dst = a.dst;
+    const int rows = a.rows, nht = a.nht;
+    const long long ld = a.ld;
+    const long long total = (long long)a.nnt * nht * 64;
+    const int nkb = nht * 5;
+    for (long long i = (long long)bid * blockDim.x + threadIdx.x; i < total; i += (long long)nb * blockDim.x) {
+        const int l = (int)(i & 63), s = l & 31, nh = l >> 5;
+        const long long g = i >> 6;
+        const int h = (int)(g % nht), nt = (int)(g / nht);
+        const int n0 = nt * 16 + nh * 8;
+        float4 q[8];
+        float o[8];
+        const int c4 = min(160 * h + 4 * s, a.cols - 4), c1 = min(160 * h + 128 + s, a.cols - 1);
+        const bool ok4 = 160 * h + 4 * s + 3 < a.cols, ok1 = 160 * h + 128 + s < a.cols;
+        if (a.v.h != nullptr) {
+            int rr[8];
+            float t4[8][4], t1[8][1];
+#pragma unroll
+            for (int r = 0; r < 8; ++r) rr[r] = min(n0 + r, rows - 1);
+            vsrc_load_rows<4, 8>(a.v, rr, c4, t4);
+            vsrc_load_rows<1, 8>(a.v, rr, c1, t1);
+#pragma unroll
+            for (int r = 0; r < 8; ++r) { q[r] = make_float4(t4[r][0], t4[r][1], t4[r][2], t4[r][3]); o[r] = t1[r][0]; }
+        } else {
+#pragma unroll
+        for (int r = 0; r < 8; ++r) {
+            const int row = min(n0 + r, rows - 1);
+            const float* p = src + (long long)row * ld;
+            q[r] = *reinterpret_cast<const float4*>(p + c4);
+            o[r] = p[c1];
+        }
+        }
+#pragma unroll
+        for (int r = 0; r < 8; ++r) {
+            if (n0 + r >= rows || !ok4) q[r] = make_float4(0.f, 0.f, 0.f, 0.f);
+            if (n0 + r >= rows || !ok1) o[r] = 0.f;
+        }
+        uint4* base = dst + ((long long)nt * nkb + 5 * h) * 3 * 64 + l;
+#pragma unroll
+        for (int j = 0; j < 5; ++j) {
+            float x[8];
+#pragma unroll
+            for (int r = 0; r < 8; ++r) x[r] = j == 0 ? q[r].x : (j == 1 ? q[r].y : (j == 2 ? q[r].z : (j == 3 ? q[r].w : o[r])));
+            uint4 w1, w2, w3;
+            if (__ballot(split_exceptional8(x)) != 0ull) split_raw8(x, w1, w2, w3);
+            else split3x8(x, w1, w2, w3);
+            base[(j * 3 + 0) * 64] = w1; base[(j * 3 + 1) * 64] = w2; base[(j * 3 + 2) * 64] = w3;
+        }
+    }
+}
+
+static bool fill_pack(SplitPackArgs& a, int& nb, const float* src, long long ld, int rows, int cols, int side, void* packed) {
+    const int tr = side >> 1;
+    if (!src || !packed || rows < 1 || cols < 1 || ld < (tr ? rows : cols) || side < 0 || side > 3) return false;
+    a.src = src; a.ld = ld; a.rows = rows; a.cols = cols; a.side = side & 1; a.dst = (uint4*)packed; a.transposed = tr;
+    memset(&a.v, 0, sizeof(a.v));
+    a.nrb = ((rows + 767) / 768) * 24; a.nkt = (cols + SPL_KT - 1) / SPL_KT;
+    const long long total = (long long)a.nrb * a.nkt * 64;
+    nb = (int)((total + 255) / 256 < 8192 ? (total + 255) / 256 : 8192);
+    return true;
+}
+static bool fill_pack_t(SplitPackTArgs& a, int& nb, const float* src, long long ld, int rows, int cols, void* packed) {
+    if (!src || !packed || rows < 1 || cols < 4 || cols % 4 != 0 || ld < cols || (ld & 3) != 0 || (reinterpret_cast<uintptr_t>(src) & 15) != 0)
+        return false;
+    a.src = src; a.ld = ld; a.rows = rows; a.cols = cols; a.nht = (cols + 159) / 160; a.nnt = (rows + 15) / 16; a.dst = (uint4*)packed;
+    memset(&a.v, 0, sizeof(a.v));
+    const long long total = (long long)a.nnt * a.nht * 64;
+    nb = (int)((total + 255) / 256);
+    return true;
+}
+}
diff --git a/taxoexpan_amd/ops.py b/taxoexpan_amd/ops.py
--- a/taxoexpan_amd/ops.py
+++ b/taxoexpan_amd/ops.py
@@ -44,6 +44,8 @@
 _NO_TAIL_CHAIN = False
 _FWD_SWEEP = 0
 _NO_VIRTUAL_X = False
+_NO_PREP_PACK = False
+_PREP_PACK_FLAGS = 0
 _NO_WALK_PLAN = False
 _NO_EGO_WALK = False
 _I32_MEMO = {}
@@ -296,6 +298,7 @@
 
 class _GatLayerState:
     __slots__ = ("X", "Wp", "mask", "Y", "alpha", "W", "al", "ar", "P", "Kh", "Pd", "Kp", "Fp", "H", "D", "seed", "cl", "prepared", "x_dropped", "Xt",
+                 "Xs", "Ws", "pk",
                  "vx")
 
 
@@ -317,12 +320,28 @@
     return sp.D % 4 == 0 and states[l].Kp % 4 == 0 and sp.H <= 4
 
 
-def _gat_layers_prepare(items, feat_p):
+def _gat_layers_prepare(items, feat_p, need=False, w_planes=()):
     import ctypes
     descs = (_lib.GatPrepareDesc * len(items))()
-    for d, (st, h, ld_h, pos, dropped) in zip(descs, items):
+    packs = (_lib.GatPreparePack * len(items))()
+    packed = False
+    for d, pk, (st, h, ld_h, pos, dropped) in zip(descs, packs, items):
         N = st.X.shape[0]
         st.vx = getattr(st, "vx", False)
+        st.Xs = st.Ws = st.pk = None
+        if not (_NO_PREP_PACK or _NO_SPLIT_GEMM) and N > 0 and (feat_p == 0.0 or (dropped and int(feat_p * 65536.0 + 0.5) > 0)):
+            if st.vx:
+                ba = (pure("txe_split_packed_bytes", N, st.Kp) + 255) // 256 * 256
+                sws = _ws(pure("txe_gat_dense_split_ws_bytes", N, st.Kh, st.Pd, st.H, st.D), st.X)
+                xtb = pure("txe_gat_dense_split_xt_bytes", N, st.Kh, st.Pd, st.H, st.D) if need else 0
+                st.Xt = _ws(xtb, st.X) if xtb else None
+                st.pk, st.Xs, st.Ws = sws, ptr(sws), ptr(sws) + ba
+                pk.Xs, pk.Ws, pk.Xt = st.Xs, st.Ws, ptr(st.Xt)
+                packed = True
+            elif st in w_planes:
+                st.pk = _ws(pure("txe_split_packed_bytes", st.Fp, st.Kp), st.X)
+                st.Ws = pk.Ws = ptr(st.pk)
+                packed = True
         st.Wp = _empty((st.Fp, st.Kp), st.X)
         st.mask = torch.empty((N, (st.Kh + st.Pd + 31) // 32), dtype=torch.int32, device=st.X.device) if feat_p > 0.0 else None
         d.h, d.ld_h, d.n_nodes, d.Kh, d.pos, d.P, d.Pd, d.X = ptr(h), ld_h, N, st.Kh, ptr(pos), ptr(st.P), st.Pd, (None if st.vx else ptr(st.X))
@@ -331,7 +350,12 @@
         st.x_dropped = bool(dropped and feat_p > 0.0)
         d.x_dropped = int(st.x_dropped)
         st.prepared = True
-    call("txe_gat_layers_prepare", ctypes.cast(descs, ctypes.c_void_p), len(items), _lib.stream_ptr())
+    if packed:
+        call("txe_gat_layers_prepare_packed", ctypes.cast(descs, ctypes.c_void_p), ctypes.cast(packs, ctypes.c_void_p), len(items),
+             _PREP_PACK_FLAGS, _lib.stream_ptr())
+    else:
+        call("txe_gat_layers_prepare", ctypes.cast(descs, ctypes.c_void_p), len(items), _lib.stream_ptr())
+    note_route("prep", "packed" if packed else "plain")
 
 
 def _gat_layer_prepare(st, h, ld_h, pos, feat_p):
@@ -422,19 +446,32 @@
         if (dropped or feat_p == 0.0) and not _NO_SPLIT_GEMM:
             wsb = pure("txe_gat_dense_split_ws_bytes", N, Kh, Pd, H, D)
             sws = _ws(wsb, st.X)
+            if getattr(st, "Xs", None) is not None:
+                call("txe_gat_dense_fwd_planes", st.Xs, st.Ws, N, Kh, Pd, H, D, ptr(st.Y), s)
+                note_route("proj", "bf16x6")
+                _launch_pending_prefetch()
+                return _gat_layer_aggregate(csr, st, N, out, ld_out, feat_p, attn_p, attn_slope, out_mode, act_slope, save, nxt, out_drop)
             xtb = pure("txe_gat_dense_split_xt_bytes", N, Kh, Pd, H, D) if save else 0
             st.Xt = _ws(xtb, st.X) if xtb else None
             if getattr(st, "vx", False):
                 call("txe_gat_dense_fwd_split_src", ptr(h), ld_h, ptr(pos), ptr(st.P), ptr(st.mask), feat_p if st.mask is not None else 0.0,
                      N, Kh, Pd, ptr(st.Wp), H, D, ptr(st.Xt), ptr(st.Y), ptr(sws), wsb, s)
             else:
-                call("txe_gat_dense_fwd_split", ptr(st.X), N, Kh, Pd, ptr(st.Wp), H, D, None, None, ptr(st.Xt), ptr(st.Y), ptr(sws), wsb, s)
+                call("txe_gat_dense_fwd_split", ptr(st.X), N, Kh, Pd, ptr(st.Wp), H, D, None, getattr(st, "Ws", None), ptr(st.Xt), ptr(st.Y), ptr(sws),
+                     wsb, s)
             note_route("proj", "bf16x6")
         else:
             call("txe_gat_dense_fwd", ptr(st.X), N, Kh, Pd, ptr(st.Wp), H, D, 0.0 if dropped else feat_p, None if dropped else ptr(st.mask), ptr(st.Y),
                  ptr(tws), tws.numel(), s)
             note_route("proj", "fp32")
         _launch_pending_prefetch()
+    _gat_layer_aggregate(csr, st, N, out, ld_out, feat_p, attn_p, attn_slope, out_mode, act_slope, save, nxt, out_drop)
+
+
+def _gat_layer_aggregate(csr, st, N, out, ld_out, feat_p, attn_p, attn_slope, out_mode, act_slope, save, nxt, out_drop):
+    H, D, Fp = st.H, st.D, st.Fp
+    F = H * D
+    s = _lib.stream_ptr()
     st.alpha = _empty((max(csr.n_edges, 1), H), st.Y) if save else None
     call("txe_gat_aggregate_fwd", ptr(csr.rowptr_in), ptr(csr.col_src), N, ptr(st.Y), Fp, ptr(st.Y) + 4 * F, ptr(st.Y) + 4 * (F + H), Fp,
          H, D, attn_slope, attn_p, st.seed + 1, out_mode, act_slope, ptr(out), ld_out, ptr(st.alpha),
@@ -632,7 +669,8 @@
                 states[0].vx = (not table) and _virtual_x_ok(states[0], src, ld_h, N, need, collapse and L == 1)
                 _gat_layers_prepare([(st, (src if l == 0 else None), (ld_h if l == 0 else 0), pos if st.P is not None else None,
                                       _x_dropped_ok(cfg, states, l, collapse))
-                                     for l, st in enumerate(states) if not (table and l == 0)], cfg.feat_p)
+                                     for l, st in enumerate(states) if not (table and l == 0)], cfg.feat_p, need,
+                                    [st for l, st in enumerate(states) if l > 0 and not (collapse and l == L - 1)])
             fused_a12 = None
             for l, st in enumerate(states):
                 last = (l == L - 1)
```

Result: slower. 32.82 million egonet-edges/s (-23.2%).
